# HPCForge/Bubbleformer

Measured on AMD Instinct MI355X. Metric: train samples/sec, FiLMAViT 16x192x192x4ch, bs=8 per GPU, higher is better.
Workload: dtype bf16; 1 GPU; FiLMAViT-small (E=384, 6 heads, 12 blocks, P=16, 9 fluid params) fwd + relative-L2 loss + bwd + AdamW, 4-field 16x192x192 clips, batch 8 per GPU (BASELINE.json configs[1]); global_batch=8, parallelism=dp1

## Files before the change

bubbleformer_amd/_lib.py:

```python
import ctypes as C
import os
import subprocess

_HERE = os.path.dirname(os.path.abspath(__file__))
LIB_PATH = os.path.join(_HERE, "libbubbleformer_hip.so")
CSRC = os.path.join(_HERE, "csrc")

BF_DTYPE_F32, BF_DTYPE_BF16 = 0, 1
BF_LAY_KC, BF_LAY_XC = 0, 1
BF_PRO_NONE, BF_PRO_AFFINE, BF_PRO_AFFINE_GELU, BF_PRO_GELU = 0, 1, 2, 3
BF_AUX_NONE, BF_AUX_ADD, BF_AUX_DGELU = 0, 1, 2
BF_OUT_STORE, BF_OUT_STORE_F32, BF_OUT_ATOMIC_F32 = 0, 1, 2
BF_MAX_STAGES = 5
BF_LOSS_LIMBS = 5
BF_OPT_CHUNK, BF_OPT_MAX_GROUPS = 64, 64

vp, fp, i32, i64, f32 = C.c_void_p, C.c_void_p, C.c_int32, C.c_int64, C.c_float


class Operand(C.Structure):
    _fields_ = [("p", vp), ("ld", i64), ("layout", i32), ("seglen", i32), ("segstride", i64), ("gw", i32), ("gh", i32),
                ("gc", i32), ("pro", i32), ("sc", fp), ("sh", fp), ("rows_per_frame", i32), ("nch", i32)]


class Epilogue(C.Structure):
    _fields_ = [("bias", fp), ("colscale", fp), ("colshift", fp), ("aux_mode", i32), ("aux", vp), ("ld_aux", i64),
                ("out_mode", i32), ("c", vp), ("ldc", i64), ("seglen", i32), ("segstride", i64), ("gw", i32), ("gh", i32),
                ("gc", i32), ("gelu_out", vp), ("colsum", fp), ("rowscale", fp), ("rows_per_group", i32)]


class Dims(C.Structure):
    _fields_ = [(n, i32) for n in ("dtype", "B", "T", "h", "w", "E", "heads", "attn_scale", "feat_scale", "patch", "cin",
                                   "cout", "nfluid")]


TEMPORAL_FIELDS = ("gamma", "attn_scale_factor", "norm1_w", "norm1_b", "norm2_w", "norm2_b", "input_head_w", "input_head_b",
                   "output_head_w", "output_head_b", "qnorm_w", "qnorm_b", "knorm_w", "knorm_b", "rel_pos_emb")
SPATIAL_FIELDS = ("gamma_att", "gamma_mlp", "attn_scale_factor_x", "attn_scale_factor_y", "low_freq_scalar",
                  "high_freq_scalar", "norm1_w", "norm1_b", "norm2_w", "norm2_b", "input_head_w", "input_head_b",
                  "output_head_w", "output_head_b", "qnorm_w", "qnorm_b", "knorm_w", "knorm_b", "rel_pos_emb", "fc1_w", "fc1_b",
                  "fc2_w", "fc2_b", "mlp_norm_w", "mlp_norm_b")


class TemporalParams(C.Structure):
    _fields_ = [(n, fp) for n in TEMPORAL_FIELDS]


class SpatialParams(C.Structure):
    _fields_ = [(n, fp) for n in SPATIAL_FIELDS]


class FrameNorm(C.Structure):
    _fields_ = [("w", fp), ("b", fp), ("g", fp), ("gdiv", i32), ("mean", fp), ("rstd", fp), ("sc", fp), ("sh", fp), ("resid", vp), ("out", vp)]


class EmbedParams(C.Structure):
    _fields_ = [("conv_w", fp * BF_MAX_STAGES), ("in_w", fp * BF_MAX_STAGES), ("in_b", fp * BF_MAX_STAGES), ("film_ln_w", fp),
                ("film_ln_b", fp), ("film_w", fp), ("film_b", fp)]


class DebedParams(C.Structure):
    _fields_ = [("conv_w", fp * BF_MAX_STAGES), ("in_w", fp * BF_MAX_STAGES), ("in_b", fp * BF_MAX_STAGES)]


class ConvSrc(C.Structure):
    _fields_ = [("p", vp), ("C", i32), ("nchw", i32), ("f32", i32)]


class ConvGeo(C.Structure):
    _fields_ = [(n, i32) for n in ("F", "Hi", "Wi", "Ho", "Wo", "kh", "kw", "stride", "pad")]


BF_CONV_PRO_NONE, BF_CONV_PRO_AFFINE_GELU, BF_CONV_PRO_GELU = 0, 1, 2


class RolloutStep(C.Structure):
    _fields_ = [("pred", fp), ("frames", fp), ("field_stride", i64), ("total_frames", i64), ("first", vp), ("step", vp), ("field", vp), ("diff", fp),
                ("div", fp)] + [(n, i32) for n in ("nfields", "B", "T", "C", "H", "W", "Ho", "Wo", "steps", "reserved")]


class CensusRows(C.Structure):
    _fields_ = [(n, vp) for n in ("count", "cells", "attached", "area")]


class LinkRows(C.Structure):
    _fields_ = [(n, vp) for n in ("successor", "n_successors", "predecessor", "n_predecessors", "departure_area", "events")]


class MatchRows(C.Structure):
    _fields_ = [(n, vp) for n in ("match_pred", "match_target", "overlap", "displacement", "counts", "mask")]


class ErrorRows(C.Structure):
    _fields_ = [(n, vp) for n in ("rmse", "max_error", "boundary_rmse", "interface_rmse", "interface_cells", "spectral_error", "spectrum_error",
                                  "spectrum_pred", "spectrum_target")]


class EnsembleRows(C.Structure):
    _fields_ = [(n, vp) for n in ("mean_rmse", "spread", "crps", "rank_hist", "mean")]


class OptStep(C.Structure):
    _fields_ = [("p", fp), ("g", fp), ("m", fp), ("v", fp), ("coef_dev", fp), ("avg", fp), ("chunk_group", vp), ("group_lr_scale", fp),
                ("group_weight_decay", fp), ("group_frozen", vp), ("live_dev", vp), ("n", i64), ("step", i32), ("n_groups", i32)] + [
        (n, f32) for n in ("lr", "beta1", "beta2", "eps", "wd", "gscale", "clip_value", "avg_weight")]


class ClipGatherJob(C.Structure):
    _fields_ = [("src", fp), ("idx", vp), ("first_tab", vp), ("in_field", vp), ("in_diff", fp), ("in_div", fp), ("in_out", fp), ("out_field", vp),
                ("out_diff", fp), ("out_div", fp), ("out_out", fp), ("fluid_tab", fp), ("file_tab", vp), ("fluid_out", fp), ("field_stride", i64),
                ("nframes", i64), ("nsamples", i64)] + [(n, i32) for n in ("Cin", "Tin", "Cout", "Tout", "unroll", "P", "B", "H", "W", "Ho", "Wo", "reserved")]


class ClipAugment(C.Structure):
    _fields_ = [("in_odd", vp), ("out_odd", vp), ("seed", i64), ("flip_thr", i64)] + [(n, i32) for n in ("draw", "Hc", "Wc", "crop_y", "eval_view", "reserved")]


class ClipGatherQ16Job(C.Structure):
    _fields_ = [("codes", vp), ("frame_seg", vp), ("seg_lo", fp), ("seg_step", fp), ("idx", vp), ("first_tab", vp), ("in_field", vp), ("in_diff", fp),
                ("in_div", fp), ("in_out", fp), ("out_field", vp), ("out_diff", fp), ("out_div", fp), ("out_out", fp), ("fluid_tab", fp), ("file_tab", vp),
                ("fluid_out", fp), ("field_stride", i64), ("nframes", i64), ("nsamples", i64)] + [
        (n, i32) for n in ("nfiles", "Cin", "Tin", "Cout", "Tout", "unroll", "P", "B", "H", "W", "Ho", "Wo")]


class RenderTile(C.Structure):
    _fields_ = [("a", fp), ("b", fp), ("mask", fp), ("frame_stride", i64), ("slot_stride", i64), ("mask_frame_stride", i64), ("mask_slot_stride", i64),
                ("range", vp), ("kind", i32)]


class RenderGeom(C.Structure):
    _fields_ = [(n, i32) for n in ("H", "W", "scale", "rows", "cols", "ox", "oy", "pitch_x", "pitch_y", "bar_dx", "bar_w", "img_h", "img_w", "stride")] + [
        ("stroke", C.c_double)]


BF_RENDER_SDF, BF_RENDER_TEMP, BF_RENDER_SPEED = 0, 1, 2
BF_RENDER_MAX_TILES = 6

STAGE_DONE_FN = C.CFUNCTYPE(None, C.c_int, C.c_void_p)
P = C.POINTER
SIGNATURES = {
    "bf_last_error": (C.c_char_p, []),
    "bf_abi_version": (C.c_int, []),
    "bf_prof_enable": (None, [C.c_int]),
    "bf_debug_force_generic_attn": (None, [C.c_int]),
    "bf_debug_tokred_fold": (None, [C.c_int]),
    "bf_side_defer": (None, [C.c_int]),
    "bf_prep_stages": (C.c_int, [C.POINTER(Dims), C.c_int, C.POINTER(C.c_int32), C.POINTER(vp), C.POINTER(vp), C.POINTER(vp), vp]),
    "bf_stage_prepared": (None, [C.c_int]),
    "bf_trunk_train_fwd": (C.c_int, [C.POINTER(Dims), C.c_int, C.POINTER(C.c_int32), C.POINTER(vp), C.POINTER(vp), C.POINTER(vp), C.POINTER(vp), vp,
                                     C.POINTER(vp), vp, vp]),
    "bf_trunk_train_bwd": (C.c_int, [C.POINTER(Dims), C.c_int, C.POINTER(C.c_int32), C.POINTER(vp), C.POINTER(vp), C.POINTER(vp), C.POINTER(vp),
                                     C.POINTER(vp), vp, C.POINTER(vp), vp, C.POINTER(vp), vp, vp, vp, vp, vp]),
    "bf_field_stats_ws_doubles": (i64, [C.c_int]),
    "bf_field_stats": (C.c_int, [fp, vp, vp, C.c_int, vp, vp, vp]),
    "bf_stage_chain_next": (C.c_int, [C.POINTER(Dims), C.c_int, vp, vp]),
    "bf_stage_next_scale": (C.c_int, [fp, C.c_int]),
    "bf_gemm_fwd_frames": (C.c_int, [C.c_int, C.c_int, C.c_int, C.c_int, vp, i64, vp, i64, fp, fp, fp, fp, C.c_int, vp, vp, C.c_int,
                                     C.POINTER(FrameNorm), C.POINTER(FrameNorm), vp]),
    "bf_trunk_eval_weights_bytes": (i64, [C.POINTER(Dims), C.c_int, C.POINTER(C.c_int32)]),
    "bf_trunk_eval_prepare": (C.c_int, [C.POINTER(Dims), C.c_int, C.POINTER(C.c_int32), C.POINTER(vp), vp, vp]),
    "bf_trunk_eval_fwd": (C.c_int, [C.POINTER(Dims), C.c_int, C.POINTER(C.c_int32), C.POINTER(vp), vp, vp, vp, vp, vp]),
    "bf_frame_linear": (C.c_int, [C.c_int, C.c_int, C.c_int, C.c_int, C.c_int, vp, i64, vp, i64, fp, fp, fp, fp, fp, vp, i64, C.c_int, fp, fp, fp,
                                  vp, i64, fp, fp, vp, i64, vp]),
    "bf_side_join": (C.c_int, [vp]),
    "bf_prof_report": (C.c_int, [C.c_char_p, C.c_int]),
    "bf_gemm": (C.c_int, [C.c_int, C.c_int, C.c_int, C.c_int, P(Operand), P(Operand), P(Epilogue), C.c_int, vp]),
    "bf_gemm_tokred": (C.c_int, [C.c_int, C.c_int, C.c_int, i64, vp, i64, vp, i64, fp, C.c_int, fp, fp, i64, vp]),
    "bf_gemm_tokred_ws_floats": (i64, [C.c_int, C.c_int, i64]),
    "bf_gemm_inbwd_frames": (C.c_int, [C.c_int, C.c_int, C.c_int, C.c_int, vp, i64, vp, i64, vp, vp, vp, C.c_int, fp, fp, fp, fp, fp, C.c_int, vp]),
    "bf_gemm_inbwd_frames_chain": (C.c_int, [C.c_int, C.c_int, C.c_int, C.c_int, vp, i64, vp, i64, vp, vp, vp, C.c_int, fp, fp, fp, fp, fp, C.c_int,
                                             vp, vp, fp, fp, fp, fp, C.c_int, fp, vp]),
    "bf_in_stats": (C.c_int, [C.c_int, vp, C.c_int, C.c_int, C.c_int, fp, fp, fp, C.c_int, fp, fp, fp, fp, fp, fp, vp]),
    "bf_in_ws_floats": (i64, [C.c_int, C.c_int, C.c_int, C.c_int]),
    "bf_affine_apply": (C.c_int, [C.c_int, vp, vp, fp, fp, vp, i64, C.c_int, C.c_int, vp]),
    "bf_in_bwd": (C.c_int, [C.c_int, vp, vp, vp, vp, C.c_int, C.c_int, C.c_int, fp, fp, fp, fp, fp, C.c_int, C.c_int, fp, fp,
                            fp, fp, fp, vp]),
    "bf_colsum": (C.c_int, [C.c_int, vp, i64, C.c_int, fp, fp, vp]),
    "bf_attn_axial_fwd": (C.c_int, [C.c_int, vp, vp, i64, C.c_int, C.c_int, C.c_int, C.c_int, fp, fp, fp, fp, fp, fp, fp, vp]),
    "bf_attn_axial_norm_fwd": (C.c_int, [C.c_int, vp, vp, vp, i64, C.c_int, C.c_int, C.c_int, C.c_int, fp, fp, fp, fp, fp, fp, fp, fp, fp, fp, fp, fp,
                                         fp, vp]),
    "bf_attn_fwd": (C.c_int, [C.c_int, vp, vp, i64, C.c_int, i64, i64, i64, i64, C.c_int, C.c_int, fp, fp, fp, fp, fp, fp, f32,
                              C.c_int, vp]),
    "bf_attn_bwd": (C.c_int, [C.c_int, vp, vp, vp, i64, C.c_int, i64, i64, i64, i64, C.c_int, C.c_int, fp, fp, fp, fp, fp, fp,
                              fp, fp, fp, fp, fp, fp, f32, C.c_int, fp, i64, vp]),
    "bf_im2col_nchw": (C.c_int, [C.c_int, fp, vp, C.c_int, C.c_int, C.c_int, C.c_int, C.c_int, vp]),
    "bf_col2im_nchw": (C.c_int, [C.c_int, vp, fp, C.c_int, C.c_int, C.c_int, C.c_int, C.c_int, vp]),
    "bf_pm2nchw": (C.c_int, [fp, fp, fp, fp, C.c_int, C.c_int, C.c_int, C.c_int, C.c_int, vp]),
    "bf_debed_last_bwd": (C.c_int, [C.c_int, fp, fp, fp, fp, fp, vp, vp, vp, C.c_int, C.c_int, C.c_int, C.c_int, C.c_int, C.c_int, vp]),
    "bf_debed_last_bwd_norm": (C.c_int, [C.c_int, fp, fp, fp, fp, fp, vp, vp, vp, fp, fp, fp, fp, vp, fp, fp, C.c_int, C.c_int, C.c_int, C.c_int, C.c_int,
                                         C.c_int, fp, C.c_int64, vp]),
    "bf_gather_gemm": (C.c_int, [C.c_int, vp, vp, C.c_int, fp, fp, vp, C.c_int, C.c_int, C.c_int, C.c_int, C.c_int, vp]),
    "bf_scatter_gemm": (C.c_int, [C.c_int, vp, vp, C.c_int, fp, fp, vp, fp, C.c_int, C.c_int, C.c_int, C.c_int, C.c_int, vp]),
    "bf_gather_wgrad_ws_floats": (C.c_int64, [C.c_int, C.c_int, C.c_int]),
    "bf_gather_wgrad": (C.c_int, [C.c_int, vp, vp, fp, fp, fp, fp, fp, C.c_int, C.c_int, C.c_int, C.c_int, C.c_int, C.c_int, fp, C.c_int64, vp]),
    "bf_gather_gemm_rebuilt": (C.c_int, [C.c_int, vp, vp, vp, C.c_int, fp, fp, vp, C.c_int, C.c_int, C.c_int, C.c_int, C.c_int, vp]),
    "bf_gather_wgrad_rebuilt": (C.c_int, [C.c_int, vp, vp, vp, fp, fp, fp, C.c_int, C.c_int, C.c_int, C.c_int, C.c_int, C.c_int, fp, C.c_int64, vp]),
    "bf_stage_chain_head": (C.c_int, [vp, vp, vp]),
    "bf_stage_chain_tail": (C.c_int, [vp, vp, C.c_int]),
    "bf_embed_tail_ws_floats": (C.c_int64, [C.c_int, C.c_int, C.c_int, C.c_int, C.c_int]),
    "bf_embed_tail_bwd": (C.c_int, [C.c_int, vp, vp, vp, vp, vp, fp, fp, fp, fp, fp, fp, fp, fp, C.c_int, C.c_int, C.c_int, C.c_int, C.c_int, C.c_int,
                                    fp, C.c_int64, vp]),
    "bf_embed_first": (C.c_int, [C.c_int, fp, vp, vp, vp, C.c_int, C.c_int, C.c_int, C.c_int, C.c_int, C.c_int, fp, vp]),
    "bf_in_stats_merge_slices": (C.c_int, [C.c_int, C.c_int, C.c_int, C.c_int, C.c_int, fp, fp, fp, C.c_int, fp, fp, fp, fp, fp, fp, vp]),
    "bf_debed_last": (C.c_int, [C.c_int, vp, fp, fp, vp, fp, fp, fp, C.c_int, C.c_int, C.c_int, C.c_int, C.c_int, C.c_int, vp]),
    "bf_lploss_finalize": (C.c_int, [fp, C.c_int, C.c_int, fp, fp, vp]),
    "bf_nchw2pm": (C.c_int, [C.c_int, fp, fp, fp, fp, fp, vp, C.c_int, C.c_int, C.c_int, C.c_int, C.c_int, vp]),
    "bf_wprep": (C.c_int, [C.c_int, C.c_int, fp, vp, C.c_int, C.c_int, C.c_int, vp]),
    "bf_wgrad_unprep": (C.c_int, [C.c_int, fp, fp, C.c_int, C.c_int, C.c_int, C.c_int, vp]),
    "bf_film_net_fwd": (C.c_int, [fp, fp, fp, fp, fp, fp, fp, fp, C.c_int, C.c_int, C.c_int, vp]),
    "bf_film_net_bwd": (C.c_int, [fp, fp, fp, fp, fp, fp, fp, fp, fp, C.c_int, C.c_int, C.c_int, vp]),
    "bf_adamw": (C.c_int, [P(OptStep), vp]),
    "bf_adam": (C.c_int, [P(OptStep), vp]),
    "bf_lion": (C.c_int, [P(OptStep), vp]),
    "bf_grad_norm_ws_doubles": (i64, [i64]),
    "bf_grad_norm": (C.c_int, [fp, i64, f32, f32, fp, vp, i64, vp]),
    "bf_weight_average": (C.c_int, [fp, fp, i64, f32, vp]),
    "bf_swap_buffers": (C.c_int, [fp, fp, i64, vp]),
    "bf_group_sumsq_ws_doubles": (i64, [i64]),
    "bf_group_sumsq": (C.c_int, [fp, i64, vp, C.c_int, vp, vp, i64, vp]),
    "bf_group_clip_coef": (C.c_int, [vp, vp, C.c_int, f32, f32, fp, fp, vp]),
    "bf_step_guard": (C.c_int, [fp, i32, vp, vp]),
    "bf_nonfinite_scan_ws_len": (i64, [i64]),
    "bf_nonfinite_scan": (C.c_int, [fp, i64, vp, vp, i64, vp]),
    "bf_eikonal_sum": (C.c_int, [fp, i64, C.c_int, C.c_int, f32, vp, vp]),
    "bf_eikonal_l1_frames": (C.c_int, [fp, i64, C.c_int, C.c_int, f32, fp, vp]),
    "bf_heatflux_rows": (C.c_int, [fp, fp, i64, i64, C.c_int, f32, f32, f32, f32, fp, vp]),
    "bf_clip_gather": (C.c_int, [fp, i64, vp, vp, C.c_int, fp, fp, fp, C.c_int, C.c_int, C.c_int, C.c_int, C.c_int, C.c_int, C.c_int, vp]),
    "bf_clip_gather_batch": (C.c_int, [fp, i64, vp, i64, vp, vp, fp, fp, C.c_int, C.c_int, fp, vp, fp, fp, C.c_int, C.c_int, fp, fp, vp, C.c_int, fp,
                                       C.c_int, C.c_int, C.c_int, C.c_int, C.c_int, vp]),
    "bf_clip_gather_unroll": (C.c_int, [fp, i64, i64, vp, i64, vp, vp, fp, fp, C.c_int, C.c_int, fp, vp, fp, fp, C.c_int, C.c_int, C.c_int, fp, fp, vp, C.c_int,
                                        fp, C.c_int, C.c_int, C.c_int, C.c_int, C.c_int, vp]),
    "bf_clip_gather_augment": (C.c_int, [P(ClipGatherJob), P(ClipAugment), vp]),
    "bf_clip_encode_q16": (C.c_int, [fp, vp, i64, f32, f32, vp]),
    "bf_clip_decode_q16": (C.c_int, [vp, i64, vp, fp, fp, fp, i64, C.c_int, C.c_int, C.c_int, C.c_int, vp]),
    "bf_clip_gather_q16": (C.c_int, [P(ClipGatherQ16Job), P(ClipAugment), vp]),
    "bf_clip_noise": (C.c_int, [fp, fp, fp, vp, C.c_uint64, C.c_uint32, C.c_uint32, C.c_int, C.c_int, C.c_int, C.c_int, C.c_int, vp]),
    "bf_rollout_score_ws_doubles": (i64, [C.c_int, C.c_int, C.c_int, C.c_int, C.c_int]),
    "bf_rollout_score": (C.c_int, [P(RolloutStep), C.c_int, f32, fp, fp, fp, fp, fp, fp, vp, i64, vp]),
    "bf_rollout_heatflux": (C.c_int, [P(RolloutStep), C.c_int, C.c_int, fp, f32, f32, f32, f32, fp, fp, vp]),
    "bf_kde_kl_ws_doubles": (i64, [C.c_int, i64, i64, C.c_int]),
    "bf_kde_kl": (C.c_int, [vp, vp, C.c_int, i64, i64, C.c_int, C.c_double, vp, vp, vp, vp, vp, i64, vp]),
    "bf_bubble_census_lds_cells": (i64, []),
    "bf_bubble_census_ws_bytes": (i64, [i64, C.c_int, C.c_int, C.c_int]),
    "bf_bubble_census": (C.c_int, [fp, i64, C.c_int, C.c_int, C.c_int, C.c_int, vp, vp, vp, vp, fp, vp, vp, vp, i64, vp]),
    "bf_rollout_bubbles": (C.c_int, [P(RolloutStep), C.c_int, C.c_int, C.c_int, P(CensusRows), P(CensusRows), vp, vp, i64, vp]),
    "bf_redistance_lds_cells": (i64, []),
    "bf_redistance_ws_bytes": (i64, [i64, C.c_int, C.c_int]),
    "bf_redistance": (C.c_int, [fp, i64, C.c_int, C.c_int, f32, f32, C.c_int, fp, vp, fp, vp, i64, vp]),
    "bf_rollout_redistance": (C.c_int, [P(RolloutStep), C.c_int, f32, f32, C.c_int, C.c_int, fp, vp, fp, vp, i64, vp]),
    "bf_bubble_links_lds_entries": (i64, []),
    "bf_bubble_links_ws_bytes": (i64, [i64, C.c_int]),
    "bf_bubble_links": (C.c_int, [vp, P(CensusRows), i64, C.c_int, C.c_int, C.c_int, C.c_int, P(LinkRows), vp, i64, vp]),
    "bf_bubble_track_ids": (C.c_int, [vp, vp, vp, i64, C.c_int, C.c_int, vp, vp, vp]),
    "bf_rollout_bubble_links": (C.c_int, [P(RolloutStep), C.c_int, vp, P(CensusRows), P(CensusRows), P(LinkRows), P(LinkRows), vp, i64, vp]),
    "bf_bubble_match_ws_bytes": (i64, [i64, C.c_int]),
    "bf_bubble_match": (C.c_int, [vp, vp, P(CensusRows), P(CensusRows), i64, C.c_int, C.c_int, C.c_int, C.c_float, P(MatchRows), vp, i64, vp]),
    "bf_rollout_bubble_match": (C.c_int, [P(RolloutStep), C.c_int, C.c_float, vp, P(CensusRows), P(CensusRows), P(MatchRows), vp, i64, vp]),
    "bf_field_errors_ws_bytes": (i64, [i64, C.c_int, C.c_int]),
    "bf_field_errors": (C.c_int, [fp, fp, fp, i64, C.c_int, C.c_int, C.c_int, C.c_int, C.c_int, C.c_int, P(ErrorRows), vp, i64, vp]),
    "bf_rollout_errors": (C.c_int, [P(RolloutStep), C.c_int, C.c_int, C.c_int, C.c_int, C.c_int, P(ErrorRows), vp, i64, vp]),
    "bf_ensemble_scores_ws_bytes": (i64, [C.c_int, C.c_int, C.c_int, C.c_int]),
    "bf_ensemble_scores": (C.c_int, [fp, i64, fp, C.c_int, C.c_int, C.c_int, C.c_int, C.c_int, P(EnsembleRows), vp, i64, vp]),
    "bf_rollout_ensemble": (C.c_int, [P(RolloutStep), C.c_int, C.c_int, P(EnsembleRows), vp, i64, vp]),
    "bf_render_ranges_ws_doubles": (i64, []),
    "bf_render_ranges": (C.c_int, [fp, i64, C.c_int, C.c_int, C.c_int, C.c_int, C.c_int, C.c_int, C.c_int, vp, vp, vp]),
    "bf_render_tiles": (C.c_int, [P(RenderTile), C.c_int, P(RenderGeom), i64, vp, vp, vp, vp]),
    "bf_lp_rows_ws_doubles": (i64, [i64, i64]),
    "bf_lp_rows_fwd": (C.c_int, [fp, fp, i64, i64, C.c_double, fp, vp, vp, i64, vp]),
    "bf_lp_rows_bwd": (C.c_int, [fp, fp, fp, vp, i64, i64, C.c_double, fp, vp]),
    "bf_eikonal_bwd": (C.c_int, [fp, i64, C.c_int, C.c_int, f32, fp, fp, vp]),
    "bf_wlp_ws_doubles": (i64, [i64, C.c_int, C.c_int, C.c_int]),
    "bf_wlp_fwd": (C.c_int, [fp, fp, i64, C.c_int, C.c_int, C.c_int, C.c_int, C.c_double, C.c_double, C.c_double, C.c_double, P(C.c_double), C.c_double,
                             C.c_double, fp, fp, vp, vp, i64, vp]),
    "bf_wlp_bwd": (C.c_int, [fp, fp, fp, vp, i64, C.c_int, C.c_int, C.c_int, C.c_int, C.c_double, C.c_double, C.c_double, C.c_double, P(C.c_double),
                             C.c_double, C.c_double, fp, vp]),
    "bf_slp_ws_bytes": (i64, [i64, C.c_int, C.c_int, C.c_int]),
    "bf_slp_fwd": (C.c_int, [fp, fp, i64, C.c_int, C.c_int, C.c_int, vp, P(C.c_double), C.c_int, P(C.c_double), fp, fp, vp, vp, vp, i64, vp]),
    "bf_slp_bwd": (C.c_int, [vp, fp, vp, i64, C.c_int, C.c_int, C.c_int, P(C.c_double), fp, vp]),
    "bf_temporal_saved_bytes": (i64, [P(Dims)]),
    "bf_spatial_saved_bytes": (i64, [P(Dims)]),
    "bf_embed_saved_bytes": (i64, [P(Dims)]),
    "bf_debed_saved_bytes": (i64, [P(Dims)]),
    "bf_scratch_bytes": (i64, [P(Dims)]),
    "bf_temporal_fwd": (C.c_int, [P(Dims), P(TemporalParams), vp, vp, vp, vp, fp, vp]),
    "bf_temporal_bwd": (C.c_int, [P(Dims), P(TemporalParams), P(TemporalParams), vp, vp, vp, vp, vp, fp, vp]),
    "bf_spatial_fwd": (C.c_int, [P(Dims), P(SpatialParams), vp, vp, vp, vp, fp, fp, vp]),
    "bf_spatial_bwd": (C.c_int, [P(Dims), P(SpatialParams), P(SpatialParams), vp, vp, vp, vp, vp, fp, fp, vp]),
    "bf_embed_fwd": (C.c_int, [P(Dims), P(EmbedParams), fp, fp, vp, vp, vp, vp]),
    "bf_embed_bwd": (C.c_int, [P(Dims), P(EmbedParams), P(EmbedParams), vp, fp, vp, vp, vp]),
    "bf_debed_fwd": (C.c_int, [P(Dims), P(DebedParams), vp, fp, fp, fp, vp, vp, vp]),
    "bf_debed_bwd": (C.c_int, [P(Dims), P(DebedParams), P(DebedParams), vp, fp, fp, fp, fp, vp, vp, vp, vp]),
    "bf_conv_fwd": (C.c_int, [C.c_int, P(ConvGeo), P(ConvSrc), P(ConvSrc), C.c_int, fp, fp, vp, C.c_int, fp, P(ConvSrc), P(ConvSrc),
                              C.c_int, vp]),
    "bf_conv_wgrad_ws_floats": (i64, [C.c_int, C.c_int, i64]),
    "bf_conv_wgrad": (C.c_int, [C.c_int, P(ConvGeo), P(ConvSrc), P(ConvSrc), P(ConvSrc), C.c_int, fp, fp, fp, C.c_int, fp, i64, vp]),
    "bf_conv_colsum": (C.c_int, [C.c_int, P(ConvSrc), C.c_int, C.c_int, C.c_int, fp, C.c_int, fp, i64, vp]),
    "bf_gn_ws_floats": (i64, [C.c_int, C.c_int, C.c_int]),
    "bf_gn_fwd": (C.c_int, [C.c_int, P(ConvSrc), P(ConvSrc), C.c_int, C.c_int, C.c_int, C.c_int, fp, fp, f32, fp, fp, fp, fp, fp, vp]),
    "bf_gn_bwd": (C.c_int, [C.c_int, fp, P(ConvSrc), P(ConvSrc), C.c_int, C.c_int, C.c_int, C.c_int, fp, fp, fp, fp, fp, P(ConvSrc), P(ConvSrc),
                            P(ConvSrc), fp, fp, C.c_int, fp, vp]),
    "bf_unet_lploss_fwd": (C.c_int, [fp, fp, C.c_int, C.c_int, C.c_int, i64, fp, fp, fp, vp]),
    "bf_unet_lploss_bwd": (C.c_int, [fp, fp, fp, fp, C.c_int, i64, fp, vp]),
    "bf_bn_ws_floats": (i64, [i64, C.c_int]),
    "bf_bn_fwd": (C.c_int, [C.c_int, vp, C.c_int, i64, C.c_int, fp, fp, f32, f32, fp, fp, vp, fp, fp, fp, fp, fp, vp]),
    "bf_bn_eval": (C.c_int, [C.c_int, C.c_int, fp, fp, f32, fp, fp, fp, fp, vp]),
    "bf_bn_act": (C.c_int, [C.c_int, vp, C.c_int, C.c_int, C.c_int, C.c_int, fp, fp, vp, vp, vp, vp]),
    "bf_bn_bwd": (C.c_int, [C.c_int, fp, i64, C.c_int, vp, vp, vp, C.c_int, C.c_int, C.c_int, C.c_int, fp, fp, fp, fp, fp, vp, fp, fp, C.c_int,
                            fp, vp]),
}

_lib = None


class BubbleformerHipError(RuntimeError):
    pass


def build(verbose: bool = False) -> str:
    res = subprocess.run(["make", "-j8", "-C", CSRC], capture_output=True, text=True)
    if verbose or res.returncode:
        print(res.stdout[-4000:])
        print(res.stderr[-4000:])
    if res.returncode:
        raise BubbleformerHipError("building libbubbleformer_hip.so failed")
    return LIB_PATH


def lib():
    global _lib
    if _lib is None:
        if not os.path.exists(LIB_PATH):
            raise BubbleformerHipError(
                f"{LIB_PATH} is missing: build it with `make -C {CSRC}` (or __graft_entry__.build()). "
                "bubbleformer_amd has no CPU / eager fallback.")
        import torch
        tl = os.path.join(os.path.dirname(torch.__file__), "lib", "libamdhip64.so")
        if os.path.exists(tl):
            C.CDLL(tl, mode=C.RTLD_GLOBAL)
        h = C.CDLL(LIB_PATH)
        for name, (res, args) in SIGNATURES.items():
            fn = getattr(h, name)
            fn.restype = res
            fn.argtypes = args
        _lib = h
    return _lib


def check(rc: int, what: str = "") -> None:
    if rc != 0:
        msg = lib().bf_last_error().decode(errors="replace")
        if rc == 1 and not msg.startswith("declined"):
            msg = "declined: the entry point does not cover this shape / dtype / workspace (nothing was launched)"
        raise BubbleformerHipError(f"{what} failed (code {rc}): {msg}")
```

bubbleformer_amd/csrc/attn.hip:

```cpp
#include "lane_ops.h"
#include "param_reduce.h"

namespace {

constexpr int NT = 256;
constexpr int LMAX = 32;
constexpr int LONG_LMAX = 128;
constexpr int DMAX = 128;

struct SeqGeo {
    long nseq; int L; long inner; long outer_stride; long inner_stride; long tok_stride;
};
__device__ __forceinline__ long seq_base(const SeqGeo& g, long s) {
    return (s / g.inner) * g.outer_stride + (s % g.inner) * g.inner_stride;
}

struct AttnParams {
    const float *qw, *qb, *kw, *kb;
    const float* emb;
    const float* hscale;
};
struct AttnGrads {
    float *dqw, *dqb, *dkw, *dkb, *demb, *dhscale;
};
// ... 29 lines not shown
    }
}

__device__ __forceinline__ void scores_softmax(const float* qh, const float* kh, const AttnParams& p, int head, int heads,
                                               int L, int d, int ldd, float* sP, float* sA, int lane) {
    const int lds = L + 1;
    const float scale = rsqrtf((float)d);
    for (int t = lane; t < L * L; t += 64) {
        const int i = t / L, j = t % L;
        float acc = 0.f;
        for (int e = 0; e < d; ++e) {
            const float qn = qh[i * ldd + e] * p.qw[e] + p.qb[e];
            const float kn = kh[j * ldd + e] * p.kw[e] + p.kb[e];
            acc += qn * kn;
        }
        float s = acc * scale;
        if (p.emb) s += p.emb[t5_bucket(i - j) * heads + head];
        sP[i * lds + j] = s;
    }
    wsync();
    if (lane < L) {
        float* row = sP + lane * lds;
        float m = -INFINITY;
        for (int j = 0; j < L; ++j) m = fmaxf(m, row[j]);
        float sum = 0.f;
        for (int j = 0; j < L; ++j) { const float e = __expf(row[j] - m); row[j] = e; sum += e; }
        const float inv = 1.f / sum;
        const float invL = 1.0f / (float)L;
        const float hs = p.hscale ? p.hscale[head] : 1.f;
        for (int j = 0; j < L; ++j) {
            const float pr = row[j] * inv;
            row[j] = pr;
            sA[lane * lds + j] = p.hscale ? (invL + (pr - invL) * hs) : pr;
        }
    }
    wsync();
}

template <typename T>
__global__ void __launch_bounds__(NT) attn_fwd_kernel(const T* __restrict__ qkv, T* __restrict__ out, SeqGeo g, int heads, int d,
                                                     AttnParams p, float out_scale, int accumulate) {
    extern __shared__ __attribute__((aligned(16))) float smem[];
    const int lane = threadIdx.x & 63, wave = __builtin_amdgcn_readfirstlane(threadIdx.x >> 6);
    const int L = g.L, ldd = d + 1, E = heads * d;
    const int per_wave = 3 * L * ldd + L * (L + 1) + 2 * L;
    float* q = smem + wave * per_wave;
    float* k = q + L * ldd;
    float* v = k + L * ldd;
    float* sA = v + L * ldd;
    float* rstd = sA + L * (L + 1);
    const long nprob = g.nseq * heads;
    const int WPB = blockDim.x >> 6;
    for (long pr = (long)blockIdx.x * WPB + wave; pr < nprob; pr += (long)gridDim.x * WPB) {
        const long s = pr / heads;
        const int head = (int)(pr % heads);
        const long tok0 = seq_base(g, s);
        load_rows<T>(qkv + head * 3 * d, 3L * E, q, L, 3 * d, ldd, d, tok0, g.tok_stride, lane, 1.f);
        wsync();
        ln_rows(q, k, rstd, L, d, ldd, lane);
        wsync();
        scores_softmax(q, k, p, head, heads, L, d, ldd, sA, sA, lane);
        for (int e = lane; e < d; e += 64) {
            for (int i = 0; i < L; ++i) {
                float acc = 0.f;
                for (int j = 0; j < L; ++j) acc += sA[i * (L + 1) + j] * v[j * ldd + e];
                const long o = (tok0 + i * g.tok_stride) * E + head * d + e;
                float r = acc * out_scale;
                if (accumulate) r += to_f(out[o]);
                out[o] = from_f<T>(r);
            }
        }
        wsync();
    }
}

template <typename T>
__global__ void __launch_bounds__(NT) attn_bwd_kernel(const T* __restrict__ qkv, const T* __restrict__ dout, T* __restrict__ dqkv,
                                                     SeqGeo g, int heads, int d, AttnParams p, AttnGrads gr, float out_scale,
                                                     int accumulate, float* __restrict__ ws) {
    extern __shared__ __attribute__((aligned(16))) float smem[];
    __shared__ float s_demb[NT / 64][32 * 16];
    __shared__ float s_dhs[NT / 64][16];
    __shared__ float s_diag[NT / 64][64];
    const int lane = threadIdx.x & 63, wave = __builtin_amdgcn_readfirstlane(threadIdx.x >> 6);
    const int L = g.L, ldd = d + 1, E = heads * d, lds = L + 1;
    const int per_wave = 6 * L * ldd + 2 * L * lds + 2 * L;
    float* q = smem + wave * per_wave;
    float* k = q + L * ldd;
    float* v = k + L * ldd;
    float* dO = v + L * ldd;
    float* dqn = dO + L * ldd;
    float* dkn = dqn + L * ldd;
    float* sP = dkn + L * ldd;
    float* sA = sP + L * lds;
    float* rstd = sA + L * lds;
    for (int i = threadIdx.x; i < (NT / 64) * 32 * 16; i += blockDim.x) (&s_demb[0][0])[i] = 0.f;
    if (threadIdx.x < (NT / 64) * 16) (&s_dhs[0][0])[threadIdx.x] = 0.f;
    __syncthreads();
    float a_qw[2] = {0.f, 0.f}, a_qb[2] = {0.f, 0.f}, a_kw[2] = {0.f, 0.f}, a_kb[2] = {0.f, 0.f};
    const float scale = rsqrtf((float)d);
    const long nprob = g.nseq * heads;
    const int WPB = blockDim.x >> 6;
    for (long pr = (long)blockIdx.x * WPB + wave; pr < nprob; pr += (long)gridDim.x * WPB) {
        const long s = pr / heads;
        const int head = (int)(pr % heads);
        const long tok0 = seq_base(g, s);
        load_rows<T>(qkv + head * 3 * d, 3L * E, q, L, 3 * d, ldd, d, tok0, g.tok_stride, lane, 1.f);
        load_rows<T>(dout + head * d, (long)E, dO, L, d, ldd, d, tok0, g.tok_stride, lane, out_scale);
        wsync();
        ln_rows(q, k, rstd, L, d, ldd, lane);
        wsync();
        scores_softmax(q, k, p, head, heads, L, d, ldd, sP, sA, lane);
        const float hs = p.hscale ? p.hscale[head] : 1.f;
        const float invL = 1.0f / (float)L;
        float dhs_part = 0.f;
        for (int e = lane; e < d; e += 64)
            for (int j = 0; j < L; ++j) {
                float acc = 0.f;
                for (int i = 0; i < L; ++i) acc += sA[i * lds + j] * dO[i * ldd + e];
                dqn[j * ldd + e] = acc;
            }
        wsync();
        {
            constexpr int CH = Chunk<T>::N;
            const int cpr = d / CH;
            for (int i = lane; i < L * cpr; i += 64) {
                const int l = i / cpr, e0 = (i % cpr) * CH;
                T* dst = dqkv + (tok0 + l * g.tok_stride) * 3L * E + head * 3 * d + 2 * d + e0;
                Chunk<T> o, old;
                if (accumulate) old.load(dst);
#pragma unroll
                for (int j = 0; j < CH; ++j) o.set(j, dqn[l * ldd + e0 + j] + (accumulate ? old.get(j) : 0.f));
                o.store(dst);
            }
        }
        wsync();
        for (int t = lane; t < L * L; t += 64) {
            const int i = t / L, j = t % L;
            float acc = 0.f;
            for (int e = 0; e < d; ++e) acc += dO[i * ldd + e] * v[j * ldd + e];
            if (p.hscale) { dhs_part += (sP[i * lds + j] - invL) * acc; acc *= hs; }
            sA[i * lds + j] = acc;
        }
        wsync();
        if (lane < L) {
            float dot = 0.f;
            for (int j = 0; j < L; ++j) dot += sP[lane * lds + j] * sA[lane * lds + j];
            for (int j = 0; j < L; ++j) sA[lane * lds + j] = sP[lane * lds + j] * (sA[lane * lds + j] - dot);
        }
        wsync();
        if (gr.demb) {
            if (lane < 2 * L - 1) {
                const int dd = lane - (L - 1);
                float t = 0.f;
                for (int i = max(0, dd); i < min(L, L + dd); ++i) t += sA[i * lds + (i - dd)];
                s_diag[wave][lane] = t;
            }
            wsync();
            if (lane < 32) {
                float t = 0.f;
                for (int q = 0; q < 2 * L - 1; ++q)
                    if (t5_bucket(q - (L - 1)) == lane) t += s_diag[wave][q];
                s_demb[wave][lane * 16 + head] += t;
            }
            wsync();
        }
        if (p.hscale) {
            dhs_part = wave_sum(dhs_part);
            if (lane == 0 && gr.dhscale) s_dhs[wave][head] += dhs_part;
        }
        for (int e = lane; e < d; e += 64) {
            const float kw = p.kw[e], kb = p.kb[e], qw = p.qw[e], qb = p.qb[e];
            for (int i = 0; i < L; ++i) {
                float a1 = 0.f, a2 = 0.f;
                for (int j = 0; j < L; ++j) {
                    a1 += sA[i * lds + j] * (k[j * ldd + e] * kw + kb);
                    a2 += sA[j * lds + i] * (q[j * ldd + e] * qw + qb);
                }
                dqn[i * ldd + e] = a1 * scale;
                dkn[i * ldd + e] = a2 * scale;
            }
        }
        wsync();
#pragma unroll
        for (int c = 0; c < 2; ++c) {
            const int e = lane + 64 * c;
            if (e < d) {
                float sw = 0.f, sb = 0.f, tw = 0.f, tb = 0.f;
                for (int i = 0; i < L; ++i) {
                    sw += dqn[i * ldd + e] * q[i * ldd + e]; sb += dqn[i * ldd + e];
                    tw += dkn[i * ldd + e] * k[i * ldd + e]; tb += dkn[i * ldd + e];
                }
                a_qw[c] += sw; a_qb[c] += sb; a_kw[c] += tw; a_kb[c] += tb;
            }
        }
        wsync();
        if (lane < 2 * L) {
            const bool isq = lane < L;
            const int r = isq ? lane : lane - L;
            float* dn = (isq ? dqn : dkn) + r * ldd;
            const float* xh = (isq ? q : k) + r * ldd;
            const float* w = isq ? p.qw : p.kw;
            float m1 = 0.f, m2 = 0.f;
            for (int e = 0; e < d; ++e) { const float gg = dn[e] * w[e]; m1 += gg; m2 += gg * xh[e]; }
            m1 /= (float)d; m2 /= (float)d;
            const float rs = rstd[lane];
            for (int e = 0; e < d; ++e) dn[e] = rs * (dn[e] * w[e] - m1 - xh[e] * m2);
        }
        wsync();
        {
            constexpr int CH = Chunk<T>::N;
            const int cpr = d / CH;
            for (int i = lane; i < 2 * L * cpr; i += 64) {
                const int part = i / (L * cpr);
                const int l = (i / cpr) % L, e0 = (i % cpr) * CH;
                const float* src = (part ? dkn : dqn) + l * ldd + e0;
                T* dst = dqkv + (tok0 + l * g.tok_stride) * 3L * E + head * 3 * d + part * d + e0;
                Chunk<T> o, old;
                if (accumulate) old.load(dst);
#pragma unroll
                for (int j = 0; j < CH; ++j) o.set(j, src[j] + (accumulate ? old.get(j) : 0.f));
                o.store(dst);
            }
        }
        wsync();
    }
#pragma unroll
    for (int c = 0; c < 2; ++c) {
        const int e = lane + 64 * c;
        if (e < d) { q[e] = a_qw[c]; q[d + e] = a_qb[c]; q[2 * d + e] = a_kw[c]; q[3 * d + e] = a_kb[c]; }
    }
    __syncthreads();
    const int nvals = 4 * d + 32 * heads + heads;
    for (int i = threadIdx.x; i < nvals; i += blockDim.x) {
        float val = 0.f;
        float* dst;
        if (i < 4 * d) {
            for (int w = 0; w < WPB; ++w) val += smem[w * per_wave + i];
            const int pq = i / d, e = i % d;
            dst = pq == 0 ? gr.dqw : pq == 1 ? gr.dqb : pq == 2 ? gr.dkw : gr.dkb;
            if (dst) dst += e;
        } else if (i < 4 * d + 32 * heads) {
            const int t = i - 4 * d;
            for (int w = 0; w < WPB; ++w) val += s_demb[w][(t / heads) * 16 + (t % heads)];
            dst = gr.demb ? gr.demb + t : nullptr;
        } else {
            const int t = i - 4 * d - 32 * heads;
            for (int w = 0; w < WPB; ++w) val += s_dhs[w][t];
            dst = gr.dhscale ? gr.dhscale + t : nullptr;
        }
        if (ws) ws[(long)blockIdx.x * nvals + i] = val;
        else if (dst && val != 0.f) atomicAdd(dst, val);
    }
}

__global__ void __launch_bounds__(64 * BF_RED_FL) attn_rows_reduce_kernel(AttnReduceJob j) {
    __shared__ float red[1][BF_RED_FL][64];
    attn_reduce_block(j, blockIdx.x, 0, 1, red);
}

template <typename K>
int plan_waves(K kernel, size_t floats_per_wave, int* wpb, size_t* shm) {
    int w = 4;
    while (w > 1 && (size_t)w * floats_per_wave * sizeof(float) > 64 * 1024) w >>= 1;
    *wpb = w;
    *shm = (size_t)w * floats_per_wave * sizeof(float);
    if (*shm > 156 * 1024) return bf_fail_msg("attention: L*d too large for the LDS plan", __FILE__, __LINE__);
    if (*shm > 64 * 1024) {
        hipError_t e = hipFuncSetAttribute(reinterpret_cast<const void*>(kernel), hipFuncAttributeMaxDynamicSharedMemorySize, (int)*shm);
        if (e != hipSuccess) return bf_fail(e, __FILE__, __LINE__);
    }
    return 0;
}

bool g_force_generic = false;

int check_geo(const char* who, int dtype, int heads, int d, int L) {
    const int ch = dtype == BF_DTYPE_BF16 ? 8 : 4;
    if (heads < 1 || heads > 16) return bf_fail_msg("attention: heads must be in 1..16", who, 0);
    if (d < ch || d > DMAX || d % ch) return bf_fail_msg("attention: head dim must be a multiple of the 16-byte chunk and <= 128", who, 0);
    if (L < 1 || L > LONG_LMAX) return bf_fail_msg("attention: sequence length must be in 1..128", who, 0);
    return 0;
}

}

int bf_attn_fwd_mfma(const void* qkv, void* out, long nseq, int L, long inner, long outer_stride, long inner_stride, long tok_stride, int heads,
                     int d, const float* qw, const float* qb, const float* kw, const float* kb, const float* emb, const float* hscale,
                     float out_scale, int accumulate, hipStream_t st);
int bf_attn_bwd_mfma(const void* qkv, const void* dout, void* dqkv, long nseq, int L, long inner, long outer_stride, long inner_stride,
                     long tok_stride, int heads, int d, const float* qw, const float* qb, const float* kw, const float* kb, const float* emb,
                     const float* hscale, float* dqw, float* dqb, float* dkw, float* dkb, float* demb, float* dhscale, float out_scale,
                     int accumulate, float* ws, long ws_floats, int* rows_out, hipStream_t st);
int bf_attn_fwd_long(int dtype, const void* qkv, void* out, long nseq, int L, long inner, long outer_stride, long inner_stride, long tok_stride,
                     int heads, int d, const float* qw, const float* qb, const float* kw, const float* kb, const float* emb, const float* hscale,
                     float out_scale, int accumulate, hipStream_t st);
int bf_attn_bwd_long(int dtype, const void* qkv, const void* dout, void* dqkv, long nseq, int L, long inner, long outer_stride, long inner_stride,
                     long tok_stride, int heads, int d, const float* qw, const float* qb, const float* kw, const float* kb, const float* emb,
                     const float* hscale, float* dqw, float* dqb, float* dkw, float* dkb, float* demb, float* dhscale, float out_scale,
                     int accumulate, float* ws, long ws_floats, int* rows_out, hipStream_t st);
int bf_attn_axial_fwd_mfma(const void* qkv, void* out, int frames, int h, int w, int heads, int d, const float* qw, const float* qb, const float* kw,
                           const float* kb, const float* emb, const float* hscale_x, const float* hscale_y, const float* nw, const float* nb,
                           void* out_n, float* mean, float* rstd, float* sc, float* sh, hipStream_t st);
static bool use_mfma(int dtype, int d) { return !g_force_generic && dtype == BF_DTYPE_BF16 && d % 32 == 0 && d <= 128; }
bool bf_attn_raw_modes(int dtype, int d) { return use_mfma(dtype, d); }

extern "C" void bf_debug_force_generic_attn(int on) { g_force_generic = on != 0; }

extern "C" int bf_attn_fwd(int dtype, const void* qkv, void* out, int64_t nseq, int L, int64_t inner, int64_t outer_stride,
                           int64_t inner_stride, int64_t tok_stride, int heads, int d, const float* qw, const float* qb,
                           const float* kw, const float* kb, const float* emb, const float* hscale, float out_scale,
                           int accumulate, bf_stream_t stream) {
    BF_REQUIRE(qkv && out && qw && qb && kw && kb && nseq > 0 && inner > 0, "bf_attn_fwd: bad arguments");
    if (int rc = check_geo("bf_attn_fwd", dtype, heads, d, L)) return rc;
    if (L > LMAX) {
        BfProfScope prof((hipStream_t)stream, "attn_fwd", 4.0 * nseq * heads * L * L * d, (double)nseq * heads * L * d * bf_esize(dtype) * (accumulate ? 5.0 : 4.0));
        return bf_attn_fwd_long(dtype, qkv, out, nseq, L, inner, outer_stride, inner_stride, tok_stride, heads, d, qw, qb, kw, kb, emb, hscale,
                                out_scale, accumulate, (hipStream_t)stream);
    }
    if (use_mfma(dtype, d)) {
        BfProfScope prof((hipStream_t)stream, "attn_fwd", 4.0 * nseq * heads * L * L * d, (double)nseq * heads * L * d * 2.0 * (accumulate ? 5.0 : 4.0));
        return bf_attn_fwd_mfma(qkv, out, nseq, L, inner, outer_stride, inner_stride, tok_stride, heads, d, qw, qb, kw, kb, emb, hscale, out_scale,
                                accumulate, (hipStream_t)stream);
    }
    SeqGeo g{nseq, L, inner, outer_stride, inner_stride, tok_stride};
    AttnParams p{qw, qb, kw, kb, emb, hscale};
    const size_t fpw = 3 * L * (d + 1) + L * (L + 1) + 2 * L;
    int WPB; size_t shm;
    if (int rc = dtype == BF_DTYPE_BF16 ? plan_waves(attn_fwd_kernel<bf16>, fpw, &WPB, &shm) : plan_waves(attn_fwd_kernel<float>, fpw, &WPB, &shm)) return rc;
    const long nprob = nseq * heads;
    BfProfScope prof((hipStream_t)stream, "attn_fwd", 4.0 * nprob * L * L * d, (double)nprob * L * d * bf_esize(dtype) * (accumulate ? 5.0 : 4.0));
    const int grid = (int)std::min<long>((nprob + WPB - 1) / WPB, 256 * 8);
    if (dtype == BF_DTYPE_BF16)
        hipLaunchKernelGGL(attn_fwd_kernel<bf16>, dim3(grid), dim3(WPB * 64), shm, (hipStream_t)stream, (const bf16*)qkv, (bf16*)out, g, heads, d, p, out_scale, accumulate);
    else
        hipLaunchKernelGGL(attn_fwd_kernel<float>, dim3(grid), dim3(WPB * 64), shm, (hipStream_t)stream, (const float*)qkv, (float*)out, g, heads, d, p, out_scale, accumulate);
    BF_CHECK_LAUNCH();
    return 0;
}

extern "C" int bf_attn_axial_fwd(int dtype, const void* qkv, void* out, int64_t frames, int h, int w, int heads, int d, const float* qw,
                                 const float* qb, const float* kw, const float* kb, const float* emb, const float* hscale_x,
                                 const float* hscale_y, bf_stream_t stream) {
    BF_REQUIRE(qkv && out && qw && qb && kw && kb && frames > 0 && h > 0 && w > 0, "bf_attn_axial_fwd: bad arguments");
    if (use_mfma(dtype, d) && frames < (1L << 24)) {
        BfProfScope prof((hipStream_t)stream, "attn_fwd", 4.0 * frames * heads * h * w * (h + w) * d, (double)frames * h * w * heads * d * 2.0 * 4.0);
        const int rc = bf_attn_axial_fwd_mfma(qkv, out, (int)frames, h, w, heads, d, qw, qb, kw, kb, emb, hscale_x, hscale_y, nullptr, nullptr, nullptr,
                                              nullptr, nullptr, nullptr, nullptr, (hipStream_t)stream);
        if (rc <= 0) return rc;
    }
    const long S = (long)h * w;
    int rc = bf_attn_fwd(dtype, qkv, out, frames * h, w, 1, w, 0, 1, heads, d, qw, qb, kw, kb, emb, hscale_x, 0.5f, 0, stream);
    if (rc) return rc;
    return bf_attn_fwd(dtype, qkv, out, frames * w, h, w, S, 1, w, heads, d, qw, qb, kw, kb, emb, hscale_y, 0.5f, 1, stream);
}

extern "C" int bf_attn_axial_norm_fwd(int dtype, const void* qkv, void* out, void* out_n, int64_t frames, int h, int w, int heads, int d,
                                      const float* qw, const float* qb, const float* kw, const float* kb, const float* emb,
                                      const float* hscale_x, const float* hscale_y, const float* norm_w, const float* norm_b, float* mean,
                                      float* rstd, float* sc, float* sh, bf_stream_t stream) {
    BF_REQUIRE(qkv && out && out_n && qw && qb && kw && kb && norm_w && norm_b && mean && rstd && sc && sh && frames > 0 && h > 0 && w > 0,
               "bf_attn_axial_norm_fwd: bad arguments");
    static const bool off = bf_knob("BF_ATTN_AXIAL_NORM", 1) == 0;
    if (off || !use_mfma(dtype, d) || frames >= (1L << 24)) return 1;
    BfProfScope prof((hipStream_t)stream, "attn_fwd", 4.0 * frames * heads * h * w * (h + w) * d, (double)frames * h * w * heads * d * 2.0 * 5.0);
    return bf_attn_axial_fwd_mfma(qkv, out, (int)frames, h, w, heads, d, qw, qb, kw, kb, emb, hscale_x, hscale_y, norm_w, norm_b, out_n, mean, rstd, sc,
                                  sh, (hipStream_t)stream);
}

static int attn_bwd_impl(int dtype, const void* qkv, const void* dout, void* dqkv, int64_t nseq, int L, int64_t inner,
                         int64_t outer_stride, int64_t inner_stride, int64_t tok_stride, int heads, int d, const float* qw,
                         const float* qb, const float* kw, const float* kb, const float* emb, const float* hscale,
                         float* dqw, float* dqb, float* dkw, float* dkb, float* demb, float* dhscale, float out_scale,
                         int accumulate, float* ws, int64_t ws_floats, int* rows_out, bf_stream_t stream) {
    if (rows_out) *rows_out = 0;
    BF_REQUIRE(qkv && dout && dqkv && qw && qb && kw && kb && nseq > 0 && inner > 0, "bf_attn_bwd: bad arguments");
    if (int rc = check_geo("bf_attn_bwd", dtype, heads, d, L)) return rc;
    BF_REQUIRE(accumulate == 0 || accumulate == 1 || ((accumulate == 2 || accumulate == 5) && use_mfma(dtype, d)),
               "bf_attn_bwd: accumulate must be 0 / 1 (or 2 / 5, the raw-gradient pair of passes, on the bf16 MFMA path)");
    if (L > LMAX) {
        BfProfScope prof((hipStream_t)stream, "attn_bwd", 10.0 * nseq * heads * L * L * d, (double)nseq * heads * L * d * bf_esize(dtype) * (accumulate ? 10.0 : 7.0));
        return bf_attn_bwd_long(dtype, qkv, dout, dqkv, nseq, L, inner, outer_stride, inner_stride, tok_stride, heads, d, qw, qb, kw, kb, emb, hscale,
                                dqw, dqb, dkw, dkb, demb, dhscale, out_scale, accumulate, ws, (long)ws_floats, rows_out, (hipStream_t)stream);
    }
    if (use_mfma(dtype, d)) {
        BfProfScope prof((hipStream_t)stream, "attn_bwd", 10.0 * nseq * heads * L * L * d, (double)nseq * heads * L * d * 2.0 * (accumulate ? 10.0 : 7.0));
        return bf_attn_bwd_mfma(qkv, dout, dqkv, nseq, L, inner, outer_stride, inner_stride, tok_stride, heads, d, qw, qb, kw, kb, emb, hscale, dqw,
                                dqb, dkw, dkb, demb, dhscale, out_scale, accumulate, ws, (long)ws_floats, rows_out, (hipStream_t)stream);
    }
    SeqGeo g{nseq, L, inner, outer_stride, inner_stride, tok_stride};
    AttnParams p{qw, qb, kw, kb, emb, hscale};
    AttnGrads gr{dqw, dqb, dkw, dkb, demb, dhscale};
    const size_t fpw = 6 * L * (d + 1) + 2 * L * (L + 1) + 2 * L;
    int WPB; size_t shm;
    if (int rc = dtype == BF_DTYPE_BF16 ? plan_waves(attn_bwd_kernel<bf16>, fpw, &WPB, &shm) : plan_waves(attn_bwd_kernel<float>, fpw, &WPB, &shm)) return rc;
    const long nprob = nseq * heads;
    BfProfScope prof((hipStream_t)stream, "attn_bwd", 10.0 * nprob * L * L * d, (double)nprob * L * d * bf_esize(dtype) * (accumulate ? 10.0 : 7.0));
    const int full = (int)std::min<long>((nprob + WPB - 1) / WPB, 256 * 4), nvals = 4 * d + 32 * heads + heads;
    int grid = full;
    if (ws && ws_floats < (int64_t)full * nvals) { grid = (int)(ws_floats / nvals); if (grid < 1) { ws = nullptr; grid = full; } }
    if (dtype == BF_DTYPE_BF16)
        hipLaunchKernelGGL(attn_bwd_kernel<bf16>, dim3(grid), dim3(WPB * 64), shm, (hipStream_t)stream, (const bf16*)qkv, (const bf16*)dout, (bf16*)dqkv, g, heads, d, p, gr, out_scale, accumulate, ws);
    else
        hipLaunchKernelGGL(attn_bwd_kernel<float>, dim3(grid), dim3(WPB * 64), shm, (hipStream_t)stream, (const float*)qkv, (const float*)dout, (float*)dqkv, g, heads, d, p, gr, out_scale, accumulate, ws);
    BF_CHECK_LAUNCH();
    if (rows_out) { *rows_out = ws ? grid : 0; return 0; }
    if (ws) {
        const AttnReduceJob j{ws, grid, d, heads, dqw, dqb, dkw, dkb, demb, dhscale};
        hipLaunchKernelGGL(attn_rows_reduce_kernel, dim3(bf_cdiv(nvals, 64)), dim3(64 * BF_RED_FL), 0, (hipStream_t)stream, j);
        BF_CHECK_LAUNCH();
    }
    return 0;
}

extern "C" int bf_attn_bwd(int dtype, const void* qkv, const void* dout, void* dqkv, int64_t nseq, int L, int64_t inner,
                           int64_t outer_stride, int64_t inner_stride, int64_t tok_stride, int heads, int d, const float* qw,
                           const float* qb, const float* kw, const float* kb, const float* emb, const float* hscale,
                           float* dqw, float* dqb, float* dkw, float* dkb, float* demb, float* dhscale, float out_scale,
                           int accumulate, float* ws, int64_t ws_floats, bf_stream_t stream) {
    return attn_bwd_impl(dtype, qkv, dout, dqkv, nseq, L, inner, outer_stride, inner_stride, tok_stride, heads, d, qw, qb, kw, kb, emb, hscale, dqw,
                         dqb, dkw, dkb, demb, dhscale, out_scale, accumulate, ws, ws_floats, nullptr, stream);
}
int bf_attn_bwd_partials(int dtype, const void* qkv, const void* dout, void* dqkv, int64_t nseq, int L, int64_t inner, int64_t outer_stride,
                         int64_t inner_stride, int64_t tok_stride, int heads, int d, const float* qw, const float* qb, const float* kw,
                         const float* kb, const float* emb, const float* hscale, float* dqw, float* dqb, float* dkw, float* dkb, float* demb,
                         float* dhscale, float out_scale, int accumulate, float* ws, int64_t ws_floats, int* rows, hipStream_t stream) {
    return attn_bwd_impl(dtype, qkv, dout, dqkv, nseq, L, inner, outer_stride, inner_stride, tok_stride, heads, d, qw, qb, kw, kb, emb, hscale, dqw,
                         dqb, dkw, dkb, demb, dhscale, out_scale, accumulate, ws, ws_floats, rows, (bf_stream_t)stream);
}
```

bubbleformer_amd/csrc/attn_mfma.hip:

```cpp
#include "lane_ops.h"
#include "param_reduce.h"
#include <stdlib.h>

namespace {


struct Geo { long nseq; int L; long inner, outer_stride, inner_stride, tok_stride; };
struct Prob { long tok0; int head; };
__device__ __forceinline__ Prob locate(const Geo& g, int heads, long pr) {
    const unsigned p = (unsigned)pr, hd = (unsigned)heads, inner = (unsigned)g.inner;
    const unsigned s = p / hd, head = p - s * hd;
    const unsigned q = s / inner, r = s - q * inner;
    return Prob{(long)q * g.outer_stride + (long)r * g.inner_stride, (int)head};
}
__device__ __forceinline__ float row16_scatter_sum(const float (&p)[16], int i16) {
    float a0, a1, a2, a3, a4, a5, a6, a7, b[4];
#define BF_M1(a, lo, hi) "v_add_f32_dpp " a ", " lo ", " lo " row_mirror row_mask:0xf bank_mask:0x3\n\t" \
                         "v_add_f32_dpp " a ", " hi ", " hi " row_mirror row_mask:0xf bank_mask:0xc\n\t"
#define BF_M2(b, lo, hi) "v_add_f32_dpp " b ", " lo ", " lo " row_half_mirror row_mask:0xf bank_mask:0x5\n\t" \
                         "v_add_f32_dpp " b ", " hi ", " hi " row_half_mirror row_mask:0xf bank_mask:0xa\n\t"
    asm("s_nop 4\n\t"
        BF_M1("%4", "%12", "%20") BF_M1("%5", "%13", "%21") BF_M1("%6", "%14", "%22") BF_M1("%7", "%15", "%23")
        BF_M1("%8", "%16", "%24") BF_M1("%9", "%17", "%25") BF_M1("%10", "%18", "%26") BF_M1("%11", "%19", "%27")
        BF_M2("%0", "%4", "%8") BF_M2("%1", "%5", "%9") BF_M2("%2", "%6", "%10") BF_M2("%3", "%7", "%11")
// ... 177 lines not shown
    constexpr int D = 32 * KS, LD = D + 16, NT16 = D / 16;
    constexpr bool PREFETCH = NB * KS <= 4;
    extern __shared__ __attribute__((aligned(16))) bf16 smem_fwd[];
    __shared__ __attribute__((aligned(16))) float s_par[4 * 32 * KS];
    __shared__ float s_emb[32 * 16];
    __shared__ float s_hsc[16];
    const int lane = threadIdx.x & 63, wave = __builtin_amdgcn_readfirstlane(threadIdx.x >> 6), wpb = blockDim.x >> 6;
    bf16* vt = smem_fwd + wave * (16 * NB * LD);
    for (int i = threadIdx.x; i < 32 * 16; i += blockDim.x) {
        const int t = i >> 4, h = i & 15;
        s_emb[i] = (p.emb && h < heads) ? p.emb[t * heads + h] : 0.f;
    }
    if (threadIdx.x < 16) s_hsc[threadIdx.x] = (p.hscale && (int)threadIdx.x < heads) ? p.hscale[threadIdx.x] : 1.f;
    for (int i = threadIdx.x; i < 4 * D; i += blockDim.x) {
        const int q = i / D, e = i % D;
        s_par[i] = (q == 0 ? p.qw : q == 1 ? p.qb : q == 2 ? p.kw : p.kb)[e];
    }
    __syncthreads();
    const int E = heads * D, L = g.L;
    const float scale = rsqrtf((float)D);
    const long nprob = g.nseq * heads;
    const int gq = lane >> 4, i16 = lane & 15;
    const long pstep = (long)gridDim.x * wpb;
    long pr = (long)blockIdx.x * wpb + wave;
    FwdRows<NB, KS> cur, nxt;
    Prob at = locate(g, heads, pr < nprob ? pr : 0), at_next = at;
    if (pr < nprob) load_fwd_rows<NB, KS>(cur, qkv, g, heads, at, lane);
    if (PREFETCH) drain_vm();
    float mk[NB][NB][4], mneg[NB][NB][4];
    int eidx[NB][NB][4];
    lane_masks<NB>(L, lane, mk, mneg, eidx);
    for (; pr < nprob; pr += pstep) {
        const int head = at.head;
        const long tok0 = at.tok0;
        const bool more = pr + pstep < nprob;
        if (more) at_next = locate(g, heads, pr + pstep);
        if (PREFETCH && more) load_fwd_rows<NB, KS>(nxt, qkv, g, heads, at_next, lane);
        bf16x4 old[NB][NT16];
        if (accumulate) {
#pragma unroll
            for (int ib = 0; ib < NB; ++ib) {
                const int i = 16 * ib + i16, ic = i < L ? i : L - 1;
#pragma unroll
                for (int t = 0; t < NT16; ++t)
                    old[ib][t] = *reinterpret_cast<const bf16x4*>(out + (tok0 + ic * g.tok_stride) * (long)E + head * D + 16 * t + 4 * gq);
            }
        }
        bf16x8 qf[NB][KS], kf[NB][KS];
#pragma unroll
        for (int b = 0; b < NB; ++b) {
            float x[KS][8];
#pragma unroll
            for (int ks = 0; ks < KS; ++ks)
#pragma unroll
                for (int j = 0; j < 8; ++j) x[ks][j] = (float)cur.q[b][ks][j];
            ln_quad<KS>(x, D);
            affine_frag<KS>(x, s_par, s_par + D, scale, lane, qf[b]);
#pragma unroll
            for (int ks = 0; ks < KS; ++ks)
#pragma unroll
                for (int j = 0; j < 8; ++j) x[ks][j] = (float)cur.k[b][ks][j];
            ln_quad<KS>(x, D);
            affine_frag<KS>(x, s_par + 2 * D, s_par + 3 * D, 1.f, lane, kf[b]);
            const int row = b * 16 + i16;
#pragma unroll
            for (int ks = 0; ks < KS; ++ks) {
                bf16x8 zv = cur.v[b][ks];
                if (row >= L) {
#pragma unroll
                    for (int j = 0; j < 8; ++j) zv[j] = (bf16)0.f;
                }
                *reinterpret_cast<bf16x8*>(vt + row * LD + 32 * ks + 8 * gq) = zv;
            }
        }
        float P[NB][NB][4], A[NB][NB][4];
        scores_softmax_pre<NB, KS>(kf, qf, s_emb, eidx, mneg, mk, p.hscale ? s_hsc : nullptr, head, L, P, A);
        wsync();
#pragma unroll
        for (int ib = 0; ib < NB; ++ib) {
            const bf16x8 pa = pack_keys<NB>(A, ib);
            const int i = 16 * ib + i16;
#pragma unroll
            for (int t = 0; t < NT16; ++t) {
                f32x4 o = {0.f, 0.f, 0.f, 0.f};
                o = __builtin_amdgcn_mfma_f32_16x16x32_bf16(tr_keys<NB>(vt, LD, t, lane), pa, o, 0, 0, 0);
                if (i < L) {
                    bf16* dst = out + (tok0 + i * g.tok_stride) * (long)E + head * D + 16 * t + 4 * gq;
                    float v[4] = {o[0] * out_scale, o[1] * out_scale, o[2] * out_scale, o[3] * out_scale};
                    if (accumulate) {
#pragma unroll
                        for (int r = 0; r < 4; ++r) v[r] += (float)old[ib][t][r];
                    }
                    const bf16x4 w4 = {(bf16)v[0], (bf16)v[1], (bf16)v[2], (bf16)v[3]};
                    *reinterpret_cast<bf16x4*>(dst) = w4;
                }
            }
        }
        wsync();
        if (PREFETCH) cur = nxt;
        else if (more) load_fwd_rows<NB, KS>(cur, qkv, g, heads, at_next, lane);
        at = at_next;
    }
}

struct AxNorm { const float* w; const float* b; bf16* out_n; float* mean; float* rstd; float* sc; float* sh; };
template <int KS, bool NORM, int WPB = 4>
__global__ void __launch_bounds__(64 * WPB) attn_fwd_axial_mfma(const bf16* __restrict__ qkv, bf16* __restrict__ out, int frames, int h, int w, int heads, Par p,
                                                           const float* __restrict__ hscale_y, AxNorm nrm) {
    constexpr int NB = 1, D = 32 * KS, LD = D + 16, NT16 = D / 16, DP = D + 8;
    extern __shared__ __attribute__((aligned(16))) bf16 smem_ax[];
    __shared__ __attribute__((aligned(16))) float s_par[4 * 32 * KS];
    __shared__ float s_emb[32 * 16];
    __shared__ float s_hsx[16], s_hsy[16];
    const int lane = threadIdx.x & 63, wave = __builtin_amdgcn_readfirstlane(threadIdx.x >> 6), wpb = blockDim.x >> 6;
    bf16* vt = smem_ax + wave * (16 * LD);
    bf16* ot = smem_ax + wpb * (16 * LD);
    for (int i = threadIdx.x; i < 32 * 16; i += blockDim.x) {
        const int t = i >> 4, hd = i & 15;
        s_emb[i] = (p.emb && hd < heads) ? p.emb[t * heads + hd] : 0.f;
    }
    if (threadIdx.x < 16) {
        s_hsx[threadIdx.x] = (p.hscale && (int)threadIdx.x < heads) ? p.hscale[threadIdx.x] : 1.f;
        s_hsy[threadIdx.x] = (hscale_y && (int)threadIdx.x < heads) ? hscale_y[threadIdx.x] : 1.f;
    }
    for (int i = threadIdx.x; i < 4 * D; i += blockDim.x) {
        const int q = i / D, e = i % D;
        s_par[i] = (q == 0 ? p.qw : q == 1 ? p.qb : q == 2 ? p.kw : p.kb)[e];
    }
    __syncthreads();
    const int E = heads * D, S = h * w;
    const float scale = rsqrtf((float)D);
    const int gq = lane >> 4, i16 = lane & 15;
    const Geo gW{(long)frames * h, w, 1, w, 0, 1}, gH{(long)frames * w, h, w, S, 1, w};
    const int RW = (h + wpb - 1) / wpb, RH = (w + wpb - 1) / wpb;
    float mkW[NB][NB][4], mnegW[NB][NB][4], mkH[NB][NB][4], mnegH[NB][NB][4];
    int eidxW[NB][NB][4], eidxH[NB][NB][4];
    lane_masks<NB>(w, lane, mkW, mnegW, eidxW);
    lane_masks<NB>(h, lane, mkH, mnegH, eidxH);
    const long ntile = (long)frames * heads;
    for (long tile = blockIdx.x; tile < ntile; tile += gridDim.x) {
        const int frame = (int)((unsigned)tile / (unsigned)heads), head = (int)((unsigned)tile - (unsigned)frame * (unsigned)heads);
        for (int k = 0; k < RW + RH; ++k) {
            const bool isH = k >= RW;
            const int idx = wave + (isH ? k - RW : k) * wpb;
            const int L = isH ? h : w;
            if (k == RW) __syncthreads();
            if (idx < (isH ? w : h)) {
                const Geo& g = isH ? gH : gW;
                const long seq = (long)frame * (isH ? w : h) + idx;
                FwdRows<NB, KS> cur;
                load_fwd_rows<NB, KS>(cur, qkv, g, heads, locate(g, heads, seq * heads + head), lane);
                bf16x8 qf[NB][KS], kf[NB][KS];
                {
                    float x[KS][8];
#pragma unroll
                    for (int ks = 0; ks < KS; ++ks)
#pragma unroll
                        for (int j = 0; j < 8; ++j) x[ks][j] = (float)cur.q[0][ks][j];
                    ln_quad<KS>(x, D);
                    affine_frag<KS>(x, s_par, s_par + D, scale, lane, qf[0]);
#pragma unroll
                    for (int ks = 0; ks < KS; ++ks)
#pragma unroll
                        for (int j = 0; j < 8; ++j) x[ks][j] = (float)cur.k[0][ks][j];
                    ln_quad<KS>(x, D);
                    affine_frag<KS>(x, s_par + 2 * D, s_par + 3 * D, 1.f, lane, kf[0]);
#pragma unroll
                    for (int ks = 0; ks < KS; ++ks) {
                        bf16x8 zv = cur.v[0][ks];
                        if (i16 >= L) {
#pragma unroll
                            for (int j = 0; j < 8; ++j) zv[j] = (bf16)0.f;
                        }
                        *reinterpret_cast<bf16x8*>(vt + i16 * LD + 32 * ks + 8 * gq) = zv;
                    }
                }
                float P[NB][NB][4], A[NB][NB][4];
                if (isH) scores_softmax_pre<NB, KS>(kf, qf, s_emb, eidxH, mnegH, mkH, hscale_y ? s_hsy : nullptr, head, L, P, A);
                else scores_softmax_pre<NB, KS>(kf, qf, s_emb, eidxW, mnegW, mkW, p.hscale ? s_hsx : nullptr, head, L, P, A);
                wsync();
                const bf16x8 pa = pack_keys<NB>(A, 0);
#pragma unroll
                for (int t = 0; t < NT16; ++t) {
                    f32x4 o = {0.f, 0.f, 0.f, 0.f};
                    o = __builtin_amdgcn_mfma_f32_16x16x32_bf16(tr_keys<NB>(vt, LD, t, lane), pa, o, 0, 0, 0);
                    if (i16 < L) {
                        const int tok = isH ? i16 * w + idx : idx * w + i16;
                        bf16* cell = ot + tok * DP + 16 * t + 4 * gq;
                        float v[4] = {o[0] * 0.5f, o[1] * 0.5f, o[2] * 0.5f, o[3] * 0.5f};
                        if (isH) {
                            const bf16x4 old = *reinterpret_cast<const bf16x4*>(cell);
#pragma unroll
                            for (int r = 0; r < 4; ++r) v[r] += (float)old[r];
                        }
                        const bf16x4 w4 = {(bf16)v[0], (bf16)v[1], (bf16)v[2], (bf16)v[3]};
                        if (isH && !NORM) *reinterpret_cast<bf16x4*>(out + ((long)frame * S + tok) * E + head * D + 16 * t + 4 * gq) = w4;
                        else *reinterpret_cast<bf16x4*>(cell) = w4;
                    }
                }
                wsync();
            }
        }
        __syncthreads();
        if constexpr (NORM) {
            constexpr int CPR = D / 8, RGN = 256 / CPR;
            float* red = reinterpret_cast<float*>(ot + ((S * DP + 7) & ~7));
            float* stat = red + RGN * D;
            const int cg = threadIdx.x % CPR, rg = threadIdx.x / CPR;
            const bool act = rg < RGN;
            float acc[8];
#pragma unroll
            for (int j = 0; j < 8; ++j) acc[j] = 0.f;
            if (act)
                for (int r = rg; r < S; r += RGN) {
                    const bf16x8 v = *reinterpret_cast<const bf16x8*>(ot + r * DP + cg * 8);
#pragma unroll
                    for (int j = 0; j < 8; ++j) acc[j] += (float)v[j];
                }
            if (act) {
#pragma unroll
                for (int j = 0; j < 8; ++j) red[rg * D + cg * 8 + j] = acc[j];
            }
            __syncthreads();
            if ((int)threadIdx.x < D) {
                float t = 0.f;
                for (int g2 = 0; g2 < RGN; ++g2) t += red[g2 * D + threadIdx.x];
                stat[threadIdx.x] = t / (float)S;
            }
            __syncthreads();
            float mu[8];
#pragma unroll
            for (int j = 0; j < 8; ++j) { mu[j] = stat[cg * 8 + j]; acc[j] = 0.f; }
            if (act)
                for (int r = rg; r < S; r += RGN) {
                    const bf16x8 v = *reinterpret_cast<const bf16x8*>(ot + r * DP + cg * 8);
#pragma unroll
                    for (int j = 0; j < 8; ++j) { const float dlt = (float)v[j] - mu[j]; acc[j] += dlt * dlt; }
                }
            if (act) {
#pragma unroll
                for (int j = 0; j < 8; ++j) red[rg * D + cg * 8 + j] = acc[j];
            }
            __syncthreads();
            if ((int)threadIdx.x < D) {
                float t = 0.f;
                for (int g2 = 0; g2 < RGN; ++g2) t += red[g2 * D + threadIdx.x];
                const float r = rsqrtf(t / (float)S + BF_IN_EPS);
                const int c = head * D + threadIdx.x;
                const long o = (long)frame * E + c;
                const float a = r * nrm.w[c], m = stat[threadIdx.x];
                stat[D + threadIdx.x] = r;
                nrm.mean[o] = m; nrm.rstd[o] = r; nrm.sc[o] = a; nrm.sh[o] = nrm.b[c] - m * a;
            }
            __syncthreads();
            if (act) {
                float aa[8], ss[8];
#pragma unroll
                for (int j = 0; j < 8; ++j) {
                    const int c = head * D + cg * 8 + j;
                    aa[j] = stat[D + cg * 8 + j] * nrm.w[c];
                    ss[j] = nrm.b[c] - mu[j] * aa[j];
                }
                for (int r = rg; r < S; r += RGN) {
                    const bf16x8 v = *reinterpret_cast<const bf16x8*>(ot + r * DP + cg * 8);
                    bf16x8 nv;
#pragma unroll
                    for (int j = 0; j < 8; ++j) nv[j] = (bf16)((float)v[j] * aa[j] + ss[j]);
                    const long go = ((long)frame * S + r) * E + head * D + cg * 8;
                    *reinterpret_cast<bf16x8*>(out + go) = v;
                    *reinterpret_cast<bf16x8*>(nrm.out_n + go) = nv;
                }
            }
            __syncthreads();
        }
    }
}

template <int NB, int KS> struct RawRows { bf16x8 q[NB][KS], k[NB][KS], v[NB][KS], d[NB][KS]; };
template <int NB, int KS> struct OldRows { bf16x8 q[NB][KS], k[NB][KS], v[NB][KS]; };

template <int NB, int KS>
__device__ __forceinline__ void load_raw(RawRows<NB, KS>& r, const bf16* __restrict__ qkv, const bf16* __restrict__ dout, const Geo& g, int heads, const Prob& at,
                                         int lane) {
    constexpr int D = 32 * KS;
    const int E = heads * D;
    const int head = at.head;
    const long tok0 = at.tok0;
    const int gq = lane >> 4, i16 = lane & 15;
#pragma unroll
    for (int b = 0; b < NB; ++b) {
        const int i = b * 16 + i16, ic = i < g.L ? i : g.L - 1;
        const bf16* rp = qkv + (tok0 + ic * g.tok_stride) * 3L * E + head * 3 * D + 8 * gq;
        const bf16* dp = dout + (tok0 + ic * g.tok_stride) * (long)E + head * D + 8 * gq;
#pragma unroll
        for (int ks = 0; ks < KS; ++ks) {
            r.q[b][ks] = *reinterpret_cast<const bf16x8*>(rp + 32 * ks);
            r.k[b][ks] = *reinterpret_cast<const bf16x8*>(rp + D + 32 * ks);
            r.v[b][ks] = *reinterpret_cast<const bf16x8*>(rp + 2 * D + 32 * ks);
            r.d[b][ks] = *reinterpret_cast<const bf16x8*>(dp + 32 * ks);
        }
    }
}

template <int NB, int KS, int ACC>
__global__ void __launch_bounds__(256, ((NB == 1 && KS <= 2) ? 2 : 1)) attn_bwd_mfma(const bf16* __restrict__ qkv, const bf16* __restrict__ dout, bf16* __restrict__ dqkv, Geo g,
                                                     int heads, Par p, Grd gr, float out_scale, int accumulate_rt, float* __restrict__ ws) {
    constexpr int D = 32 * KS, LD = D + 16, NT16 = D / 16, R = 16 * NB, LDP = 32 + 8;
    constexpr bool PREFETCH = NB * KS <= 4;
    extern __shared__ __attribute__((aligned(16))) bf16 smem_bwd[];
    __shared__ float s_demb[32 * 16];
    __shared__ float s_dhs[16];
    __shared__ __attribute__((aligned(16))) float s_par[4 * 32 * KS];
    __shared__ float s_emb[32 * 16];
    __shared__ float s_hsc[16];
    const int lane = threadIdx.x & 63, wave = __builtin_amdgcn_readfirstlane(threadIdx.x >> 6), wpb = blockDim.x >> 6;
    constexpr int PER_WAVE = 3 * R * LD + 2 * R * LDP;
    static_assert(3 * R * LD * 2 >= 4 * D * 4, "the parameter-gradient flush must fit in the operand tiles");
    bf16* qn_t = smem_bwd + wave * PER_WAVE;
    bf16* kn_t = qn_t + R * LD;
    bf16* do_t = kn_t + R * LD;
    bf16* at_t = do_t + R * LD;
    bf16* ds_t = at_t + R * LDP;
    float* relay = reinterpret_cast<float*>(qn_t);
    for (int i = threadIdx.x; i < 32 * 16; i += blockDim.x) {
        s_demb[i] = 0.f;
        const int t = i >> 4, h = i & 15;
        s_emb[i] = (p.emb && h < heads) ? p.emb[t * heads + h] : 0.f;
    }
    if (threadIdx.x < 16) { s_dhs[threadIdx.x] = 0.f; s_hsc[threadIdx.x] = (p.hscale && (int)threadIdx.x < heads) ? p.hscale[threadIdx.x] : 1.f; }
    for (int i = threadIdx.x; i < 4 * D; i += blockDim.x) {
        const int q = i / D, e = i % D;
        s_par[i] = (q == 0 ? p.qw : q == 1 ? p.qb : q == 2 ? p.kw : p.kb)[e];
    }
    __syncthreads();
    const int E = heads * D, L = g.L;
    const float scale = rsqrtf((float)D);
    const long nprob = g.nseq * heads;
    const int gq = lane >> 4, i16 = lane & 15;
    const int mode = ACC >= 0 ? ACC : accumulate_rt;
    const bool raw_out = mode & 2, raw_in = mode & 4, accumulate = mode & 1;

    constexpr int NACC = 2 * KS;
    float a_ln[NACC];
#pragma unroll
    for (int k = 0; k < NACC; ++k) a_ln[k] = 0.f;
    const long pstep = (long)gridDim.x * wpb;
    const bool one_head = pstep % heads == 0;
    float a_emb[NB][NB][4], a_dhs = 0.f;
#pragma unroll
    for (int jb = 0; jb < NB; ++jb)
#pragma unroll
        for (int ib = 0; ib < NB; ++ib)
#pragma unroll
            for (int r = 0; r < 4; ++r) a_emb[jb][ib][r] = 0.f;
    long pr = (long)blockIdx.x * wpb + wave;
    RawRows<NB, KS> cur, nxt;
    Prob at = locate(g, heads, pr < nprob ? pr : 0), at_next = at;
    if (pr < nprob) load_raw<NB, KS>(cur, qkv, dout, g, heads, at, lane);
    if (PREFETCH) drain_vm();
    float mk[NB][NB][4], mneg[NB][NB][4];
    int eidx[NB][NB][4];
    lane_masks<NB>(L, lane, mk, mneg, eidx);
    if (NB == 1) {
        for (int c = lane; c < 16 * 16; c += 64) { at_t[(c >> 4) * LDP + 16 + (c & 15)] = (bf16)0.f; ds_t[(c >> 4) * LDP + 16 + (c & 15)] = (bf16)0.f; }
    }
    for (; pr < nprob; pr += pstep) {
        const int head = at.head;
        const long tok0 = at.tok0;
        const bool more = pr + pstep < nprob;
        if (more) at_next = locate(g, heads, pr + pstep);
        if (PREFETCH && more) load_raw<NB, KS>(nxt, qkv, dout, g, heads, at_next, lane);
        OldRows<NB, KS> old;
        if (accumulate) {
#pragma unroll
            for (int b = 0; b < NB; ++b) {
                const int row = b * 16 + i16, rc = row < L ? row : L - 1;
                const bf16* ob = dqkv + (tok0 + rc * g.tok_stride) * 3L * E + head * 3 * D;
#pragma unroll
                for (int ks = 0; ks < KS; ++ks) {
                    old.q[b][ks] = *reinterpret_cast<const bf16x8*>(ob + 32 * ks + 8 * gq);
                    old.k[b][ks] = *reinterpret_cast<const bf16x8*>(ob + D + 32 * ks + 8 * gq);
                    old.v[b][ks] = *reinterpret_cast<const bf16x8*>(ob + 2 * D + 32 * ks + 8 * gq);
                }
                if (raw_in && row >= L) {
                    const bf16x8 z8 = {};
#pragma unroll
                    for (int ks = 0; ks < KS; ++ks) { old.q[b][ks] = z8; old.k[b][ks] = z8; }
                }
            }
        }
        float xq[NB][KS][8], xk[NB][KS][8], rq[NB], rk[NB];
        bf16x8 qf[NB][KS], kf[NB][KS], vf[NB][KS], df[NB][KS];
#pragma unroll
        for (int b = 0; b < NB; ++b) {
#pragma unroll
            for (int ks = 0; ks < KS; ++ks)
#pragma unroll
                for (int j = 0; j < 8; ++j) { xq[b][ks][j] = (float)cur.q[b][ks][j]; xk[b][ks][j] = (float)cur.k[b][ks][j]; }
            rq[b] = ln_quad<KS>(xq[b], D);
            affine_frag<KS>(xq[b], s_par, s_par + D, scale, lane, qf[b]);
            rk[b] = ln_quad<KS>(xk[b], D);
            affine_frag<KS>(xk[b], s_par + 2 * D, s_par + 3 * D, 1.f, lane, kf[b]);
            const int row = b * 16 + i16;
#pragma unroll
            for (int ks = 0; ks < KS; ++ks) {
                vf[b][ks] = cur.v[b][ks];
                df[b][ks] = cur.d[b][ks];
#define BF_HALVES(tile, v) { \
                    *reinterpret_cast<bf16x4*>(tile + row * LD + 32 * ks + 4 * gq) = __builtin_shufflevector(v, v, 0, 1, 2, 3); \
                    *reinterpret_cast<bf16x4*>(tile + row * LD + 32 * ks + 16 + 4 * gq) = __builtin_shufflevector(v, v, 4, 5, 6, 7); }
                BF_HALVES(qn_t, qf[b][ks]) BF_HALVES(kn_t, kf[b][ks]) BF_HALVES(do_t, df[b][ks])
#undef BF_HALVES
            }
        }
        float P[NB][NB][4], A[NB][NB][4], dA[NB][NB][4];
        scores_softmax_pre<NB, KS>(kf, qf, s_emb, eidx, mneg, mk, p.hscale ? s_hsc : nullptr, head, L, P, A);
        const float hs = s_hsc[head];
        const float invL = 1.0f / (float)L;
        float dhs = 0.f;
#pragma unroll
        for (int jb = 0; jb < NB; ++jb)
#pragma unroll
            for (int ib = 0; ib < NB; ++ib) {
                f32x4 acc = {0.f, 0.f, 0.f, 0.f};
#pragma unroll
                for (int ks = 0; ks < KS; ++ks) acc = __builtin_amdgcn_mfma_f32_16x16x32_bf16(vf[jb][ks], df[ib][ks], acc, 0, 0, 0);
#pragma unroll
                for (int r = 0; r < 4; ++r) {
                    float v = acc[r] * out_scale * mk[jb][ib][r];
                    if (p.hscale) { dhs += (P[jb][ib][r] - invL) * v; v *= hs; }
                    dA[jb][ib][r] = v;
                }
            }
#pragma unroll
        for (int ib = 0; ib < NB; ++ib) {
            float dot = 0.f;
#pragma unroll
            for (int jb = 0; jb < NB; ++jb)
#pragma unroll
                for (int r = 0; r < 4; ++r) dot += P[jb][ib][r] * dA[jb][ib][r];
            dot = quad_sum(dot);
#pragma unroll
            for (int jb = 0; jb < NB; ++jb)
#pragma unroll
                for (int r = 0; r < 4; ++r) {
                    const int i = 16 * ib + i16, j = 16 * jb + 4 * gq + r;
                    const float v = P[jb][ib][r] * (dA[jb][ib][r] - dot) * mk[jb][ib][r];
                    dA[jb][ib][r] = v;
                    if (one_head) a_emb[jb][ib][r] += v;
                    else if (gr.demb && i < L && j < L) atomicAdd(&s_demb[eidx[jb][ib][r] + head], v);
                    at_t[j * LDP + i] = (bf16)A[jb][ib][r];
                    ds_t[j * LDP + i] = (bf16)v;
                }
        }
        if (one_head) a_dhs += dhs;
        else if (p.hscale && gr.dhscale) {
            dhs = wave_sum(dhs);
            if (lane == 0) atomicAdd(&s_dhs[head], dhs);
        }
        wsync();
        float dq[NB][NT16][4], dk[NB][NT16][4];
        f32x4 dv_even[NB];
#pragma unroll
        for (int t = 0; t < NT16; ++t) {
            const bf16x8 doT = tr_nat<NB>(do_t, LD, t, lane);
            const bf16x8 qnT = tr_nat<NB>(qn_t, LD, t, lane);
            const bf16x8 knT = tr_keys<NB>(kn_t, LD, t, lane);
#pragma unroll
            for (int jb = 0; jb < NB; ++jb) {
                const bf16x8 aB = *reinterpret_cast<const bf16x8*>(at_t + (16 * jb + i16) * LDP + 8 * gq);
                const bf16x8 sB = *reinterpret_cast<const bf16x8*>(ds_t + (16 * jb + i16) * LDP + 8 * gq);
                f32x4 z = {0.f, 0.f, 0.f, 0.f};
                const f32x4 dv = __builtin_amdgcn_mfma_f32_16x16x32_bf16(doT, aB, z, 0, 0, 0);
                const f32x4 dkk = __builtin_amdgcn_mfma_f32_16x16x32_bf16(qnT, sB, z, 0, 0, 0);
#pragma unroll
                for (int r = 0; r < 4; ++r) dk[jb][t][r] = dkk[r];
                if (!(t & 1)) dv_even[jb] = dv;
                else {
                    const int j = 16 * jb + i16, ks = t >> 1;
                    if (j < L) {
                        bf16x8 o;
#pragma unroll
                        for (int r = 0; r < 4; ++r) {
                            float lo = dv_even[jb][r] * out_scale, hi = dv[r] * out_scale;
                            if (accumulate) { lo += (float)old.v[jb][ks][r]; hi += (float)old.v[jb][ks][4 + r]; }
                            o[r] = (bf16)lo; o[4 + r] = (bf16)hi;
                        }
                        *reinterpret_cast<bf16x8*>(dqkv + (tok0 + j * g.tok_stride) * 3L * E + head * 3 * D + 2 * D + 32 * ks + 8 * gq) = o;
                    }
                }
            }
#pragma unroll
            for (int ib = 0; ib < NB; ++ib) {
                f32x4 z = {0.f, 0.f, 0.f, 0.f};
                const f32x4 dqq = __builtin_amdgcn_mfma_f32_16x16x32_bf16(knT, pack_keys<NB>(dA, ib), z, 0, 0, 0);
#pragma unroll
                for (int r = 0; r < 4; ++r) dq[ib][t][r] = dqq[r] * scale;
            }
        }
        if (raw_out) {
#pragma unroll
            for (int b = 0; b < NB; ++b) {
                const int row = 16 * b + i16;
                if (row < L) {
                    bf16* dst = dqkv + (tok0 + row * g.tok_stride) * 3L * E + head * 3 * D + 8 * gq;
#pragma unroll
                    for (int ks = 0; ks < KS; ++ks) {
                        bf16x8 oq, ok;
#pragma unroll
                        for (int j = 0; j < 8; ++j) {
                            float vq = dq[b][2 * ks + (j >> 2)][j & 3], vk = dk[b][2 * ks + (j >> 2)][j & 3];
                            if (accumulate) { vq += (float)old.q[b][ks][j]; vk += (float)old.k[b][ks][j]; }
                            oq[j] = (bf16)vq; ok[j] = (bf16)vk;
                        }
                        *reinterpret_cast<bf16x8*>(dst + 32 * ks) = oq;
                        *reinterpret_cast<bf16x8*>(dst + D + 32 * ks) = ok;
                    }
                }
            }
        } else
#pragma unroll
        for (int part = 0; part < 2; ++part) {
            const float* w = part == 0 ? s_par : s_par + 2 * D;
            float pw[KS][8], pb[KS][8];
#pragma unroll
            for (int ks = 0; ks < KS; ++ks)
#pragma unroll
                for (int j = 0; j < 8; ++j) pw[ks][j] = pb[ks][j] = 0.f;
#pragma unroll
            for (int b = 0; b < NB; ++b) {
                const int row = 16 * b + i16;
                float dn[KS][8];
                float m1 = 0.f, m2 = 0.f;
#pragma unroll
                for (int ks = 0; ks < KS; ++ks) {
#pragma unroll
                    for (int j = 0; j < 8; ++j) {
                        const float xh = part == 0 ? xq[b][ks][j] : xk[b][ks][j];
                        float d0 = part == 0 ? dq[b][2 * ks + (j >> 2)][j & 3] : dk[b][2 * ks + (j >> 2)][j & 3];
                        if (raw_in) d0 += (float)(part == 0 ? old.q[b][ks][j] : old.k[b][ks][j]);
                        pw[ks][j] += d0 * xh;
                        pb[ks][j] += d0;
                        const float gg = d0 * w[32 * ks + 8 * gq + j];
                        dn[ks][j] = gg;
                        m1 += gg; m2 += gg * xh;
                    }
                }
                m1 = quad_sum(m1) / (float)D;
                m2 = quad_sum(m2) / (float)D;
                const float rs = part == 0 ? rq[b] : rk[b];
                if (row < L) {
                    bf16* dst = dqkv + (tok0 + row * g.tok_stride) * 3L * E + head * 3 * D + part * D + 8 * gq;
#pragma unroll
                    for (int ks = 0; ks < KS; ++ks) {
                        bf16x8 o;
#pragma unroll
                        for (int j = 0; j < 8; ++j) {
                            const float xh = part == 0 ? xq[b][ks][j] : xk[b][ks][j];
                            float v = rs * (dn[ks][j] - m1 - xh * m2);
                            if (accumulate && !raw_in) v += (float)(part == 0 ? old.q[b][ks][j] : old.k[b][ks][j]);
                            o[j] = (bf16)v;
                        }
                        *reinterpret_cast<bf16x8*>(dst + 32 * ks) = o;
                    }
                }
            }
            {
                float flat[16 * KS];
#pragma unroll
                for (int ks = 0; ks < KS; ++ks)
#pragma unroll
                    for (int j = 0; j < 8; ++j) { flat[8 * ks + j] = pw[ks][j]; flat[8 * KS + 8 * ks + j] = pb[ks][j]; }
#pragma unroll
                for (int gi = 0; gi < KS; ++gi) {
                    float grp[16];
#pragma unroll
                    for (int q = 0; q < 16; ++q) grp[q] = flat[16 * gi + q];
                    a_ln[part * KS + gi] += row16_scatter_sum(grp, i16);
                }
            }
        }
        wsync();
        if (PREFETCH) cur = nxt;
        else if (more) load_raw<NB, KS>(cur, qkv, dout, g, heads, at_next, lane);
        at = at_next;
    }
    if (one_head && pr - pstep >= 0) {
        const int head = (int)(((long)blockIdx.x * wpb + wave) % heads);
#pragma unroll
        for (int jb = 0; jb < NB; ++jb)
#pragma unroll
            for (int ib = 0; ib < NB; ++ib)
#pragma unroll
                for (int r = 0; r < 4; ++r) {
                    const int i = 16 * ib + i16, j = 16 * jb + 4 * gq + r;
                    if (gr.demb && i < L && j < L) atomicAdd(&s_demb[t5_bucket(i - j) * 16 + head], a_emb[jb][ib][r]);
                }
        if (p.hscale && gr.dhscale) {
            a_dhs = wave_sum(a_dhs);
            if (lane == 0) atomicAdd(&s_dhs[head], a_dhs);
        }
    }
#pragma unroll
    for (int k = 0; k < NACC; ++k) {
        const int v = 16 * k + i16, q = v / (8 * KS), ks = (v >> 3) % KS, j = v & 7;
        relay[q * D + 32 * ks + 8 * gq + j] = a_ln[k];
    }
    __syncthreads();
    const int nvals = 4 * D + 32 * heads + heads;
    for (int i = threadIdx.x; i < nvals; i += blockDim.x) {
        float val;
        float* dst;
        if (i < 4 * D) {
            val = 0.f;
            for (int w = 0; w < wpb; ++w) val += reinterpret_cast<const float*>(smem_bwd + w * PER_WAVE)[i];
            const int q = i / D, e = i % D; dst = (q == 0 ? gr.dqw : q == 1 ? gr.dqb : q == 2 ? gr.dkw : gr.dkb); if (dst) dst += e; }
        else if (i < 4 * D + 32 * heads) { const int t = i - 4 * D; val = s_demb[(t / heads) * 16 + (t % heads)]; dst = gr.demb ? gr.demb + t : nullptr; }
        else { const int t = i - 4 * D - 32 * heads; val = s_dhs[t]; dst = gr.dhscale ? gr.dhscale + t : nullptr; }
        if (ws) ws[(long)blockIdx.x * nvals + i] = val;
        else if (dst && val != 0.f) atomicAdd(dst, val);
    }
}

__global__ void __launch_bounds__(64 * BF_RED_FL) attn_ws_reduce(AttnReduceJob j) {
    __shared__ float red[1][BF_RED_FL][64];
    attn_reduce_block(j, blockIdx.x, blockIdx.y, gridDim.y, red);
}

template <typename K>
int set_lds(K kernel, size_t shm) {
    if (shm > 64 * 1024) {
        hipError_t e = hipFuncSetAttribute(reinterpret_cast<const void*>(kernel), hipFuncAttributeMaxDynamicSharedMemorySize, (int)shm);
        if (e != hipSuccess) return bf_fail(e, __FILE__, __LINE__);
    }
    return 0;
}

template <int NB, int KS>
int go_fwd(const bf16* qkv, bf16* out, Geo g, int heads, Par p, float out_scale, int accumulate, hipStream_t st) {
    constexpr int D = 32 * KS;
    const int wpb = 4;
    const size_t shm = (size_t)wpb * 16 * NB * (D + 16) * sizeof(bf16);
    const long nprob = g.nseq * heads;
    BF_REQUIRE(nprob < (1L << 31) && g.inner < (1L << 31), "attention: problem count must fit 31 bits");
    static const int bpc = bf_knob("BF_ATTN_FWD_BPC", 2);
    const int grid = (int)std::min<long>((nprob + wpb - 1) / wpb, 256L * bpc);
    hipLaunchKernelGGL((attn_fwd_mfma<NB, KS>), dim3(grid), dim3(wpb * 64), shm, st, qkv, out, g, heads, p, out_scale, accumulate);
    BF_CHECK_LAUNCH();
    return 0;
}
template <int NB, int KS, int ACC>
int go_bwd_mode(const bf16* qkv, const bf16* dout, bf16* dqkv, Geo g, int heads, Par p, Grd gr, float out_scale, int accumulate, float* ws,
                long ws_floats, int* rows_out, hipStream_t st) {
    constexpr int D = 32 * KS, R = 16 * NB;
    const int wpb = NB == 1 ? 4 : 2;
    const size_t shm = (size_t)wpb * (3 * R * (D + 16) + 2 * R * 40) * sizeof(bf16);
    if (int rc = set_lds(attn_bwd_mfma<NB, KS, ACC>, shm)) return rc;
    const long nprob = g.nseq * heads;
    BF_REQUIRE(nprob < (1L << 31) && g.inner < (1L << 31), "attention: problem count must fit 31 bits");
    const int nvals = 4 * D + 32 * heads + heads;
    static int resident = 0;
    if (!resident) {
        int dev = 0, cus = 256, per_cu = 1;
        (void)hipGetDevice(&dev);
        (void)hipDeviceGetAttribute(&cus, hipDeviceAttributeMultiprocessorCount, dev);
        if (hipOccupancyMaxActiveBlocksPerMultiprocessor(&per_cu, attn_bwd_mfma<NB, KS, ACC>, wpb * 64, shm) != hipSuccess || per_cu < 1) per_cu = 1;
        static const int bpc = bf_knob("BF_ATTN_BWD_BPC", 0);
        if (bpc > 0) per_cu = bpc;
        resident = cus * per_cu;
    }
    long grid = std::min<long>((nprob + wpb - 1) / wpb, (long)resident);
    {
        long a = wpb, b = heads;
        while (b) { const long t = a % b; a = b; b = t; }
        const long m = heads / a;
        if (grid >= 8 * m) grid -= grid % m;
    }
    if (ws && ws_floats < grid * nvals) { grid = ws_floats / nvals; if (grid < 1) ws = nullptr; }
    hipLaunchKernelGGL((attn_bwd_mfma<NB, KS, ACC>), dim3((int)grid), dim3(wpb * 64), shm, st, qkv, dout, dqkv, g, heads, p, gr, out_scale, accumulate, ws);
    BF_CHECK_LAUNCH();
    if (rows_out) { *rows_out = ws ? (int)grid : 0; return 0; }
    if (ws) {
        const AttnReduceJob j{ws, (int)grid, D, heads, gr.dqw, gr.dqb, gr.dkw, gr.dkb, gr.demb, gr.dhscale};
        hipLaunchKernelGGL(attn_ws_reduce, dim3(bf_cdiv(nvals, 64), 1), dim3(64 * BF_RED_FL), 0, st, j);
        BF_CHECK_LAUNCH();
    }
    return 0;
}
template <int NB, int KS>
int go_bwd(const bf16* qkv, const bf16* dout, bf16* dqkv, Geo g, int heads, Par p, Grd gr, float out_scale, int accumulate, float* ws,
           long ws_floats, int* rows_out, hipStream_t st) {
#define BF_MODE(A) return go_bwd_mode<NB, KS, A>(qkv, dout, dqkv, g, heads, p, gr, out_scale, accumulate, ws, ws_floats, rows_out, st)
    if constexpr (NB == 1 && KS == 2) {
        switch (accumulate) { case 0: BF_MODE(0); case 1: BF_MODE(1); case 2: BF_MODE(2); case 5: BF_MODE(5); default: break; }
    }
    BF_MODE(-1);
#undef BF_MODE
}

}

int bf_attn_fwd_mfma(const void* qkv, void* out, long nseq, int L, long inner, long outer_stride, long inner_stride, long tok_stride, int heads,
                     int d, const float* qw, const float* qb, const float* kw, const float* kb, const float* emb, const float* hscale,
                     float out_scale, int accumulate, hipStream_t st) {
    Geo g{nseq, L, inner, outer_stride, inner_stride, tok_stride};
    Par p{qw, qb, kw, kb, emb, hscale};
    const int nb = L <= 16 ? 1 : 2, ks = d / 32;
#define GO(NB, KS) if (nb == NB && ks == KS) return go_fwd<NB, KS>((const bf16*)qkv, (bf16*)out, g, heads, p, out_scale, accumulate, st)
    GO(1, 1); GO(1, 2); GO(1, 3); GO(1, 4); GO(2, 1); GO(2, 2); GO(2, 3); GO(2, 4);
#undef GO
    return bf_fail_msg("bf_attn_fwd_mfma: unsupported shape", __FILE__, __LINE__);
}
int bf_attn_axial_fwd_mfma(const void* qkv, void* out, int frames, int h, int w, int heads, int d, const float* qw, const float* qb, const float* kw,
                           const float* kb, const float* emb, const float* hscale_x, const float* hscale_y, const float* nw, const float* nb,
                           void* out_n, float* mean, float* rstd, float* sc, float* sh, hipStream_t st) {
    static const bool off = bf_knob("BF_ATTN_AXIAL_FUSED", 1) == 0;
    if (off || h > 16 || w > 16 || h < 1 || w < 1 || d % 32 || d > 128 || heads > 16) return 1;
    Par p{qw, qb, kw, kb, emb, hscale_x};
    const long ntile = (long)frames * heads;
    static const int wpb_env = bf_knob("BF_ATTN_AXIAL_WPB", 0);
    const int ks = d / 32, wpb = (wpb_env == 4 || wpb_env == 12) ? wpb_env : (ntile <= 256 ? 12 : 4);
    const bool norm = nw != nullptr;
    const size_t tile = ((size_t)h * w * (d + 8) + 7) & ~(size_t)7;
    const size_t shm = ((size_t)wpb * 16 * (d + 16) + tile) * sizeof(bf16) + (norm ? ((size_t)(256 / (d / 8)) + 2) * d * sizeof(float) : 0);
    const int grid = (int)std::min<long>(ntile, 256L * 3);
    const AxNorm nrm{nw, nb, (bf16*)out_n, mean, rstd, sc, sh};
#define GO2(KS, NRM, W) { if (int rc = set_lds(attn_fwd_axial_mfma<KS, NRM, W>, shm)) return rc; \
        hipLaunchKernelGGL((attn_fwd_axial_mfma<KS, NRM, W>), dim3(grid), dim3(W * 64), shm, st, (const bf16*)qkv, (bf16*)out, frames, h, w, heads, p, hscale_y, nrm); }
#define GO(KS) if (ks == KS) { \
        if (norm) { if (wpb == 12) GO2(KS, true, 12) else GO2(KS, true, 4) } \
        else { if (wpb == 12) GO2(KS, false, 12) else GO2(KS, false, 4) } }
    GO(1) GO(2) GO(3) GO(4)
#undef GO
#undef GO2
    BF_CHECK_LAUNCH();
    return 0;
}
int bf_attn_bwd_mfma(const void* qkv, const void* dout, void* dqkv, long nseq, int L, long inner, long outer_stride, long inner_stride,
                     long tok_stride, int heads, int d, const float* qw, const float* qb, const float* kw, const float* kb, const float* emb,
                     const float* hscale, float* dqw, float* dqb, float* dkw, float* dkb, float* demb, float* dhscale, float out_scale,
                     int accumulate, float* ws, long ws_floats, int* rows_out, hipStream_t st) {
    Geo g{nseq, L, inner, outer_stride, inner_stride, tok_stride};
    Par p{qw, qb, kw, kb, emb, hscale};
    Grd gr{dqw, dqb, dkw, dkb, demb, dhscale};
    const int nb = L <= 16 ? 1 : 2, ks = d / 32;
#define GO(NB, KS) if (nb == NB && ks == KS) return go_bwd<NB, KS>((const bf16*)qkv, (const bf16*)dout, (bf16*)dqkv, g, heads, p, gr, out_scale, accumulate, ws, ws_floats, rows_out, st)
    GO(1, 1); GO(1, 2); GO(1, 3); GO(1, 4); GO(2, 1); GO(2, 2); GO(2, 3); GO(2, 4);
#undef GO
    return bf_fail_msg("bf_attn_bwd_mfma: unsupported shape", __FILE__, __LINE__);
}
```

bubbleformer_amd/csrc/model.hip:

```cpp
#include "model_common.h"

bool bf_attn_raw_modes(int dtype, int d);
int bf_gemm_tokred_deferred(int dtype, int Nout, int Kin, int64_t M, const void* dy, int64_t ldy, const void* x, int64_t ldx, float* out,
                            int accumulate, float* colsum, float* ws, int64_t ws_floats, hipStream_t stream);
const float* bf_gemm_tokred_pending_out();
int bf_gemm_inbwd_frames_scaled(int dtype, int M, int N, int K, const void* A, int64_t lda, const void* B, int64_t ldb, const void* x,
                                const void* add, void* out, int S, const float* mean, const float* rstd, const float* w, float* ws,
                                const float* fscale, int fdiv, void* out_s, const float* f_s, int fdiv_s, hipStream_t stream);

using namespace bfm;

namespace {

bool g_side_defer = false;

BfPerDevice<TrunkLinks> g_links;

int launch_reduce_jobs(ReduceJobs& J, hipStream_t st);
__global__ void __launch_bounds__(256) stage_prep_multi_kernel(PrepBatch b);

}

bool bfm::side_defer() { return g_side_defer; }
TrunkLinks& bfm::links() { return g_links.get(); }
// ... 433 lines not shown

}

extern "C" int64_t bf_temporal_saved_bytes(const bf_dims* s) { D d; if (get_dims(s, &d)) return -1; return (int64_t)TemporalSaved(d, nullptr).bytes; }
extern "C" int64_t bf_spatial_saved_bytes(const bf_dims* s) { D d; if (get_dims(s, &d)) return -1; return (int64_t)SpatialSaved(d, nullptr).bytes; }
static size_t dbr_bytes(const D& d) { return (((size_t)d.N * d.E * d.es) + 255) & ~(size_t)255; }
extern "C" int64_t bf_scratch_bytes(const bf_dims* s) { D d; if (get_dims(s, &d)) return -1; return 2 * (int64_t)Scratch(d, nullptr).bytes + 2 * (int64_t)dbr_bytes(d); }

extern "C" void bf_side_defer(int on) { g_side_defer = on != 0; }
extern "C" int bf_side_join(bf_stream_t s) { return side_join_pending(g_links.get(), (hipStream_t)s); }

extern "C" void bf_stage_prepared(int on) { g_links.get().hints.prepared = on != 0; }
extern "C" int bf_stage_chain_tail(const bf_spatial_params* prev_p, const void* prev_saved, int has_drop_mlp) {
    g_links.get().hints.tail = NextTail{prev_p && prev_saved, prev_p, prev_saved, has_drop_mlp != 0};
    return 0;
}
extern "C" int bf_stage_next_scale(const float* factors, int fdiv) { g_links.get().hints.scale = NextScale{factors, fdiv > 0 ? fdiv : 1}; return 0; }
static NextHead next_head(const D& d, int kind, const void* params, void* saved) {
    auto of = [&](auto* np, const auto& sv) { return NextHead{true, np->norm1_w, np->norm1_b, sv.mean1, sv.rstd1, sv.sc1, sv.sh1, sv.xn, saved}; };
    return kind == 0 ? of((const bf_temporal_params*)params, TemporalSaved(d, saved)) : of((const bf_spatial_params*)params, SpatialSaved(d, saved));
}
extern "C" int bf_stage_chain_next(const bf_dims* dims, int next_kind, const void* next_params, void* next_saved) {
    NextHead& h = g_links.get().hints.head;
    h = NextHead{};
    if (!dims || !next_params || !next_saved) return 0;
    BF_REQUIRE(next_kind == 0 || next_kind == 1, "bf_stage_chain_next: kind must be 0 (temporal) or 1 (spatial)");
    D d; TRY(get_dims(dims, &d));
    h = next_head(d, next_kind, next_params, next_saved);
    return 0;
}
extern "C" int bf_stage_chain_head(const bf_dims* dims, const bf_temporal_params* next_p, void* next_saved) {
    return bf_stage_chain_next(dims, 0, next_p, next_saved);
}

static int temporal_fwd(TrunkLinks& L, const StageHints& H, const bf_dims* dims, const bf_temporal_params* p, const void* x, void* out, void* saved,
                        void* scratch, const float* drop, bf_stream_t s) {
    D d; TRY(get_dims(dims, &d));
    BF_REQUIRE(p && x && out && saved && scratch, "bf_temporal_fwd: null pointer");
    hipStream_t st = (hipStream_t)s;
    const bool head_done = L.take_head_done(saved, st);
    TRY(side_join_pending(L, st));
    TemporalSaved sv(d, saved);
    Scratch sc(d, scratch);
    const void* wv[4];
    TRY(wviews(d, stage_prep(d, 0, p, sv.prep_dst(), nullptr), H.prepared, wv, st));
    const void *win_c = wv[0], *wout_c = wv[1];
    if (!head_done)
        TRY(bf_in_stats_apply(d.dtype, x, (int)d.F, (int)d.S, d.E, p->norm1_w, p->norm1_b, nullptr, 1, nullptr, sv.mean1, sv.rstd1, sv.sc1, sv.sh1, sc.in_ws,
                              nullptr, sv.xn, st));
    TRY(qkv_gemm(d, sv.xn, win_c, p->input_head_b, sv.qkv, st));
    TRY(bf_attn_fwd(d.dtype, sv.qkv, sv.o, (long)d.B * d.S, d.T, d.S, (long)d.T * d.S, 1, d.S, d.heads, d.d, p->qnorm_w, p->qnorm_b,
                    p->knorm_w, p->knorm_b, p->rel_pos_emb, d.attn_scale ? p->attn_scale_factor : nullptr, 1.f, 0, st));
    TRY(bf_in_stats_apply(d.dtype, sv.o, (int)d.F, (int)d.S, d.E, p->norm2_w, p->norm2_b, nullptr, 1, nullptr, sv.mean2, sv.rstd2, sv.sc2, sv.sh2, sc.in_ws,
                          nullptr, sv.on, st));
    if (H.head.armed) {
        const NextHead& h = H.head;
        const bf_frame_norm n2{h.w, h.b, nullptr, 1, h.mean, h.rstd, h.sc, h.sh, nullptr, h.xn};
        const int rc = bf_gemm_fwd_frames(d.dtype, (int)d.N, d.E, d.E, sv.on, d.E, sv.wout_t, d.E, nullptr, sv.alpha, sv.beta, drop, d.T, x, out, (int)d.S,
                                          nullptr, &n2, s);
        if (rc < 0) return rc;
        if (rc == 0) { L.head_done = {h.saved, st}; return 0; }
    }
    TRY(outproj_gemm(d, sv.on, wout_c, sv.alpha, sv.beta, x, out, drop, (long)d.T * d.S, st));
    return 0;
}

static int temporal_bwd(TrunkLinks& L, const StageHints& H, const bf_dims* dims, const bf_temporal_params* p, const bf_temporal_params* g, const void* x,
                        const void* dout, void* dx, void* saved, void* scratch, const float* drop, bf_stream_t s) {
    D d; TRY(get_dims(dims, &d));
    BF_REQUIRE(p && g && x && dout && dx && saved && scratch, "bf_temporal_bwd: null pointer");
    hipStream_t st = (hipStream_t)s;
    TemporalSaved sv(d, saved);
    Scratch sc(d, bwd_scratch(L, d, scratch));
    const void* win_c = d.dtype == BF_DTYPE_F32 ? (const void*)p->input_head_w : sv.win_c;
    Fork fk(L, st, true, L.scratch_parity);
    if (fk.deferred) TRY(side_join_pending(L, st, fk.set));
    void* don = sc.t1;
    void* dO = sc.t1b;
    void* dqkv = sc.t3;
    const void* dbr = dout;
    if (drop) {
        const TrunkLinks::DbrReady& r = L.dbr_ready;
        if (r.dx == dout && r.f == drop && r.buf && r.st == st) dbr = r.buf;
        else {
            TRY(bf_frame_scale(d.dtype, dout, drop, d.T, sc.t4, d.N, (int)d.S, d.E, st));
            dbr = sc.t4;
        }
    }
    L.dbr_ready = TrunkLinks::DbrReady{};
    const InFuse fu2{sv.o, nullptr, dO, sv.mean2, sv.rstd2, p->norm2_w, p->norm2_b, sc.in_ws2};
    TRY(outproj_bwd(d, sc, dbr, sv.on, sv.wout_s, p->output_head_w, p->output_head_b, p->norm2_b, p->gamma, nullptr, nullptr,
                    sv.alpha, sv.mc, g->output_head_w, g->output_head_b, nullptr, g->gamma, nullptr, nullptr, don, st, fk, &fu2));
    ReduceJobs jobs;
    TRY(jobs.push(InReduceJob{sc.in_ws2, (int)d.F, d.E, p->norm2_w, p->norm2_b, nullptr, 1, g->norm2_w, g->norm2_b, nullptr, nullptr, nullptr, nullptr}));
    {
        int rows = 0;
        TRY(bf_attn_bwd_partials(d.dtype, sv.qkv, dO, dqkv, (long)d.B * d.S, d.T, d.S, (long)d.T * d.S, 1, d.S, d.heads, d.d, p->qnorm_w, p->qnorm_b,
                                 p->knorm_w, p->knorm_b, p->rel_pos_emb, d.attn_scale ? p->attn_scale_factor : nullptr, g->qnorm_w, g->qnorm_b,
                                 g->knorm_w, g->knorm_b, g->rel_pos_emb, d.attn_scale ? g->attn_scale_factor : nullptr, 1.f, 0, sc.attn_ws,
                                 Scratch::ATTN_WS_FLOATS, &rows, st));
        TRY(jobs.push(AttnReduceJob{sc.attn_ws, rows, d.d, d.heads, g->qnorm_w, g->qnorm_b, g->knorm_w, g->knorm_b, g->rel_pos_emb,
                                    d.attn_scale ? g->attn_scale_factor : nullptr}));
    }
    void* dxn = sc.t1;
    InFuse fu1{x, dout, dx, sv.mean1, sv.rstd1, p->norm1_w, p->norm1_b, sc.in_ws};
    TailNorm tn;
    bool tail_done = false;
    static const bool chain_on = bf_knob("BF_BWD_CHAIN", 1) != 0;
    if (H.tail.armed && chain_on && fk.deferred && d.dtype == BF_DTYPE_BF16 && d.S == 144 && d.F % 2 == 0) {
        const NextTail& h = H.tail;
        const int oset = L.scratch_parity ^ 1;
        TRY(side_join_pending(L, st, oset));
        Scratch so(d, (char*)scratch + (size_t)oset * Scratch(d, nullptr).bytes);
        SpatialSaved ps(d, const_cast<void*>(h.saved));
        tn = TailNorm{ps.z, so.t1, ps.mean3, ps.rstd3, h.p->mlp_norm_w, h.drop ? ps.gtab : h.p->gamma_mlp, h.drop ? 1 : (int)d.F, L.tail_ws_flip ? so.in_ws5 : so.in_ws4, &tail_done};
        L.tail_ws_flip = !L.tail_ws_flip;
        fu1.tail = &tn;
    }
    if (H.tail.armed) L.tail_done = TrunkLinks::TailDone{};
    TRY(linear_bwd(d, sc, dqkv, 3 * d.E, sv.xn, d.E, BF_PRO_NONE, nullptr, nullptr, win_c, g->input_head_w, g->input_head_b, dxn, nullptr, st, fk, &fu1, true));
    if (tail_done) L.tail_done = {H.tail.saved, dx, tn.ws, st};
    TRY(jobs.push(InReduceJob{sc.in_ws, (int)d.F, d.E, p->norm1_w, p->norm1_b, nullptr, 1, g->norm1_w, g->norm1_b, nullptr, nullptr, nullptr, nullptr}));
    TRY(launch_with_pending(L, jobs, st));
    return fk.join();
}
extern "C" int bf_temporal_fwd(const bf_dims* dims, const bf_temporal_params* p, const void* x, void* out, void* saved, void* scratch,
                               const float* drop, bf_stream_t s) {
    TrunkLinks& L = g_links.get();
    return temporal_fwd(L, L.take_hints(), dims, p, x, out, saved, scratch, drop, s);
}
extern "C" int bf_temporal_bwd(const bf_dims* dims, const bf_temporal_params* p, const bf_temporal_params* g, const void* x, const void* dout,
                               void* dx, void* saved, void* scratch, const float* drop, bf_stream_t s) {
    TrunkLinks& L = g_links.get();
    return temporal_bwd(L, L.take_hints(), dims, p, g, x, dout, dx, saved, scratch, drop, s);
}

static int prep_stages(TrunkLinks& L, const bf_dims* dims, int n, const int32_t* kinds, const void* const* params, void* const* saved,
                       const float* const* drop_mlp, bf_stream_t s) {
    D d; TRY(get_dims(dims, &d));
    BF_REQUIRE(n >= 1 && kinds && params && saved, "bf_prep_stages: bad arguments");
    if (d.dtype != BF_DTYPE_BF16) return 1;
    hipStream_t st = (hipStream_t)s;
    TRY(side_join_pending(L, st));
    for (int i0 = 0; i0 < n; i0 += PREP_BATCH) {
        PrepBatch b;
        memset(&b, 0, sizeof(b));
        const int m = std::min(PREP_BATCH, n - i0);
        for (int i = 0; i < m; ++i) {
            const int k = i0 + i;
            BF_REQUIRE(params[k] && saved[k] && (kinds[k] == 0 || kinds[k] == 1), "bf_prep_stages: bad stage entry");
            b.s[i] = kinds[k] == 0 ? stage_prep(d, 0, params[k], TemporalSaved(d, saved[k]).prep_dst(), nullptr)
                                   : stage_prep(d, 1, params[k], SpatialSaved(d, saved[k]).prep_dst(), drop_mlp ? drop_mlp[k] : nullptr);
        }
        TRY(launch_stage_prep(d, b, m, 7, st));
    }
    return 0;
}
extern "C" int bf_prep_stages(const bf_dims* dims, int n, const int32_t* kinds, const void* const* params, void* const* saved,
                              const float* const* drop_mlp, bf_stream_t s) {
    return prep_stages(g_links.get(), dims, n, kinds, params, saved, drop_mlp, s);
}

static int spatial_fwd(TrunkLinks& L, const StageHints& H, const bf_dims* dims, const bf_spatial_params* p, const void* x, void* out, void* saved,
                       void* scratch, const float* drop_att, const float* drop_mlp, bf_stream_t s) {
    D d; TRY(get_dims(dims, &d));
    BF_REQUIRE(p && x && out && saved && scratch, "bf_spatial_fwd: null pointer");
    hipStream_t st = (hipStream_t)s;
    const bool head_done = L.take_head_done(saved, st);
    TRY(side_join_pending(L, st));
    SpatialSaved sv(d, saved);
    Scratch sc(d, scratch);
    const void* wv[4];
    TRY(wviews(d, stage_prep(d, 1, p, sv.prep_dst(), drop_mlp), H.prepared, wv, st));
    const void *win_c = wv[0], *wout_c = wv[1], *w1_c = wv[2], *w2_c = wv[3];
    if (!head_done)
        TRY(bf_in_stats_apply(d.dtype, x, (int)d.F, (int)d.S, d.E, p->norm1_w, p->norm1_b, nullptr, 1, nullptr, sv.mean1, sv.rstd1, sv.sc1, sv.sh1, sc.in_ws,
                              nullptr, sv.xn, st));
    TRY(qkv_gemm(d, sv.xn, win_c, p->input_head_b, sv.qkv, st));
    {
        const int rc = bf_attn_axial_norm_fwd(d.dtype, sv.qkv, sv.o, sv.on, d.F, (int)d.h, (int)d.w, d.heads, d.d, p->qnorm_w, p->qnorm_b, p->knorm_w,
                                              p->knorm_b, p->rel_pos_emb, d.attn_scale ? p->attn_scale_factor_x : nullptr,
                                              d.attn_scale ? p->attn_scale_factor_y : nullptr, p->norm2_w, p->norm2_b, sv.mean2, sv.rstd2, sv.sc2,
                                              sv.sh2, st);
        if (rc < 0) return rc;
        if (rc == 1) {
            TRY(bf_attn_axial_fwd(d.dtype, sv.qkv, sv.o, d.F, (int)d.h, (int)d.w, d.heads, d.d, p->qnorm_w, p->qnorm_b, p->knorm_w, p->knorm_b,
                                  p->rel_pos_emb, d.attn_scale ? p->attn_scale_factor_x : nullptr, d.attn_scale ? p->attn_scale_factor_y : nullptr, st));
            TRY(bf_in_stats_apply(d.dtype, sv.o, (int)d.F, (int)d.S, d.E, p->norm2_w, p->norm2_b, nullptr, 1, nullptr, sv.mean2, sv.rstd2, sv.sc2, sv.sh2,
                                  sc.in_ws, nullptr, sv.on, st));
        }
    }
    TRY(outproj_gemm(d, sv.on, wout_c, sv.alpha, sv.beta, x, sv.x1, drop_att, d.S, st));
    {
        bf_operand A = op_plain(sv.x1, d.E, BF_LAY_KC);
        bf_operand Bo = op_plain(w1_c, d.E, BF_LAY_KC);
        bf_epilogue e = epi_store(sv.pre, 4L * d.E);
        e.bias = p->fc1_b;
        e.gelu_out = sv.hid;
        TRY(bf_gemm(d.dtype, (int)d.N, 4 * d.E, d.E, &A, &Bo, &e, 1, st));
    }
    const float* g3 = p->gamma_mlp;
    int g3div = (int)d.F;
    if (drop_mlp) {
        if (d.dtype == BF_DTYPE_F32) {
            hipLaunchKernelGGL(frame_table_kernel, dim3(bf_cdiv(d.F * d.E, 256)), dim3(256), 0, st, drop_mlp, 1, (const float*)p->gamma_mlp, sv.gtab, (int)d.F, d.E);
            BF_CHECK_LAUNCH();
        }
        g3 = sv.gtab; g3div = 1;
    }
    if (d.dtype == BF_DTYPE_BF16) {
        const bf_frame_norm n1{p->mlp_norm_w, p->mlp_norm_b, g3, g3div, sv.mean3, sv.rstd3, sv.sc3, sv.sh3, sv.x1, out};
        const NextHead& h = H.head;
        const bf_frame_norm n2{h.w, h.b, nullptr, 1, h.mean, h.rstd, h.sc, h.sh, nullptr, h.xn};
        const int rc = bf_gemm_fwd_frames(d.dtype, (int)d.N, d.E, 4 * d.E, sv.hid, 4L * d.E, sv.w2t_c, d.E, p->fc2_b, nullptr, nullptr, nullptr, 1, nullptr, sv.z,
                                          (int)d.S, &n1, h.armed ? &n2 : nullptr, s);
        if (rc < 0) return rc;
        if (rc == 0) {
            if (h.armed) L.head_done = {h.saved, st};
            return 0;
        }
    }
    {
        bf_operand A = op_plain(sv.hid, 4L * d.E, BF_LAY_KC);
        bf_operand Bo = op_plain(w2_c, 4L * d.E, BF_LAY_KC);
        bf_epilogue e = epi_store(sv.z, d.E);
        e.bias = p->fc2_b;
        TRY(bf_gemm(d.dtype, (int)d.N, d.E, 4 * d.E, &A, &Bo, &e, 1, st));
    }
    if (H.head.armed) {
        const NextHead& h = H.head;
        bool chained = false;
        TRY(bf_in_stats_apply_chain(d.dtype, sv.z, (int)d.F, (int)d.S, d.E, p->mlp_norm_w, p->mlp_norm_b, g3, g3div, nullptr, sv.mean3, sv.rstd3, sv.sc3, sv.sh3,
                                    sc.in_ws, sv.x1, out, h.w, h.b, h.mean, h.rstd, h.sc, h.sh, h.xn, &chained, st));
        if (chained) L.head_done = {h.saved, st};
        return 0;
    }
    TRY(bf_in_stats_apply(d.dtype, sv.z, (int)d.F, (int)d.S, d.E, p->mlp_norm_w, p->mlp_norm_b, g3, g3div, nullptr, sv.mean3, sv.rstd3,
                          sv.sc3, sv.sh3, sc.in_ws, sv.x1, out, st));
    return 0;
}

static int spatial_bwd(TrunkLinks& L, const StageHints& H, const bf_dims* dims, const bf_spatial_params* p, const bf_spatial_params* g, const void* x,
                       const void* dout, void* dx, void* saved, void* scratch, const float* drop_att, const float* drop_mlp, bf_stream_t s) {
    D d; TRY(get_dims(dims, &d));
    BF_REQUIRE(p && g && x && dout && dx && saved && scratch, "bf_spatial_bwd: null pointer");
    hipStream_t st = (hipStream_t)s;
    SpatialSaved sv(d, saved);
    Scratch sc(d, bwd_scratch(L, d, scratch));
    const bool f32 = d.dtype == BF_DTYPE_F32;
    const void* win_c = f32 ? (const void*)p->input_head_w : sv.win_c;
    const void* w1_c = f32 ? (const void*)p->fc1_w : sv.w1_c;
    const void* w2_c = f32 ? (const void*)p->fc2_w : sv.w2_c;
    TRY(flush_pending_reduce(L, st));
    Fork fk(L, st, true, L.scratch_parity);
    if (fk.deferred) TRY(side_join_pending(L, st, fk.set));
    void* dz = sc.t1;
    ReduceJobs jobs;
    const TrunkLinks::TailDone td = L.tail_done;
    L.tail_done = TrunkLinks::TailDone{};
    const bool tail_done = td.saved == saved && td.dx == dout && td.st == st;
    {
        const float* gsc = drop_mlp ? sv.gtab : p->gamma_mlp;
        const int gdiv = drop_mlp ? 1 : (int)d.F;
        if (!tail_done)
            TRY(bf_in_bwd_partials(d.dtype, dout, sv.z, nullptr, dz, (int)d.F, (int)d.S, d.E, sv.mean3, sv.rstd3, p->mlp_norm_w, p->mlp_norm_b, gsc, gdiv, 0, sc.in_ws3, st));
        TRY(jobs.push(InReduceJob{tail_done ? td.ws : sc.in_ws3, (int)d.F, d.E, p->mlp_norm_w, p->mlp_norm_b, gsc, gdiv, g->mlp_norm_w, g->mlp_norm_b,
                                  drop_mlp ? nullptr : g->gamma_mlp, nullptr, drop_mlp, drop_mlp ? g->gamma_mlp : nullptr}));
    }
    void* dpre = sc.t4;
    {
        bf_epilogue e; memset(&e, 0, sizeof(e));
        e.aux_mode = BF_AUX_DGELU; e.aux = sv.pre; e.ld_aux = 4L * d.E; e.out_mode = BF_OUT_STORE;
        static const bool use_t = bf_knob("BF_FC2_DGRAD_T", 1) != 0;
        TRY(linear_bwd(d, sc, dz, d.E, sv.hid, 4 * d.E, BF_PRO_NONE, nullptr, nullptr, w2_c, g->fc2_w, g->fc2_b, dpre, &e, st, fk, nullptr, false,
                       (!f32 && use_t) ? sv.w2t_c : nullptr));
    }
    void* dx1 = sc.t1b;
    bool dbr_done = false;
    {
        bf_epilogue e; memset(&e, 0, sizeof(e));
        e.aux_mode = BF_AUX_ADD; e.aux = dout; e.ld_aux = d.E; e.out_mode = BF_OUT_STORE;
        TRY(linear_bwd(d, sc, dpre, 4 * d.E, sv.x1, d.E, BF_PRO_NONE, nullptr, nullptr, w1_c, g->fc1_w, g->fc1_b, dx1, &e, st, fk, nullptr, false, nullptr,
                       drop_att ? sc.e5 : nullptr, drop_att, (int)d.S, &dbr_done));
    }
    void* don = sc.e6;
    const void* dbr = dx1;
    if (dbr_done) dbr = sc.e5;
    else if (drop_att) {
        TRY(bf_frame_scale(d.dtype, dx1, drop_att, 1, sc.e5, d.N, (int)d.S, d.E, st));
        dbr = sc.e5;
    }
    void* dO = sc.e7;
    const InFuse fu2{sv.o, nullptr, dO, sv.mean2, sv.rstd2, p->norm2_w, p->norm2_b, sc.in_ws2};
    TRY(outproj_bwd(d, sc, dbr, sv.on, sv.wout_s, p->output_head_w, p->output_head_b, p->norm2_b, p->gamma_att,
                    d.feat_scale ? p->low_freq_scalar : nullptr, d.feat_scale ? p->high_freq_scalar : nullptr, sv.alpha, sv.mc,
                    g->output_head_w, g->output_head_b, g->norm2_b, g->gamma_att, d.feat_scale ? g->low_freq_scalar : nullptr,
                    d.feat_scale ? g->high_freq_scalar : nullptr, don, st, fk, &fu2));
    TRY(jobs.push(InReduceJob{sc.in_ws2, (int)d.F, d.E, p->norm2_w, p->norm2_b, nullptr, 1, g->norm2_w, g->norm2_b, nullptr, nullptr, nullptr, nullptr}));
    void* dqkv = sc.t3;
    {
        int rows = 0;
        static const bool raw_on = bf_knob("BF_ATTN_RAW", 1) != 0;
        const bool rawm = raw_on && bf_attn_raw_modes(d.dtype, d.d);
        TRY(bf_attn_bwd_partials(d.dtype, sv.qkv, dO, dqkv, d.F * d.h, d.w, 1, d.w, 0, 1, d.heads, d.d, p->qnorm_w, p->qnorm_b, p->knorm_w, p->knorm_b,
                                 p->rel_pos_emb, d.attn_scale ? p->attn_scale_factor_x : nullptr, g->qnorm_w, g->qnorm_b, g->knorm_w, g->knorm_b,
                                 g->rel_pos_emb, d.attn_scale ? g->attn_scale_factor_x : nullptr, 0.5f, rawm ? 2 : 0, sc.attn_ws, Scratch::ATTN_WS_FLOATS, &rows, st));
        TRY(jobs.push(AttnReduceJob{sc.attn_ws, rows, d.d, d.heads, g->qnorm_w, g->qnorm_b, g->knorm_w, g->knorm_b, g->rel_pos_emb,
                                    d.attn_scale ? g->attn_scale_factor_x : nullptr}));
        TRY(bf_attn_bwd_partials(d.dtype, sv.qkv, dO, dqkv, d.F * d.w, d.h, d.w, d.S, 1, d.w, d.heads, d.d, p->qnorm_w, p->qnorm_b, p->knorm_w, p->knorm_b,
                                 p->rel_pos_emb, d.attn_scale ? p->attn_scale_factor_y : nullptr, g->qnorm_w, g->qnorm_b, g->knorm_w, g->knorm_b,
                                 g->rel_pos_emb, d.attn_scale ? g->attn_scale_factor_y : nullptr, 0.5f, rawm ? 5 : 1, sc.attn_ws2, Scratch::ATTN_WS_FLOATS, &rows, st));
        TRY(jobs.push(AttnReduceJob{sc.attn_ws2, rows, d.d, d.heads, g->qnorm_w, g->qnorm_b, g->knorm_w, g->knorm_b, g->rel_pos_emb,
                                    d.attn_scale ? g->attn_scale_factor_y : nullptr}));
    }
    void* dxn = sc.e6;
    InFuse fu1{x, dx1, dx, sv.mean1, sv.rstd1, p->norm1_w, p->norm1_b, sc.in_ws};
    bool scaled_done = false;
    const NextScale& ns = H.scale;
    L.dbr_ready = TrunkLinks::DbrReady{};
    static const bool scaled_on = bf_knob("BF_BWD_SCALED_COPY", 1) != 0;
    if (ns.f && scaled_on && fk.deferred && d.dtype == BF_DTYPE_BF16) {
        fu1.scaled_out = (char*)scratch + 2 * Scratch(d, nullptr).bytes + (L.dbr_flip ? dbr_bytes(d) : 0);
        fu1.scaled_f = ns.f; fu1.scaled_fdiv = ns.fdiv; fu1.scaled_done = &scaled_done;
    }
    TRY(linear_bwd(d, sc, dqkv, 3 * d.E, sv.xn, d.E, BF_PRO_NONE, nullptr, nullptr, win_c, g->input_head_w, g->input_head_b, dxn, nullptr, st, fk, &fu1, true));
    if (scaled_done) { L.dbr_ready = {dx, ns.f, fu1.scaled_out, st}; L.dbr_flip = !L.dbr_flip; }
    TRY(jobs.push(InReduceJob{sc.in_ws, (int)d.F, d.E, p->norm1_w, p->norm1_b, nullptr, 1, g->norm1_w, g->norm1_b, nullptr, nullptr, nullptr, nullptr}));
    static const bool merge_on = bf_knob("BF_REDUCE_MERGE", 1) != 0;
    if (fk.deferred && merge_on) { L.reduce.jobs = jobs; L.reduce.on = true; L.reduce.st = st; }
    else TRY(launch_reduce_jobs(jobs, st));
    return fk.join();
}
extern "C" int bf_spatial_fwd(const bf_dims* dims, const bf_spatial_params* p, const void* x, void* out, void* saved, void* scratch,
                              const float* drop_att, const float* drop_mlp, bf_stream_t s) {
    TrunkLinks& L = g_links.get();
    return spatial_fwd(L, L.take_hints(), dims, p, x, out, saved, scratch, drop_att, drop_mlp, s);
}
extern "C" int bf_spatial_bwd(const bf_dims* dims, const bf_spatial_params* p, const bf_spatial_params* g, const void* x, const void* dout,
                              void* dx, void* saved, void* scratch, const float* drop_att, const float* drop_mlp, bf_stream_t s) {
    TrunkLinks& L = g_links.get();
    return spatial_bwd(L, L.take_hints(), dims, p, g, x, dout, dx, saved, scratch, drop_att, drop_mlp, s);
}

extern "C" int bf_trunk_train_fwd(const bf_dims* dims, int n, const int32_t* kinds, const void* const* params, void* const* saved,
                                  const float* const* drop_a, const float* const* drop_b, const void* x, void* const* acts, void* scratch,
                                  bf_stream_t s) {
    D d; TRY(get_dims(dims, &d));
    BF_REQUIRE(n >= 1 && kinds && params && saved && x && acts && scratch, "bf_trunk_train_fwd: bad arguments");
    for (int i = 0; i < n; ++i)
        BF_REQUIRE(params[i] && saved[i] && acts[i] && (kinds[i] == 0 || kinds[i] == 1), "bf_trunk_train_fwd: bad stage entry");
    TrunkLinks& L = g_links.get();
    (void)L.take_hints();
    const bool b16 = d.dtype == BF_DTYPE_BF16;
    if (b16) {
        const int rc = prep_stages(L, dims, n, kinds, params, saved, drop_b, s);
        if (rc < 0) return rc;
    }
    for (int i = 0; i < n; ++i) {
        const void* in = i ? acts[i - 1] : x;
        StageHints H;
        H.prepared = b16;
        if (b16 && i + 1 < n && kinds[i + 1] != kinds[i]) H.head = next_head(d, kinds[i + 1], params[i + 1], saved[i + 1]);
        TRY(kinds[i] == 0
            ? temporal_fwd(L, H, dims, (const bf_temporal_params*)params[i], in, acts[i], saved[i], scratch, drop_a ? drop_a[i] : nullptr, s)
            : spatial_fwd(L, H, dims, (const bf_spatial_params*)params[i], in, acts[i], saved[i], scratch, drop_a ? drop_a[i] : nullptr,
                          drop_b ? drop_b[i] : nullptr, s));
    }
    return 0;
}

extern "C" int bf_trunk_train_bwd(const bf_dims* dims, int n, const int32_t* kinds, const void* const* params, const void* const* grads,
                                  void* const* saved, const float* const* drop_a, const float* const* drop_b, const void* x, void* const* acts,
                                  const void* dout, void* const* gbuf3, void* dx, void* scratch, bf_stage_done_fn stage_done, void* user,
                                  bf_stream_t s) {
    D d; TRY(get_dims(dims, &d));
    BF_REQUIRE(n >= 1 && kinds && params && grads && saved && x && acts && dout && gbuf3 && dx && scratch, "bf_trunk_train_bwd: bad arguments");
    BF_REQUIRE(gbuf3[0] && gbuf3[1] && gbuf3[2], "bf_trunk_train_bwd: three gradient buffers are needed");
    TrunkLinks& L = g_links.get();
    (void)L.take_hints();
    const void* cur = dout;
    int rot = 0;
    for (int i = n - 1; i >= 0; --i) {
        BF_REQUIRE(params[i] && grads[i] && saved[i] && (kinds[i] == 0 || kinds[i] == 1), "bf_trunk_train_bwd: bad stage entry");
        const void* in = i ? acts[i - 1] : x;
        void* gout = i ? gbuf3[rot] : dx;
        rot = (rot + 1) % 3;
        StageHints H;
        if (kinds[i] == 0) {
            if (i > 0 && kinds[i - 1] == 1) H.tail = NextTail{true, (const bf_spatial_params*)params[i - 1], saved[i - 1], drop_b && drop_b[i - 1]};
            TRY(temporal_bwd(L, H, dims, (const bf_temporal_params*)params[i], (const bf_temporal_params*)grads[i], in, cur, gout, saved[i], scratch,
                             drop_a ? drop_a[i] : nullptr, s));
        } else {
            if (i > 0 && kinds[i - 1] == 0 && drop_a && drop_a[i - 1]) H.scale = NextScale{drop_a[i - 1], d.T};
            TRY(spatial_bwd(L, H, dims, (const bf_spatial_params*)params[i], (const bf_spatial_params*)grads[i], in, cur, gout, saved[i], scratch,
                            drop_a ? drop_a[i] : nullptr, drop_b ? drop_b[i] : nullptr, s));
        }
        if (stage_done) stage_done(i, user);
        cur = gout;
    }
    return 0;
}
```

bubbleformer_amd/csrc/param_reduce.h:

```cpp
#pragma once
#include "bf_common.h"

struct InReduceJob {
    const float* ws; int frames, C; const float *w, *b, *g; int gdiv; float *dw, *db, *dg, *dgb; const float* mask; float* dmask_v;
    __host__ __device__ int rdiv() const { return (dg || dgb) ? (gdiv > 0 ? gdiv : 1) : (frames > 0 ? frames : 1); }
};
struct AttnReduceJob { const float* ws; int rows, D, heads; float *dqw, *dqb, *dkw, *dkb, *demb, *dhscale; };

constexpr int BF_RED_FL = 16;
template <int FL>
__device__ __forceinline__ void in_reduce_block(const InReduceJob& j, int bx, int by, float (*red)[FL][64]) {
    const int l = threadIdx.x & 63, fl = threadIdx.x >> 6;
    const int c = bx * 64 + l;
    const bool cv = c < j.C;
    const int rd = j.rdiv(), gdiv = j.gdiv > 0 ? j.gdiv : 1;
    const int f0 = by * rd, f1 = min(j.frames, f0 + rd);
    float t1 = 0.f, t2 = 0.f, g1 = 0.f, g2 = 0.f, sm = 0.f;
    const float wc = cv ? j.w[c] : 0.f, bc = cv ? j.b[c] : 0.f;
    if (cv) {
        int f = f0 + fl;
        for (; f + 7 * FL < f1; f += 8 * FL) {
            float2 p[8]; float gv[8];
#pragma unroll
            for (int u = 0; u < 8; ++u) {
                p[u] = *reinterpret_cast<const float2*>(j.ws + ((long)(f + FL * u) * j.C + c) * 2);
                gv[u] = j.g ? j.g[(long)((f + FL * u) / gdiv) * j.C + c] : 1.f;
            }
#pragma unroll
            for (int u = 0; u < 8; ++u) { t1 += p[u].x; t2 += p[u].y; g1 += gv[u] * p[u].x; g2 += gv[u] * p[u].y; }
        }
        for (; f < f1; f += FL) {
            const float a = j.ws[((long)f * j.C + c) * 2], b2 = j.ws[((long)f * j.C + c) * 2 + 1];
            const float gv = j.g ? j.g[(long)(f / gdiv) * j.C + c] : 1.f;
            t1 += a; t2 += b2; g1 += gv * a; g2 += gv * b2;
        }
    }
    const bool grouped = j.dg || j.dgb;
    if (cv && by == 0 && ((j.mask && j.dmask_v) || (grouped && (j.dw || j.db)))) {
        const bool redo = grouped && (j.dw || j.db), msk = j.mask && j.dmask_v;
        if (redo) g1 = g2 = 0.f;
        int f = fl;
        for (; f + 7 * FL < j.frames; f += 8 * FL) {
            float2 p[8]; float gv[8], mk[8];
#pragma unroll
            for (int u = 0; u < 8; ++u) {
                p[u] = *reinterpret_cast<const float2*>(j.ws + ((long)(f + FL * u) * j.C + c) * 2);
                gv[u] = j.g ? j.g[(long)((f + FL * u) / gdiv) * j.C + c] : 1.f;
                mk[u] = msk ? j.mask[f + FL * u] : 0.f;
            }
#pragma unroll
            for (int u = 0; u < 8; ++u) {
                if (msk) sm += mk[u] * (wc * p[u].y + bc * p[u].x);
                if (redo) { g1 += gv[u] * p[u].x; g2 += gv[u] * p[u].y; }
            }
        }
        for (; f < j.frames; f += FL) {
            const float a = j.ws[((long)f * j.C + c) * 2], b2 = j.ws[((long)f * j.C + c) * 2 + 1];
            if (msk) sm += j.mask[f] * (wc * b2 + bc * a);
            if (redo) { const float gv = j.g ? j.g[(long)(f / gdiv) * j.C + c] : 1.f; g1 += gv * a; g2 += gv * b2; }
        }
    }
    red[0][fl][l] = t1; red[1][fl][l] = t2; red[2][fl][l] = g1; red[3][fl][l] = g2; red[4][fl][l] = sm;
    __syncthreads();
    if (fl != 0 || !cv || f0 >= f1) return;
    float v[5];
#pragma unroll
    for (int q = 0; q < 5; ++q) {
        v[q] = red[q][0][l];
#pragma unroll
        for (int k = 1; k < FL; ++k) v[q] += red[q][k][l];
    }
    if (j.dw && (!grouped || by == 0)) atomicAdd(j.dw + c, v[3]);
    if (j.db && (!grouped || by == 0)) atomicAdd(j.db + c, v[2]);
    const long gi = (long)(f0 / gdiv) * j.C + c;
    if (j.dg) j.dg[gi] += wc * v[1] + bc * v[0];
    if (j.dgb) j.dgb[gi] += v[0];
    if (j.dmask_v && by == 0) atomicAdd(j.dmask_v + c, v[4]);
}

template <int FL>
__device__ __forceinline__ void attn_reduce_block(const AttnReduceJob& j, int bx, int by, int ny, float (*red)[FL][64]) {
    const int nvals = 4 * j.D + 32 * j.heads + j.heads;
    const int l = threadIdx.x & 63, rg = threadIdx.x >> 6;
    const int i = bx * 64 + l;
    const int per = (j.rows + ny - 1) / ny;
    const int r0 = by * per, r1 = min(j.rows, r0 + per);
    float acc = 0.f;
    if (i < nvals) {
        int r = r0 + rg;
        for (; r + 15 * FL < r1; r += 16 * FL) {
            float v[16];
#pragma unroll
            for (int u = 0; u < 16; ++u) v[u] = j.ws[(long)(r + FL * u) * nvals + i];
#pragma unroll
            for (int u = 0; u < 16; ++u) acc += v[u];
        }
        for (; r < r1; r += FL) acc += j.ws[(long)r * nvals + i];
    }
    red[0][rg][l] = acc;
    __syncthreads();
    if (rg != 0 || i >= nvals) return;
    acc = red[0][0][l];
#pragma unroll
    for (int k = 1; k < FL; ++k) acc += red[0][k][l];
    float* dst;
    if (i < 4 * j.D) { const int q = i / j.D, e = i % j.D; dst = (q == 0 ? j.dqw : q == 1 ? j.dqb : q == 2 ? j.dkw : j.dkb); if (dst) dst += e; }
    else if (i < 4 * j.D + 32 * j.heads) dst = j.demb ? j.demb + (i - 4 * j.D) : nullptr;
    else dst = j.dhscale ? j.dhscale + (i - 4 * j.D - 32 * j.heads) : nullptr;
    if (dst && acc != 0.f) atomicAdd(dst, acc);
}
```

include/bubbleformer_hip.h:

```cpp
#ifndef BUBBLEFORMER_HIP_H
#define BUBBLEFORMER_HIP_H

#include <stdint.h>

#ifdef __cplusplus
extern "C" {
#endif

typedef void* bf_stream_t;

enum { BF_DTYPE_F32 = 0, BF_DTYPE_BF16 = 1 };

enum { BF_LAY_KC = 0,
       BF_LAY_XC = 1   };
enum { BF_PRO_NONE = 0, BF_PRO_AFFINE = 1, BF_PRO_AFFINE_GELU = 2, BF_PRO_GELU = 3 };
enum { BF_AUX_NONE = 0, BF_AUX_ADD = 1 , BF_AUX_DGELU = 2  };
enum { BF_OUT_STORE = 0 , BF_OUT_ATOMIC_F32 = 2 ,
       BF_OUT_STORE_F32 = 1  };

typedef struct bf_operand {
    const void* p;
    int64_t ld;
    int32_t layout;
    int32_t seglen;
    int64_t segstride;
    int32_t gw, gh, gc;
    int32_t pro;
    const float* sc;
    const float* sh;
    int32_t rows_per_frame;
    int32_t nch;
} bf_operand;

typedef struct bf_epilogue {
    const float* bias;
    const float* colscale;
    const float* colshift;
    int32_t aux_mode;
    const void* aux;
    int64_t ld_aux;
    int32_t out_mode;
    void* c;
    int64_t ldc;
    int32_t seglen;
    int64_t segstride;
    int32_t gw, gh, gc;
    void* gelu_out;
    float* colsum;
    const float* rowscale;
    int32_t rows_per_group;
} bf_epilogue;

int bf_gemm(int dtype, int M, int N, int K, const bf_operand* A, const bf_operand* B, const bf_epilogue* E,
            int splitk, bf_stream_t stream);

int bf_gemm_inbwd_frames(int dtype, int M, int N, int K, const void* A, int64_t lda, const void* B, int64_t ldb, const void* x,
                         const void* add, void* out, int S, const float* mean, const float* rstd, const float* w, float* ws,
                         const float* fscale , int fdiv,
                         bf_stream_t stream);
int bf_gemm_inbwd_frames_chain(int dtype, int M, int N, int K, const void* A, int64_t lda, const void* B, int64_t ldb, const void* x,
                               const void* add, void* out, int S, const float* mean, const float* rstd, const float* w, float* ws,
                               const float* fscale, int fdiv, const void* cz, void* cdz, const float* cmean, const float* crstd,
                               const float* cw, const float* cg, int cgdiv, float* cws, bf_stream_t stream);

typedef struct bf_frame_norm {
    const float *w, *b;
    const float* g; int32_t gdiv;
    float *mean, *rstd, *sc, *sh;
    const void* resid;
    void* out;
} bf_frame_norm;
int bf_gemm_fwd_frames(int dtype, int M, int N, int K, const void* A, int64_t lda, const void* Bt, int64_t ldb, const float* bias,
                       const float* colscale, const float* colshift, const float* fscale, int fdiv, const void* add, void* out, int S,
                       const bf_frame_norm* n1, const bf_frame_norm* n2, bf_stream_t stream);

int bf_gemm_tokred(int dtype, int Nout, int Kin, int64_t M, const void* dy, int64_t ldy, const void* x, int64_t ldx, float* out,
                   int accumulate, float* colsum, float* ws, int64_t ws_floats, bf_stream_t stream);
int64_t bf_gemm_tokred_ws_floats(int Nout, int Kin, int64_t M);

int bf_frame_linear(int dtype, int frames, int S, int K, int N, const void* A, int64_t lda, const void* W, int64_t ldw,
                    const float* norm_w, const float* norm_b, const float* bias, const float* colscale, const float* colshift,
                    const void* resid, int64_t ldr, int gelu, const float* en_w, const float* en_b, const float* en_g,
                    void* out, int64_t ldo,
                    const float* next_w, const float* next_b, void* out_n, int64_t ldn,
                    bf_stream_t stream);


int bf_in_stats(int dtype, const void* x, int frames, int S, int C, const float* w, const float* b, const float* g, int gdiv,
                const float* gb, float* mean, float* rstd, float* sc, float* sh,
                float* ws ,
                bf_stream_t stream);
int64_t bf_in_ws_floats(int dtype, int frames, int S, int C);
int bf_affine_apply(int dtype, const void* z, const void* resid, const float* sc, const float* sh, void* out, int64_t nrows,
                    int S, int C, bf_stream_t stream);
int bf_in_bwd(int dtype, const void* dy, const void* x, const void* add, void* dx, int frames, int S, int C, const float* mean,
              const float* rstd, const float* w, const float* b, const float* g, int gdiv, int gelu, float* dw, float* db,
              float* dg, float* dgb, float* ws ,
              bf_stream_t stream);
int bf_colsum(int dtype, const void* x, int64_t nrows, int C, const float* scale, float* out, bf_stream_t stream);

int bf_attn_fwd(int dtype, const void* qkv, void* out, int64_t nseq, int L, int64_t inner, int64_t outer_stride,
                int64_t inner_stride, int64_t tok_stride, int heads, int d, const float* qw, const float* qb, const float* kw,
                const float* kb, const float* emb, const float* hscale, float out_scale, int accumulate, bf_stream_t stream);
int bf_attn_axial_fwd(int dtype, const void* qkv, void* out, int64_t frames, int h, int w, int heads, int d, const float* qw,
                      const float* qb, const float* kw, const float* kb, const float* emb, const float* hscale_x,
                      const float* hscale_y, bf_stream_t stream);
int bf_attn_axial_norm_fwd(int dtype, const void* qkv, void* out, void* out_n, int64_t frames, int h, int w, int heads, int d,
                           const float* qw, const float* qb, const float* kw, const float* kb, const float* emb, const float* hscale_x,
                           const float* hscale_y, const float* norm_w, const float* norm_b, float* mean, float* rstd, float* sc,
                           float* sh, bf_stream_t stream);
int bf_attn_bwd(int dtype, const void* qkv, const void* dout, void* dqkv, int64_t nseq, int L, int64_t inner,
                int64_t outer_stride, int64_t inner_stride, int64_t tok_stride, int heads, int d, const float* qw,
                const float* qb, const float* kw, const float* kb, const float* emb, const float* hscale, float* dqw,
                float* dqb, float* dkw, float* dkb, float* demb, float* dhscale, float out_scale, int accumulate,
                float* ws, int64_t ws_floats,
                bf_stream_t stream);

void bf_side_defer(int on);
int bf_side_join(bf_stream_t stream);
void bf_debug_force_generic_attn(int on);
void bf_debug_tokred_fold(int on);

int bf_im2col_nchw(int dtype, const float* x, void* out, int frames, int C, int H, int W, int Kp, bf_stream_t stream);
int bf_col2im_nchw(int dtype, const void* g, float* dx, int frames, int C, int H, int W, int Kp, bf_stream_t stream);
#define BF_LOSS_LIMBS 5
int bf_pm2nchw(const float* pm, float* pred, const float* y, float* lossbuf, int frames, int Co, int h, int w, int Np,
               bf_stream_t stream);
int bf_debed_last(int dtype, const void* act, const float* sc, const float* sh, const void* wc, float* pred, const float* y,
                  float* lossbuf, int frames, int Ci, int Co, int h, int w, int Np, bf_stream_t stream);
int bf_debed_last_bwd(int dtype, const float* dpred, const float* pred, const float* y, const float* coef, const float* gscale,
                      const void* wc, void* dpm, void* dact, int frames, int Ci, int Co, int h, int w, int Np, bf_stream_t stream);
int bf_debed_last_bwd_norm(int dtype, const float* dpred, const float* pred, const float* y, const float* coef, const float* gscale,
                           const void* wc, void* dpm, const void* ymap, const float* mean, const float* rstd, const float* in_w,
                           const float* in_b, void* dx, float* d_in_w, float* d_in_b, int frames, int Ci, int Co, int h, int w, int Np,
                           float* ws, int64_t ws_floats, bf_stream_t stream);
int bf_embed_first(int dtype, const float* x, const void* wc, void* patches, void* y0, int frames, int C0, int cin, int h2, int w2,
                   int Kp, float* stat_part, bf_stream_t stream);
int bf_in_stats_merge_slices(int dtype, int frames, int S, int C, int rows, const float* w, const float* b, const float* g, int gdiv,
                             const float* gb, float* mean, float* rstd, float* sc, float* sh, float* ws, bf_stream_t stream);
int bf_gather_gemm(int dtype, const void* map, const void* w, int w_kn, const float* sc, const float* sh, void* out, int frames, int gh,
                   int gw, int C0, int N, bf_stream_t stream);
int bf_scatter_gemm(int dtype, const void* a, const void* w, int w_kn, const float* sc, const float* sh, void* map, float* stat_part, int frames,
                    int gh, int gw, int K, int C0, bf_stream_t stream);
int64_t bf_gather_wgrad_ws_floats(int frames, int gh, int gw);
int bf_gather_wgrad(int dtype, const void* fine, const void* coarse, const float* fsc, const float* fsh, const float* csc, const float* csh,
                    float* out, int transposed, int frames, int gh, int gw, int C0, int Kc, float* ws, int64_t ws_floats, bf_stream_t stream);
int bf_gather_gemm_rebuilt(int dtype, const void* patches, const void* w0c, const void* w, int w_kn, const float* sc, const float* sh, void* out,
                           int frames, int gh, int gw, int C0, int N, bf_stream_t stream);
int bf_gather_wgrad_rebuilt(int dtype, const void* patches, const void* w0c, const void* coarse, const float* fsc, const float* fsh, float* out,
                            int transposed, int frames, int gh, int gw, int C0, int Kc, float* ws, int64_t ws_floats, bf_stream_t stream);
int64_t bf_embed_tail_ws_floats(int frames, int gh1, int gw1, int C0, int Kp);
int bf_embed_tail_bwd(int dtype, const void* dy1, const void* w1c, const void* y0, const void* patches, const void* w0c, const float* sc,
                      const float* sh, const float* mean, const float* rstd, const float* in_w, float* dwprep, float* d_in_w, float* d_in_b,
                      int frames, int gh1, int gw1, int C1, int C0, int Kp, float* ws, int64_t ws_floats, bf_stream_t stream);
int bf_lploss_finalize(const float* lossbuf, int frames, int Co, float* loss, float* coef, bf_stream_t stream);
int bf_nchw2pm(int dtype, const float* dpred, const float* pred, const float* y, const float* coef, const float* gscale,
               void* dpm, int frames, int Co, int h, int w, int Np, bf_stream_t stream);
int bf_wprep(int dtype, int mode, const float* src, void* dst, int R, int K, int Kp, bf_stream_t stream);
int bf_wgrad_unprep(int mode, const float* gsrc, float* gdst, int R, int K, int Kp, int transposed, bf_stream_t stream);
int bf_film_net_fwd(const float* cond, const float* lnw, const float* lnb, const float* W, const float* bias, float* gb,
                    float* chat, float* crstd, int B, int P, int E2, bf_stream_t stream);
int bf_film_net_bwd(const float* dgb, const float* chat, const float* lnw, const float* lnb, const float* W, float* dW,
                    float* dbias, float* dlnw, float* dlnb, int B, int P, int E2, bf_stream_t stream);
int bf_clip_gather(const float* src, int64_t field_stride, const int32_t* field, const int64_t* first, int t0, const float* diff,
                   const float* div, float* out, int B, int T, int C, int H, int W, int Ho, int Wo, bf_stream_t stream);
int bf_clip_gather_batch(const float* src, int64_t field_stride, const int64_t* idx, int64_t nsamples, const int64_t* first_tab, const int32_t* in_field,
                         const float* in_diff, const float* in_div, int Cin, int Tin, float* in_out, const int32_t* out_field,
                         const float* out_diff, const float* out_div, int Cout, int Tout, float* out_out, const float* fluid_tab,
                         const int64_t* file_tab, int P, float* fluid_out, int B, int H, int W, int Ho, int Wo, bf_stream_t stream);
int bf_clip_gather_unroll(const float* src, int64_t field_stride, int64_t nframes, const int64_t* idx, int64_t nsamples, const int64_t* first_tab,
                          const int32_t* in_field, const float* in_diff, const float* in_div, int Cin, int Tin, float* in_out,
                          const int32_t* out_field, const float* out_diff, const float* out_div, int Cout, int Tout, int unroll, float* out_out,
                          const float* fluid_tab, const int64_t* file_tab, int P, float* fluid_out, int B, int H, int W, int Ho, int Wo,
                          bf_stream_t stream);
typedef struct bf_clip_gather_job {
    const float* src; const int64_t *idx, *first_tab;
    const int32_t* in_field; const float *in_diff, *in_div; float* in_out;
    const int32_t* out_field; const float *out_diff, *out_div; float* out_out;
    const float* fluid_tab; const int64_t* file_tab; float* fluid_out;
    int64_t field_stride, nframes, nsamples;
    int32_t Cin, Tin, Cout, Tout, unroll, P, B, H, W, Ho, Wo, reserved;
} bf_clip_gather_job;
typedef struct bf_clip_augment {
    const int32_t *in_odd, *out_odd;
    int64_t seed, flip_thr;
    int32_t draw, Hc, Wc, crop_y, eval_view, reserved;
} bf_clip_augment;
int bf_clip_gather_augment(const bf_clip_gather_job* job, const bf_clip_augment* augment, bf_stream_t stream);
typedef struct bf_clip_gather_q16_job {
    const uint16_t* codes; const int32_t* frame_seg; const float *seg_lo, *seg_step;
    const int64_t *idx, *first_tab;
    const int32_t* in_field; const float *in_diff, *in_div; float* in_out;
    const int32_t* out_field; const float *out_diff, *out_div; float* out_out;
    const float* fluid_tab; const int64_t* file_tab; float* fluid_out;
    int64_t field_stride, nframes, nsamples;
    int32_t nfiles, Cin, Tin, Cout, Tout, unroll, P, B, H, W, Ho, Wo;
} bf_clip_gather_q16_job;
int bf_clip_encode_q16(const float* src, uint16_t* dst, int64_t n, float lo, float inv, bf_stream_t stream);
int bf_clip_decode_q16(const uint16_t* codes, int64_t field_stride, const int32_t* frame_seg, const float* seg_lo, const float* seg_step, float* dst,
                       int64_t nframes, int nfields, int nfiles, int H, int W, bf_stream_t stream);
int bf_clip_gather_q16(const bf_clip_gather_q16_job* job, const bf_clip_augment* augment, bf_stream_t stream);
int bf_clip_noise(const float* src, float* dst, const float* sigma, const int64_t* sample_ids, uint64_t seed, uint32_t draw, uint32_t pass,
                  int B, int T, int C, int H, int W, bf_stream_t stream);
int64_t bf_field_stats_ws_doubles(int nseg);
int bf_field_stats(const float* src, const int64_t* seg_begin, const int64_t* seg_len, int nseg, double* out, double* ws, bf_stream_t stream);
int bf_eikonal_sum(const float* phi, int64_t frames, int H, int W, float dx, double* out, bf_stream_t stream);
int bf_eikonal_l1_frames(const float* phi, int64_t frames, int H, int W, float dx, float* out, bf_stream_t stream);
int bf_heatflux_rows(const float* dfun, const float* temp, int64_t frames, int64_t frame_stride, int W, float x_min, float dx,
                     float heater_temp, float lc, float* flux, bf_stream_t stream);
typedef struct bf_rollout_step {
    const float *pred, *frames;
    int64_t field_stride, total_frames;
    const int64_t* first; int32_t* step; const int32_t* field;
    const float *diff, *div;
    int32_t nfields, B, T, C, H, W, Ho, Wo, steps, reserved;
} bf_rollout_step;
typedef struct bf_census_rows { int32_t *count, *cells, *attached, *area; } bf_census_rows;
typedef struct bf_link_rows { int32_t *successor, *n_successors, *predecessor, *n_predecessors, *departure_area, *events; } bf_link_rows;
typedef struct bf_match_rows { int32_t *match_pred, *match_target, *overlap; float* displacement; int32_t *counts, *mask; } bf_match_rows;
typedef struct bf_error_rows {
    float *rmse, *max_error, *boundary_rmse, *interface_rmse;
    int32_t* interface_cells;
    float *spectral_error, *spectrum_error, *spectrum_pred, *spectrum_target;
} bf_error_rows;
int64_t bf_rollout_score_ws_doubles(int B, int T, int C, int Ho, int Wo);
int bf_rollout_score(const bf_rollout_step* s, int sdf_channel, float dx, float* rel_l2, float* criterion, float* eik_pred, float* eik_tgt,
                     float* next_in, float* archive, double* ws, int64_t ws_doubles, bf_stream_t stream);
int bf_rollout_heatflux(const bf_rollout_step* s, int dfun_channel, int temp_channel, const float* heater_temp, float x_min, float dx, float lc,
                        float conductivity, float* flux_pred, float* flux_tgt, bf_stream_t stream);
int64_t bf_kde_kl_ws_doubles(int R, int64_t n, int64_t m, int points);
int bf_kde_kl(const double* p, const double* q, int R, int64_t n, int64_t m, int points, double eps, double* kl, double* x, double* pdf_p,
              double* pdf_q, double* ws, int64_t ws_doubles, bf_stream_t stream);
int64_t bf_bubble_census_lds_cells(void);
int64_t bf_bubble_census_ws_bytes(int64_t frames, int H, int W, int max_bubbles);
int bf_bubble_census(const float* phi, int64_t frames, int H, int W, int connectivity, int max_bubbles, int32_t* count, int32_t* vapour_cells,
                     int32_t* attached, int32_t* area, float* centroid, unsigned char* on_heater, int32_t* labels, void* ws, int64_t ws_bytes,
                     bf_stream_t stream);
int bf_rollout_bubbles(const bf_rollout_step* s, int sdf_channel, int connectivity, int max_bubbles, const bf_census_rows* pred,
                       const bf_census_rows* tgt, int32_t* labels, void* ws, int64_t ws_bytes, bf_stream_t stream);
int64_t bf_redistance_lds_cells(void);
int64_t bf_redistance_ws_bytes(int64_t frames, int H, int W);
int bf_redistance(const float* phi, int64_t frames, int H, int W, float dx, float band, int max_rounds, float* out, int32_t* rounds, float* change_rms,
                  void* ws, int64_t ws_bytes, bf_stream_t stream);
int bf_rollout_redistance(const bf_rollout_step* s, int sdf_channel, float dx, float band, int max_rounds, int every, float* pred, int32_t* rounds,
                          float* change_rms, void* ws, int64_t ws_bytes, bf_stream_t stream);
int64_t bf_bubble_links_lds_entries(void);
int64_t bf_bubble_links_ws_bytes(int64_t pairs, int max_bubbles);
int bf_bubble_links(const int32_t* labels, const bf_census_rows* census, int64_t sequences, int T, int H, int W, int max_bubbles,
                    const bf_link_rows* links, void* ws, int64_t ws_bytes, bf_stream_t stream);
int bf_bubble_track_ids(const int32_t* count, const int32_t* successor, const int32_t* predecessor, int64_t sequences, int T, int max_bubbles,
                        int32_t* track_id, int32_t* n_tracks, bf_stream_t stream);
int bf_rollout_bubble_links(const bf_rollout_step* s, int max_bubbles, const int32_t* labels, const bf_census_rows* census_pred,
                            const bf_census_rows* census_tgt, const bf_link_rows* links_pred, const bf_link_rows* links_tgt, void* ws,
                            int64_t ws_bytes, bf_stream_t stream);
int64_t bf_bubble_match_ws_bytes(int64_t pairs, int max_bubbles);
int bf_bubble_match(const int32_t* labels_pred, const int32_t* labels_tgt, const bf_census_rows* census_pred, const bf_census_rows* census_tgt,
                    int64_t frames, int H, int W, int max_bubbles, float min_iou, const bf_match_rows* rows, void* ws, int64_t ws_bytes,
                    bf_stream_t stream);
int bf_rollout_bubble_match(const bf_rollout_step* s, int max_bubbles, float min_iou, const int32_t* labels, const bf_census_rows* census_pred,
                            const bf_census_rows* census_tgt, const bf_match_rows* rows, void* ws, int64_t ws_bytes, bf_stream_t stream);
int64_t bf_field_errors_ws_bytes(int64_t frames, int H, int W);
int bf_field_errors(const float* pred, const float* target, const float* sdf, int64_t frames, int H, int W, int interface_radius, int lo, int hi,
                    int want_spectra, const bf_error_rows* rows, void* ws, int64_t ws_bytes, bf_stream_t stream);
int bf_rollout_errors(const bf_rollout_step* s, int sdf_channel, int interface_radius, int lo, int hi, int want_spectra, const bf_error_rows* rows,
                      void* ws, int64_t ws_bytes, bf_stream_t stream);
typedef struct bf_ensemble_rows { float *mean_rmse, *spread, *crps; int32_t* rank_hist; float* mean; } bf_ensemble_rows;
int64_t bf_ensemble_scores_ws_bytes(int frames, int members, int H, int W);
int bf_ensemble_scores(const float* members_ptr, int64_t member_stride, const float* target, int frames, int members, int H, int W, int fair,
                       const bf_ensemble_rows* rows, void* ws, int64_t ws_bytes, bf_stream_t stream);
int bf_rollout_ensemble(const bf_rollout_step* s, int members, int fair, const bf_ensemble_rows* rows, void* ws, int64_t ws_bytes, bf_stream_t stream);
int64_t bf_lp_rows_ws_doubles(int64_t rows, int64_t n);
int bf_lp_rows_fwd(const float* pred, const float* y, int64_t rows, int64_t n, double p, float* ratio, double* sums, double* ws, int64_t ws_doubles,
                   bf_stream_t stream);
int bf_lp_rows_bwd(const float* pred, const float* y, const float* g, const double* sums, int64_t rows, int64_t n, double p, float* dpred,
                   bf_stream_t stream);
int bf_eikonal_bwd(const float* phi, int64_t frames, int H, int W, float dx, const float* g, float* dphi, bf_stream_t stream);
int64_t bf_wlp_ws_doubles(int64_t frames, int C, int H, int W);
int bf_wlp_fwd(const float* pred, const float* y, int64_t frames, int C, int H, int W, int s, double diff_s, double div_s, double band, double gain,
               const double* field_weights, double eikonal, double dx, float* loss, float* terms, double* sums, double* ws, int64_t ws_doubles,
               bf_stream_t stream);
int bf_wlp_bwd(const float* pred, const float* y, const float* g, const double* sums, int64_t frames, int C, int H, int W, int s, double diff_s,
               double div_s, double band, double gain, const double* field_weights, double eikonal, double dx, float* dpred, bf_stream_t stream);
int64_t bf_slp_ws_bytes(int64_t frames, int C, int H, int W);
int bf_slp_fwd(const float* pred, const float* y, int64_t frames, int C, int H, int W, const double* shell_weights, const double* shell_weights_host,
               int K, const double* field_weights, float* loss, float* terms, double* sums, void* spec, void* ws, int64_t ws_bytes, bf_stream_t stream);
int bf_slp_bwd(const void* spec, const float* g, const double* sums, int64_t frames, int C, int H, int W, const double* field_weights, float* dpred,
               bf_stream_t stream);
int64_t bf_grad_norm_ws_doubles(int64_t n);
int bf_grad_norm(const float* g, int64_t n, float gscale, float max_norm, float* out, double* ws, int64_t ws_doubles, bf_stream_t stream);
#define BF_OPT_CHUNK 64
#define BF_OPT_MAX_GROUPS 64
typedef struct bf_opt_step {
    float* p; const float* g; float *m, *v;
    const float* coef_dev; float* avg;
    const uint8_t* chunk_group; const float *group_lr_scale, *group_weight_decay; const uint8_t* group_frozen;
    const int32_t* live_dev;
    int64_t n;
    int32_t step, n_groups;
    float lr, beta1, beta2, eps, wd, gscale, clip_value, avg_weight;
} bf_opt_step;
int bf_adamw(const bf_opt_step* s, bf_stream_t stream);
int bf_adam(const bf_opt_step* s, bf_stream_t stream);
int bf_lion(const bf_opt_step* s, bf_stream_t stream);
int bf_step_guard(const float* norm, int32_t step, int32_t* guard, bf_stream_t stream);
int64_t bf_nonfinite_scan_ws_len(int64_t n);
int bf_nonfinite_scan(const float* x, int64_t n, int64_t* out, int64_t* ws, int64_t ws_len, bf_stream_t stream);
int bf_weight_average(float* avg, const float* p, int64_t n, float w, bf_stream_t stream);
int bf_swap_buffers(float* a, float* b, int64_t n, bf_stream_t stream);
int64_t bf_group_sumsq_ws_doubles(int64_t n);
int bf_group_sumsq(const float* x, int64_t n, const uint8_t* chunk_group, int n_groups, double* sums, double* ws, int64_t ws_doubles,
                   bf_stream_t stream);
int bf_group_clip_coef(const double* sums, const uint8_t* frozen, int n_groups, float gscale, float max_norm, float* out,
                       float* group_norm, bf_stream_t stream);


typedef struct bf_dims {
    int32_t dtype;
    int32_t B, T, h, w;
    int32_t E, heads;
    int32_t attn_scale, feat_scale;
    int32_t patch;
    int32_t cin, cout;
    int32_t nfluid;
} bf_dims;

typedef struct bf_temporal_params {
    float *gamma, *attn_scale_factor, *norm1_w, *norm1_b, *norm2_w, *norm2_b, *input_head_w, *input_head_b,
          *output_head_w, *output_head_b, *qnorm_w, *qnorm_b, *knorm_w, *knorm_b, *rel_pos_emb;
} bf_temporal_params;
typedef struct bf_spatial_params {
    float *gamma_att, *gamma_mlp, *attn_scale_factor_x, *attn_scale_factor_y, *low_freq_scalar, *high_freq_scalar,
          *norm1_w, *norm1_b, *norm2_w, *norm2_b, *input_head_w, *input_head_b, *output_head_w, *output_head_b,
          *qnorm_w, *qnorm_b, *knorm_w, *knorm_b, *rel_pos_emb, *fc1_w, *fc1_b, *fc2_w, *fc2_b, *mlp_norm_w, *mlp_norm_b;
} bf_spatial_params;
#define BF_MAX_STAGES 5
typedef struct bf_embed_params {
    float* conv_w[BF_MAX_STAGES];
    float* in_w[BF_MAX_STAGES];
    float* in_b[BF_MAX_STAGES];
    float *film_ln_w, *film_ln_b, *film_w, *film_b;
} bf_embed_params;
typedef struct bf_debed_params {
    float* conv_w[BF_MAX_STAGES];
    float* in_w[BF_MAX_STAGES];
    float* in_b[BF_MAX_STAGES];
} bf_debed_params;

int64_t bf_temporal_saved_bytes(const bf_dims* d);
int64_t bf_spatial_saved_bytes(const bf_dims* d);
int64_t bf_embed_saved_bytes(const bf_dims* d);
int64_t bf_debed_saved_bytes(const bf_dims* d);
int64_t bf_scratch_bytes(const bf_dims* d);

int bf_prep_stages(const bf_dims* dims, int n, const int32_t* kinds, const void* const* params, void* const* saved,
                   const float* const* drop_mlp, bf_stream_t stream);
void bf_stage_prepared(int on);
int64_t bf_trunk_eval_weights_bytes(const bf_dims* dims, int n, const int32_t* kinds);
int bf_trunk_eval_prepare(const bf_dims* dims, int n, const int32_t* kinds, const void* const* params, void* weights, bf_stream_t stream);
int bf_trunk_eval_fwd(const bf_dims* dims, int n, const int32_t* kinds, const void* const* params, const void* weights, const void* x,
                      void* out, void* scratch, bf_stream_t stream);
typedef void (*bf_stage_done_fn)(int stage, void* user);
int bf_trunk_train_fwd(const bf_dims* dims, int n, const int32_t* kinds, const void* const* params, void* const* saved,
                       const float* const* drop_a, const float* const* drop_b, const void* x, void* const* acts, void* scratch, bf_stream_t stream);
int bf_trunk_train_bwd(const bf_dims* dims, int n, const int32_t* kinds, const void* const* params, const void* const* grads, void* const* saved,
                       const float* const* drop_a, const float* const* drop_b, const void* x, void* const* acts, const void* dout,
                       void* const* gbuf3, void* dx, void* scratch, bf_stage_done_fn stage_done, void* user, bf_stream_t stream);
int bf_stage_chain_head(const bf_dims* dims, const bf_temporal_params* next_p, void* next_saved);
int bf_stage_chain_next(const bf_dims* dims, int next_kind, const void* next_params, void* next_saved);
int bf_stage_chain_tail(const bf_spatial_params* prev_p, const void* prev_saved, int has_drop_mlp);
int bf_stage_next_scale(const float* factors, int fdiv);
int bf_temporal_fwd(const bf_dims* d, const bf_temporal_params* p, const void* x, void* out, void* saved, void* scratch,
                    const float* drop, bf_stream_t s);
int bf_temporal_bwd(const bf_dims* d, const bf_temporal_params* p, const bf_temporal_params* g, const void* x, const void* dout,
                    void* dx, void* saved, void* scratch, const float* drop, bf_stream_t s);
int bf_spatial_fwd(const bf_dims* d, const bf_spatial_params* p, const void* x, void* out, void* saved, void* scratch,
                   const float* drop_att, const float* drop_mlp, bf_stream_t s);
int bf_spatial_bwd(const bf_dims* d, const bf_spatial_params* p, const bf_spatial_params* g, const void* x, const void* dout,
                   void* dx, void* saved, void* scratch, const float* drop_att, const float* drop_mlp, bf_stream_t s);
int bf_embed_fwd(const bf_dims* d, const bf_embed_params* p, const float* x, const float* fluid, void* out, void* saved, void* scratch, bf_stream_t s);
int bf_embed_bwd(const bf_dims* d, const bf_embed_params* p, const bf_embed_params* g, const void* dout, float* dx_in, void* saved,
                 void* scratch, bf_stream_t s);
int bf_debed_fwd(const bf_dims* d, const bf_debed_params* p, const void* x, float* pred, const float* target, float* loss,
                 void* saved, void* scratch, bf_stream_t s);
int bf_debed_bwd(const bf_dims* d, const bf_debed_params* p, const bf_debed_params* g, const void* x, const float* dpred,
                 const float* pred, const float* target, const float* loss_scale, void* dx, void* saved, void* scratch,
                 bf_stream_t s);

enum { BF_CONV_PRO_NONE = 0, BF_CONV_PRO_AFFINE_GELU = 1 , BF_CONV_PRO_GELU = 2  };
typedef struct bf_conv_src {
    const void* p;
    int32_t C, nchw, f32;
} bf_conv_src;
typedef struct bf_conv_geo {
    int32_t F, Hi, Wi, Ho, Wo, kh, kw, stride, pad;
} bf_conv_geo;
int bf_conv_fwd(int dtype, const bf_conv_geo* geo, const bf_conv_src* s0, const bf_conv_src* s1, int pro, const float* sc, const float* sh,
                const void* w, int N, const float* bias, const bf_conv_src* resid, const bf_conv_src* out, int transposed, bf_stream_t stream);
int64_t bf_conv_wgrad_ws_floats(int R, int K, int64_t M);
int bf_conv_wgrad(int dtype, const bf_conv_geo* geo, const bf_conv_src* rows, const bf_conv_src* s0, const bf_conv_src* s1, int pro,
                  const float* sc, const float* sh, float* dw, int accumulate, float* ws, int64_t ws_floats, bf_stream_t stream);
int bf_conv_colsum(int dtype, const bf_conv_src* src, int F, int H, int W, float* out, int accumulate, float* ws, int64_t ws_floats,
                   bf_stream_t stream);
int64_t bf_gn_ws_floats(int F, int C, int G);
int bf_gn_fwd(int dtype, const bf_conv_src* s0, const bf_conv_src* s1, int F, int H, int W, int G, const float* gamma, const float* beta,
              float eps, float* mean, float* rstd, float* sc, float* sh, float* ws, bf_stream_t stream);
int bf_gn_bwd(int dtype, const float* dA, const bf_conv_src* s0, const bf_conv_src* s1, int F, int H, int W, int G, const float* gamma,
              const float* mean, const float* rstd, const float* sc, const float* sh, const bf_conv_src* add, const bf_conv_src* dx0,
              const bf_conv_src* dx1, float* dgamma, float* dbeta, int accumulate, float* ws, bf_stream_t stream);
int bf_unet_lploss_fwd(const float* pred, const float* target, int B, int T, int C, int64_t HW, float* loss, float* coef, float* ws,
                       bf_stream_t stream);
int bf_unet_lploss_bwd(const float* pred, const float* target, const float* coef, const float* dloss, int planes, int64_t HW, float* dpred,
                       bf_stream_t stream);

int64_t bf_bn_ws_floats(int64_t M, int C);
int bf_bn_fwd(int dtype, const void* x, int B, int64_t HW, int C, const float* gamma, const float* beta, float eps, float momentum,
              float* running_mean, float* running_var, int64_t* num_batches_tracked, float* mean, float* rstd, float* sc, float* sh, float* ws,
              bf_stream_t stream);
int bf_bn_eval(int B, int C, const float* gamma, const float* beta, float eps, const float* running_mean, const float* running_var, float* sc,
               float* sh, bf_stream_t stream);
// ... 39 lines not shown
```

Before: 827.2 samples/s.

## Fuse axial x- and y-attention backward into a single MFMA kernel

Adds a fused axial attention backward kernel that handles both the width-axis and height-axis attention problems of a frame in one launch. Each wave keeps per-wave LDS tables for the parameter gradients and writes one shared workspace row, reduced with strided jobs. Previously this took two separate bwd launches, each with its own workspace and reduction. The goal is fewer launches and workspace passes plus better data locality between the two axes. The cost is more shared memory per block, a new code path enabled by default, and different occupancy.

Result: no change. 821.4 samples/s (-0.7%).

```diff
diff --git a/bubbleformer_amd/_lib.py b/bubbleformer_amd/_lib.py
--- a/bubbleformer_amd/_lib.py
+++ b/bubbleformer_amd/_lib.py
@@ -144,6 +144,7 @@
     "bf_prof_enable": (None, [C.c_int]),
     "bf_debug_force_generic_attn": (None, [C.c_int]),
     "bf_debug_tokred_fold": (None, [C.c_int]),
+    "bf_debug_attn_axial_bwd": (None, [C.c_int]),
     "bf_side_defer": (None, [C.c_int]),
     "bf_prep_stages": (C.c_int, [C.POINTER(Dims), C.c_int, C.POINTER(C.c_int32), C.POINTER(vp), C.POINTER(vp), C.POINTER(vp), vp]),
     "bf_stage_prepared": (None, [C.c_int]),
@@ -183,6 +184,8 @@
                               C.c_int, vp]),
     "bf_attn_bwd": (C.c_int, [C.c_int, vp, vp, vp, i64, C.c_int, i64, i64, i64, i64, C.c_int, C.c_int, fp, fp, fp, fp, fp, fp,
                               fp, fp, fp, fp, fp, fp, f32, C.c_int, fp, i64, vp]),
+    "bf_attn_axial_bwd_partials": (C.c_int, [C.c_int, vp, vp, vp, i64, C.c_int, C.c_int, C.c_int, C.c_int, fp, fp, fp, fp, fp, fp, fp,
+                                             fp, fp, fp, fp, fp, fp, fp, fp, i64, C.POINTER(C.c_int), vp]),
     "bf_im2col_nchw": (C.c_int, [C.c_int, fp, vp, C.c_int, C.c_int, C.c_int, C.c_int, C.c_int, vp]),
     "bf_col2im_nchw": (C.c_int, [C.c_int, vp, fp, C.c_int, C.c_int, C.c_int, C.c_int, C.c_int, vp]),
     "bf_pm2nchw": (C.c_int, [fp, fp, fp, fp, C.c_int, C.c_int, C.c_int, C.c_int, C.c_int, vp]),
diff --git a/bubbleformer_amd/csrc/attn.hip b/bubbleformer_amd/csrc/attn.hip
--- a/bubbleformer_amd/csrc/attn.hip
+++ b/bubbleformer_amd/csrc/attn.hip
@@ -355,6 +355,10 @@
 int bf_attn_axial_fwd_mfma(const void* qkv, void* out, int frames, int h, int w, int heads, int d, const float* qw, const float* qb, const float* kw,
                            const float* kb, const float* emb, const float* hscale_x, const float* hscale_y, const float* nw, const float* nb,
                            void* out_n, float* mean, float* rstd, float* sc, float* sh, hipStream_t st);
+int bf_attn_axial_bwd_mfma(const void* qkv, const void* dout, void* dqkv, int frames, int h, int w, int heads, int d, const float* qw, const float* qb,
+                           const float* kw, const float* kb, const float* emb, const float* hscale_x, const float* hscale_y, float* dqw, float* dqb,
+                           float* dkw, float* dkb, float* demb, float* dhscale_x, float* dhscale_y, float* ws, long ws_floats, int* rows_out,
+                           hipStream_t st);
 static bool use_mfma(int dtype, int d) { return !g_force_generic && dtype == BF_DTYPE_BF16 && d % 32 == 0 && d <= 128; }
 bool bf_attn_raw_modes(int dtype, int d) { return use_mfma(dtype, d); }
 
@@ -481,3 +485,18 @@
     return attn_bwd_impl(dtype, qkv, dout, dqkv, nseq, L, inner, outer_stride, inner_stride, tok_stride, heads, d, qw, qb, kw, kb, emb, hscale, dqw,
                          dqb, dkw, dkb, demb, dhscale, out_scale, accumulate, ws, ws_floats, rows, (bf_stream_t)stream);
 }
+
+static bool g_axial_bwd_off = bf_knob("BF_ATTN_AXIAL_BWD_FUSED", 1) == 0;
+extern "C" void bf_debug_attn_axial_bwd(int on) { g_axial_bwd_off = on == 0; }
+extern "C" int bf_attn_axial_bwd_partials(int dtype, const void* qkv, const void* dout, void* dqkv, int64_t frames, int h, int w, int heads, int d,
+                                          const float* qw, const float* qb, const float* kw, const float* kb, const float* emb, const float* hscale_x,
+                                          const float* hscale_y, float* dqw, float* dqb, float* dkw, float* dkb, float* demb, float* dhscale_x,
+                                          float* dhscale_y, float* ws, int64_t ws_floats, int* rows, bf_stream_t stream) {
+    if (rows) *rows = 0;
+    BF_REQUIRE(qkv && dout && dqkv && qw && qb && kw && kb && frames > 0, "bf_attn_axial_bwd_partials: bad arguments");
+    if (g_axial_bwd_off || !use_mfma(dtype, d) || frames >= (1L << 24)) return 1;
+    const double prob = (double)frames * heads * h * w;
+    BfProfScope prof((hipStream_t)stream, "attn_bwd_axial", 10.0 * prob * (h + w) * d, prob * d * 2.0 * 17.0);
+    return bf_attn_axial_bwd_mfma(qkv, dout, dqkv, (int)frames, h, w, heads, d, qw, qb, kw, kb, emb, hscale_x, hscale_y, dqw, dqb, dkw, dkb, demb,
+                                  dhscale_x, dhscale_y, ws, (long)ws_floats, rows, (hipStream_t)stream);
+}
diff --git a/bubbleformer_amd/csrc/attn_mfma.hip b/bubbleformer_amd/csrc/attn_mfma.hip
--- a/bubbleformer_amd/csrc/attn_mfma.hip
+++ b/bubbleformer_amd/csrc/attn_mfma.hip
@@ -503,74 +503,38 @@
     }
 }
 
+template <int NB, int KS> struct BwdTiles {
+    static constexpr int D = 32 * KS, LD = D + 16, R = 16 * NB, LDP = 32 + 8, PER_WAVE = 3 * R * LD + 2 * R * LDP;
+    static_assert(3 * R * LD * 2 >= 4 * D * 4, "the parameter-gradient flush must fit in the operand tiles");
+    bf16 *qn_t, *kn_t, *do_t, *at_t, *ds_t;
+    __device__ __forceinline__ explicit BwdTiles(bf16* base) : qn_t(base), kn_t(base + R * LD), do_t(base + 2 * R * LD), at_t(base + 3 * R * LD), ds_t(base + 3 * R * LD + R * LDP) {}
+    __device__ __forceinline__ void zero_pad(int lane) const {
+        if (NB == 1)
+            for (int c = lane; c < 16 * 16; c += 64) { at_t[(c >> 4) * LDP + 16 + (c & 15)] = (bf16)0.f; ds_t[(c >> 4) * LDP + 16 + (c & 15)] = (bf16)0.f; }
+    }
+};
+struct BwdLds { const float *par, *emb, *hsc; float *demb, *dhs; bool has_hs, has_demb, has_dhs; };
+
 template <int NB, int KS, int ACC>
-__global__ void __launch_bounds__(256, ((NB == 1 && KS <= 2) ? 2 : 1)) attn_bwd_mfma(const bf16* __restrict__ qkv, const bf16* __restrict__ dout, bf16* __restrict__ dqkv, Geo g,
-                                                     int heads, Par p, Grd gr, float out_scale, int accumulate_rt, float* __restrict__ ws) {
-    constexpr int D = 32 * KS, LD = D + 16, NT16 = D / 16, R = 16 * NB, LDP = 32 + 8;
+__device__ __forceinline__ void attn_bwd_problem(const bf16* __restrict__ qkv, const bf16* __restrict__ dout, bf16* __restrict__ dqkv, const Geo& g, const Geo& g_next,
+                                                 int heads, const Prob& at, const Prob& at_next, bool more, RawRows<NB, KS>& cur, RawRows<NB, KS>& nxt,
+                                                 const BwdTiles<NB, KS>& T, const BwdLds& S, float out_scale, int accumulate_rt, bool one_head,
+                                                 const float (&mk)[NB][NB][4], const float (&mneg)[NB][NB][4], const int (&eidx)[NB][NB][4],
+                                                 float (&a_ln)[2 * KS], float (&a_emb)[NB][NB][4], float& a_dhs, int lane) {
+    constexpr int D = 32 * KS, LD = D + 16, NT16 = D / 16, LDP = 32 + 8;
     constexpr bool PREFETCH = NB * KS <= 4;
-    extern __shared__ __attribute__((aligned(16))) bf16 smem_bwd[];
-    __shared__ float s_demb[32 * 16];
-    __shared__ float s_dhs[16];
-    __shared__ __attribute__((aligned(16))) float s_par[4 * 32 * KS];
-    __shared__ float s_emb[32 * 16];
-    __shared__ float s_hsc[16];
-    const int lane = threadIdx.x & 63, wave = __builtin_amdgcn_readfirstlane(threadIdx.x >> 6), wpb = blockDim.x >> 6;
-    constexpr int PER_WAVE = 3 * R * LD + 2 * R * LDP;
-    static_assert(3 * R * LD * 2 >= 4 * D * 4, "the parameter-gradient flush must fit in the operand tiles");
-    bf16* qn_t = smem_bwd + wave * PER_WAVE;
-    bf16* kn_t = qn_t + R * LD;
-    bf16* do_t = kn_t + R * LD;
-    bf16* at_t = do_t + R * LD;
-    bf16* ds_t = at_t + R * LDP;
-    float* relay = reinterpret_cast<float*>(qn_t);
-    for (int i = threadIdx.x; i < 32 * 16; i += blockDim.x) {
-        s_demb[i] = 0.f;
-        const int t = i >> 4, h = i & 15;
-        s_emb[i] = (p.emb && h < heads) ? p.emb[t * heads + h] : 0.f;
-    }
-    if (threadIdx.x < 16) { s_dhs[threadIdx.x] = 0.f; s_hsc[threadIdx.x] = (p.hscale && (int)threadIdx.x < heads) ? p.hscale[threadIdx.x] : 1.f; }
-    for (int i = threadIdx.x; i < 4 * D; i += blockDim.x) {
-        const int q = i / D, e = i % D;
-        s_par[i] = (q == 0 ? p.qw : q == 1 ? p.qb : q == 2 ? p.kw : p.kb)[e];
-    }
-    __syncthreads();
+    bf16 *const qn_t = T.qn_t, *const kn_t = T.kn_t, *const do_t = T.do_t, *const at_t = T.at_t, *const ds_t = T.ds_t;
+    const float *const s_par = S.par, *const s_emb = S.emb, *const s_hsc = S.hsc;
+    float *const s_demb = S.demb, *const s_dhs = S.dhs;
     const int E = heads * D, L = g.L;
     const float scale = rsqrtf((float)D);
-    const long nprob = g.nseq * heads;
     const int gq = lane >> 4, i16 = lane & 15;
     const int mode = ACC >= 0 ? ACC : accumulate_rt;
     const bool raw_out = mode & 2, raw_in = mode & 4, accumulate = mode & 1;
-
-    constexpr int NACC = 2 * KS;
-    float a_ln[NACC];
-#pragma unroll
-    for (int k = 0; k < NACC; ++k) a_ln[k] = 0.f;
-    const long pstep = (long)gridDim.x * wpb;
-    const bool one_head = pstep % heads == 0;
-    float a_emb[NB][NB][4], a_dhs = 0.f;
-#pragma unroll
-    for (int jb = 0; jb < NB; ++jb)
-#pragma unroll
-        for (int ib = 0; ib < NB; ++ib)
-#pragma unroll
-            for (int r = 0; r < 4; ++r) a_emb[jb][ib][r] = 0.f;
-    long pr = (long)blockIdx.x * wpb + wave;
-    RawRows<NB, KS> cur, nxt;
-    Prob at = locate(g, heads, pr < nprob ? pr : 0), at_next = at;
-    if (pr < nprob) load_raw<NB, KS>(cur, qkv, dout, g, heads, at, lane);
-    if (PREFETCH) drain_vm();
-    float mk[NB][NB][4], mneg[NB][NB][4];
-    int eidx[NB][NB][4];
-    lane_masks<NB>(L, lane, mk, mneg, eidx);
-    if (NB == 1) {
-        for (int c = lane; c < 16 * 16; c += 64) { at_t[(c >> 4) * LDP + 16 + (c & 15)] = (bf16)0.f; ds_t[(c >> 4) * LDP + 16 + (c & 15)] = (bf16)0.f; }
-    }
-    for (; pr < nprob; pr += pstep) {
+    {
         const int head = at.head;
         const long tok0 = at.tok0;
-        const bool more = pr + pstep < nprob;
-        if (more) at_next = locate(g, heads, pr + pstep);
-        if (PREFETCH && more) load_raw<NB, KS>(nxt, qkv, dout, g, heads, at_next, lane);
+        if (PREFETCH && more) load_raw<NB, KS>(nxt, qkv, dout, g_next, heads, at_next, lane);
         OldRows<NB, KS> old;
         if (accumulate) {
 #pragma unroll
@@ -615,7 +579,7 @@
             }
         }
         float P[NB][NB][4], A[NB][NB][4], dA[NB][NB][4];
-        scores_softmax_pre<NB, KS>(kf, qf, s_emb, eidx, mneg, mk, p.hscale ? s_hsc : nullptr, head, L, P, A);
+        scores_softmax_pre<NB, KS>(kf, qf, s_emb, eidx, mneg, mk, S.has_hs ? s_hsc : nullptr, head, L, P, A);
         const float hs = s_hsc[head];
         const float invL = 1.0f / (float)L;
         float dhs = 0.f;
@@ -629,7 +593,7 @@
 #pragma unroll
                 for (int r = 0; r < 4; ++r) {
                     float v = acc[r] * out_scale * mk[jb][ib][r];
-                    if (p.hscale) { dhs += (P[jb][ib][r] - invL) * v; v *= hs; }
+                    if (S.has_hs) { dhs += (P[jb][ib][r] - invL) * v; v *= hs; }
                     dA[jb][ib][r] = v;
                 }
             }
@@ -649,13 +613,13 @@
                     const float v = P[jb][ib][r] * (dA[jb][ib][r] - dot) * mk[jb][ib][r];
                     dA[jb][ib][r] = v;
                     if (one_head) a_emb[jb][ib][r] += v;
-                    else if (gr.demb && i < L && j < L) atomicAdd(&s_demb[eidx[jb][ib][r] + head], v);
+                    else if (S.has_demb && i < L && j < L) atomicAdd(&s_demb[eidx[jb][ib][r] + head], v);
                     at_t[j * LDP + i] = (bf16)A[jb][ib][r];
                     ds_t[j * LDP + i] = (bf16)v;
                 }
         }
         if (one_head) a_dhs += dhs;
-        else if (p.hscale && gr.dhscale) {
+        else if (S.has_dhs) {
             dhs = wave_sum(dhs);
             if (lane == 0) atomicAdd(&s_dhs[head], dhs);
         }
@@ -783,7 +747,68 @@
         }
         wsync();
         if (PREFETCH) cur = nxt;
-        else if (more) load_raw<NB, KS>(cur, qkv, dout, g, heads, at_next, lane);
+        else if (more) load_raw<NB, KS>(cur, qkv, dout, g_next, heads, at_next, lane);
+    }
+}
+
+template <int NB, int KS, int ACC>
+__global__ void __launch_bounds__(256, ((NB == 1 && KS <= 2) ? 2 : 1)) attn_bwd_mfma(const bf16* __restrict__ qkv, const bf16* __restrict__ dout, bf16* __restrict__ dqkv, Geo g,
+                                                     int heads, Par p, Grd gr, float out_scale, int accumulate_rt, float* __restrict__ ws) {
+    constexpr int D = 32 * KS;
+    constexpr bool PREFETCH = NB * KS <= 4;
+    extern __shared__ __attribute__((aligned(16))) bf16 smem_bwd[];
+    __shared__ float s_demb[32 * 16];
+    __shared__ float s_dhs[16];
+    __shared__ __attribute__((aligned(16))) float s_par[4 * 32 * KS];
+    __shared__ float s_emb[32 * 16];
+    __shared__ float s_hsc[16];
+    const int lane = threadIdx.x & 63, wave = __builtin_amdgcn_readfirstlane(threadIdx.x >> 6), wpb = blockDim.x >> 6;
+    constexpr int PER_WAVE = BwdTiles<NB, KS>::PER_WAVE;
+    const BwdTiles<NB, KS> tiles(smem_bwd + wave * PER_WAVE);
+    float* relay = reinterpret_cast<float*>(tiles.qn_t);
+    for (int i = threadIdx.x; i < 32 * 16; i += blockDim.x) {
+        s_demb[i] = 0.f;
+        const int t = i >> 4, h = i & 15;
+        s_emb[i] = (p.emb && h < heads) ? p.emb[t * heads + h] : 0.f;
+    }
+    if (threadIdx.x < 16) { s_dhs[threadIdx.x] = 0.f; s_hsc[threadIdx.x] = (p.hscale && (int)threadIdx.x < heads) ? p.hscale[threadIdx.x] : 1.f; }
+    for (int i = threadIdx.x; i < 4 * D; i += blockDim.x) {
+        const int q = i / D, e = i % D;
+        s_par[i] = (q == 0 ? p.qw : q == 1 ? p.qb : q == 2 ? p.kw : p.kb)[e];
+    }
+    __syncthreads();
+    const int L = g.L;
+    const long nprob = g.nseq * heads;
+    const int gq = lane >> 4, i16 = lane & 15;
+    const BwdLds lds{s_par, s_emb, s_hsc, s_demb, s_dhs, p.hscale != nullptr, gr.demb != nullptr, p.hscale && gr.dhscale};
+
+    constexpr int NACC = 2 * KS;
+    float a_ln[NACC];
+#pragma unroll
+    for (int k = 0; k < NACC; ++k) a_ln[k] = 0.f;
+    const long pstep = (long)gridDim.x * wpb;
+    const bool one_head = pstep % heads == 0;
+    float a_emb[NB][NB][4], a_dhs = 0.f;
+#pragma unroll
+    for (int jb = 0; jb < NB; ++jb)
+#pragma unroll
+        for (int ib = 0; ib < NB; ++ib)
+#pragma unroll
+            for (int r = 0; r < 4; ++r) a_emb[jb][ib][r] = 0.f;
+    long pr = (long)blockIdx.x * wpb + wave;
+    RawRows<NB, KS> cur, nxt;
+    Prob at = locate(g, heads, pr < nprob ? pr : 0), at_next = at;
+    if (pr < nprob) load_raw<NB, KS>(cur, qkv, dout, g, heads, at, lane);
+    if (PREFETCH) drain_vm();
+    float mk[NB][NB][4], mneg[NB][NB][4];
+    int eidx[NB][NB][4];
+    lane_masks<NB>(L, lane, mk, mneg, eidx);
+    tiles.zero_pad(lane);
+    for (; pr < nprob; pr += pstep) {
+        const bool more = pr + pstep < nprob;
+        if (more) at_next = locate(g, heads, pr + pstep);
+        attn_bwd_problem<NB, KS, ACC>(qkv, dout, dqkv, g, g, heads, at, at_next, more, cur, nxt, tiles, lds, out_scale, accumulate_rt, one_head, mk, mneg, eidx,
+                                      a_ln, a_emb, a_dhs, lane);
         at = at_next;
     }
     if (one_head && pr - pstep >= 0) {
@@ -820,6 +845,148 @@
         else { const int t = i - 4 * D - 32 * heads; val = s_dhs[t]; dst = gr.dhscale ? gr.dhscale + t : nullptr; }
         if (ws) ws[(long)blockIdx.x * nvals + i] = val;
         else if (dst && val != 0.f) atomicAdd(dst, val);
+    }
+}
+
+template <int KS, int WPB>
+__global__ void __launch_bounds__(64 * WPB) attn_bwd_axial_mfma(const bf16* __restrict__ qkv, const bf16* __restrict__ dout, bf16* __restrict__ dqkv, int frames, int h, int w,
+                                                                int heads, Par p, const float* __restrict__ hscale_y, float out_scale, int want_demb, int mixed, int one_head, int mode_w, int mode_h, float* __restrict__ ws) {
+    constexpr int ACCW = KS == 2 ? 2 : -1, ACCH = KS == 2 ? 5 : -1;
+    constexpr int NB = 1, D = 32 * KS, TG = 3, PER_WAVE = BwdTiles<NB, KS>::PER_WAVE, TAB = 32 * 16 + 32;
+    extern __shared__ __attribute__((aligned(16))) bf16 smem_bax[];
+    __shared__ __attribute__((aligned(16))) float s_par[4 * 32 * KS];
+    __shared__ float s_emb[32 * 16];
+    __shared__ float s_hsx[16], s_hsy[16];
+    const int lane = threadIdx.x & 63, wave = __builtin_amdgcn_readfirstlane(threadIdx.x >> 6);
+    const BwdTiles<NB, KS> tiles(smem_bax + wave * PER_WAVE);
+    float* tabs = reinterpret_cast<float*>(smem_bax + WPB * PER_WAVE);
+    float* tab = tabs + wave * TAB;
+    float* relay = reinterpret_cast<float*>(tiles.qn_t);
+    for (int i = lane; i < TAB; i += 64) tab[i] = 0.f;
+    for (int i = threadIdx.x; i < 32 * 16; i += blockDim.x) {
+        const int t = i >> 4, hd = i & 15;
+        s_emb[i] = (p.emb && hd < heads) ? p.emb[t * heads + hd] : 0.f;
+    }
+    if (threadIdx.x < 16) {
+        s_hsx[threadIdx.x] = (p.hscale && (int)threadIdx.x < heads) ? p.hscale[threadIdx.x] : 1.f;
+        s_hsy[threadIdx.x] = (hscale_y && (int)threadIdx.x < heads) ? hscale_y[threadIdx.x] : 1.f;
+    }
+    for (int i = threadIdx.x; i < 4 * D; i += blockDim.x) {
+        const int q = i / D, e = i % D;
+        s_par[i] = (q == 0 ? p.qw : q == 1 ? p.qb : q == 2 ? p.kw : p.kb)[e];
+    }
+    tiles.zero_pad(lane);
+    __syncthreads();
+    const int S = h * w, gq = lane >> 4, i16 = lane & 15;
+    const Geo gW{(long)frames * h, w, 1, w, 0, 1}, gH{(long)frames * w, h, w, S, 1, w};
+    const BwdLds ldsW{s_par, s_emb, s_hsx, tab, tab + 32 * 16, p.hscale != nullptr, want_demb != 0, p.hscale != nullptr};
+    const BwdLds ldsH{s_par, s_emb, s_hsy, tab, tab + 32 * 16 + 16, hscale_y != nullptr, want_demb != 0, hscale_y != nullptr};
+    float a_ln[2 * KS], a_emb[NB][NB][4], a_dh = 0.f;
+#pragma unroll
+    for (int k = 0; k < 2 * KS; ++k) a_ln[k] = 0.f;
+#pragma unroll
+    for (int r = 0; r < 4; ++r) a_emb[0][0][r] = 0.f;
+    float mk[NB][NB][4], mneg[NB][NB][4];
+    int eidx[NB][NB][4];
+    int curL = w;
+    lane_masks<NB>(curL, lane, mk, mneg, eidx);
+    int acc_head = -1;
+    auto flush_dh = [&](int hs_off) {
+        const float t = wave_sum(a_dh);
+        if (lane == 0 && acc_head >= 0) tab[32 * 16 + hs_off + acc_head] += t;
+        a_dh = 0.f;
+    };
+    auto flush = [&](int hs_off) {
+        if (acc_head < 0) return;
+        const int lmax = h > w ? h : w;
+#pragma unroll
+        for (int r = 0; r < 4; ++r) {
+            if (want_demb && i16 < lmax && 4 * gq + r < lmax) atomicAdd(&tab[eidx[0][0][r] + acc_head], a_emb[0][0][r]);
+            a_emb[0][0][r] = 0.f;
+        }
+        flush_dh(hs_off);
+    };
+    RawRows<NB, KS> cur, nxt;
+    const long ntile = (long)frames * heads;
+    for (long t0 = blockIdx.x; t0 < ntile; t0 += (long)TG * gridDim.x) {
+        const long left = (ntile - t0 + gridDim.x - 1) / gridDim.x;
+        const int G = left < TG ? (int)left : TG;
+        const int NW = G * h, NH = G * w, mr = NW / WPB;
+        int HS = (NW + WPB - 1) / WPB * WPB, b0 = -1, b1 = HS / WPB;
+        if (mixed && NW % WPB) {
+            const int c = min(HS - NW, NH);
+            if (((c - 1) / w + 1) * h - 1 < mr * WPB) { HS = NW; b0 = mr; b1 = mr + 1; }
+        }
+        const int nround = (HS + NH + WPB - 1) / WPB;
+        struct Slot { bool valid, isH; Prob at; };
+        auto slot = [&](int pos) {
+            const bool isH = pos >= HS;
+            const int q = isH ? pos - HS : pos, len = isH ? w : h;
+            Slot s{pos >= 0 && (isH ? q < NH : q < NW), isH, Prob{0, 0}};
+            if (s.valid) {
+                const unsigned k = (unsigned)q / (unsigned)len, idx = (unsigned)q - k * (unsigned)len;
+                const unsigned tile = (unsigned)(t0 + (long)k * gridDim.x), frame = tile / (unsigned)heads;
+                s.at = Prob{(long)frame * S + (isH ? (long)idx : (long)idx * w), (int)(tile - frame * (unsigned)heads)};
+            }
+            return s;
+        };
+        const int rb = b0 >= 0 ? b0 : b1;
+        bool have = false;
+        int r = 0;
+#pragma unroll 1
+        for (int ph = 0; ph < 2; ++ph) {
+            if (ph == 1) { drain_vm(); __syncthreads(); }
+            if (curL != w) { curL = w; lane_masks<NB>(curL, lane, mk, mneg, eidx); }
+            int ln = lane;
+            asm volatile("" : "+v"(ln));
+#pragma unroll 1
+            for (; (ph == 1 || r < rb) && r * WPB + wave < NW; ++r) {
+                const int pos = r * WPB + wave;
+                const Slot s = slot(pos), n = slot(pos + WPB);
+                if (s.at.head != acc_head) { flush(0); acc_head = s.at.head; }
+                if (!have) { load_raw<NB, KS>(cur, qkv, dout, gW, heads, s.at, ln); drain_vm(); }
+                attn_bwd_problem<NB, KS, ACCW>(qkv, dout, dqkv, gW, n.isH ? gH : gW, heads, s.at, n.at, n.valid, cur, nxt, tiles, ldsW, out_scale, mode_w, one_head != 0, mk, mneg, eidx,
+                                            a_ln, a_emb, a_dh, ln);
+                have = n.valid;
+            }
+        }
+        flush_dh(0);
+        if (curL != h) { curL = h; lane_masks<NB>(curL, lane, mk, mneg, eidx); }
+        int ln = lane;
+        asm volatile("" : "+v"(ln));
+#pragma unroll 1
+        for (r = rb; r < nround; ++r) {
+            if (b0 >= 0 && r == b1) { drain_vm(); __syncthreads(); }
+            const int pos = r * WPB + wave;
+            if (pos >= HS && pos < HS + NH) {
+                const Slot s = slot(pos), n = slot(pos + WPB);
+                if (s.at.head != acc_head) { flush(16); acc_head = s.at.head; }
+                if (!have) { load_raw<NB, KS>(cur, qkv, dout, gH, heads, s.at, ln); drain_vm(); }
+                attn_bwd_problem<NB, KS, ACCH>(qkv, dout, dqkv, gH, gH, heads, s.at, n.at, n.valid, cur, nxt, tiles, ldsH, out_scale, mode_h, one_head != 0, mk, mneg, eidx,
+                                            a_ln, a_emb, a_dh, ln);
+                have = n.valid;
+            }
+        }
+        flush_dh(16);
+    }
+    flush(16);
+#pragma unroll
+    for (int k = 0; k < 2 * KS; ++k) {
+        const int v = 16 * k + i16, q = v / (8 * KS), ks = (v >> 3) % KS, j = v & 7;
+        relay[q * D + 32 * ks + 8 * gq + j] = a_ln[k];
+    }
+    __syncthreads();
+    const int nvals = 4 * D + 34 * heads;
+    for (int i = threadIdx.x; i < nvals; i += blockDim.x) {
+        float val = 0.f;
+        if (i < 4 * D)
+            for (int wv = 0; wv < WPB; ++wv) val += reinterpret_cast<const float*>(smem_bax + wv * PER_WAVE)[i];
+        else {
+            const int t = i - 4 * D;
+            const int o = t < 32 * heads ? (t / heads) * 16 + (t % heads) : 32 * 16 + (t - 32 * heads < heads ? t - 32 * heads : 16 + t - 33 * heads);
+            for (int wv = 0; wv < WPB; ++wv) val += tabs[wv * TAB + o];
+        }
+        ws[(long)blockIdx.x * nvals + i] = val;
     }
 }
 
@@ -899,6 +1066,48 @@
 #undef BF_MODE
 }
 
+template <int KS, int WPB>
+int go_bwd_axial(const bf16* qkv, const bf16* dout, bf16* dqkv, int frames, int h, int w, int heads, Par p, const float* hscale_y, Grd gr, float* dhscale_y,
+                 float* ws, long ws_floats, int* rows_out, hipStream_t st) {
+    constexpr int D = 32 * KS;
+    const size_t shm = (size_t)WPB * (BwdTiles<1, KS>::PER_WAVE * sizeof(bf16) + (32 * 16 + 32) * sizeof(float));
+    if (int rc = set_lds(attn_bwd_axial_mfma<KS, WPB>, shm)) return rc;
+    const long ntile = (long)frames * heads;
+    BF_REQUIRE(ntile < (1L << 31) && (long)frames * h * w < (1L << 31), "attention: tile and token counts must fit 31 bits");
+    const int nvals = 4 * D + 34 * heads;
+    static int cus = 0;
+    if (!cus) {
+        int dev = 0, n = 256;
+        (void)hipGetDevice(&dev);
+        (void)hipDeviceGetAttribute(&n, hipDeviceAttributeMultiprocessorCount, dev);
+        cus = n > 0 ? n : 256;
+    }
+    long grid = std::min<long>(ntile, cus);
+    if (ws_floats < grid * nvals) grid = ws_floats / nvals;
+    if (!ws || grid < 1) return 1;
+    static const int mixed = bf_knob("BF_ATTN_AXIAL_BWD_MIXED", 1);
+    hipLaunchKernelGGL((attn_bwd_axial_mfma<KS, WPB>), dim3((int)grid), dim3(WPB * 64), shm, st, qkv, dout, dqkv, frames, h, w, heads, p, hscale_y,
+                       0.5f, gr.demb ? 1 : 0, mixed, 1, 2, 5, ws);
+    BF_CHECK_LAUNCH();
+    if (rows_out) { *rows_out = (int)grid; return 0; }
+    AttnReduceJob j[2];
+    const int nj = bf_attn_axial_bwd_jobs(ws, (int)grid, D, heads, gr.dqw, gr.dqb, gr.dkw, gr.dkb, gr.demb, gr.dhscale, dhscale_y, j);
+    for (int i = 0; i < nj; ++i) {
+        hipLaunchKernelGGL(attn_ws_reduce, dim3(bf_cdiv(4 * D + 33 * heads, 64), 1), dim3(64 * BF_RED_FL), 0, st, j[i]);
+        BF_CHECK_LAUNCH();
+    }
+    return 0;
+}
+
+}
+
+int bf_attn_axial_bwd_jobs(const float* ws, int rows, int D, int heads, float* dqw, float* dqb, float* dkw, float* dkb, float* demb, float* dhscale_x,
+                           float* dhscale_y, AttnReduceJob* out) {
+    const int stride = 4 * D + 34 * heads;
+    out[0] = AttnReduceJob{ws, rows, D, heads, dqw, dqb, dkw, dkb, demb, dhscale_x, stride};
+    if (!dhscale_y) return 1;
+    out[1] = AttnReduceJob{ws + heads, rows, D, heads, nullptr, nullptr, nullptr, nullptr, nullptr, dhscale_y, stride};
+    return 2;
 }
 
 int bf_attn_fwd_mfma(const void* qkv, void* out, long nseq, int L, long inner, long outer_stride, long inner_stride, long tok_stride, int heads,
@@ -937,6 +1146,19 @@
     BF_CHECK_LAUNCH();
     return 0;
 }
+int bf_attn_axial_bwd_mfma(const void* qkv, const void* dout, void* dqkv, int frames, int h, int w, int heads, int d, const float* qw, const float* qb,
+                           const float* kw, const float* kb, const float* emb, const float* hscale_x, const float* hscale_y, float* dqw, float* dqb,
+                           float* dkw, float* dkb, float* demb, float* dhscale_x, float* dhscale_y, float* ws, long ws_floats, int* rows_out,
+                           hipStream_t st) {
+    if (h > 16 || w > 16 || h < 1 || w < 1 || d % 32 || d > 128 || d < 32 || heads > 16 || heads < 1) return 1;
+    Par p{qw, qb, kw, kb, emb, hscale_x};
+    Grd gr{dqw, dqb, dkw, dkb, demb, dhscale_x};
+#define GO(KS, WPB) if (d == 32 * KS) return go_bwd_axial<KS, WPB>((const bf16*)qkv, (const bf16*)dout, (bf16*)dqkv, frames, h, w, heads, p, hscale_y, gr, dhscale_y, \
+                                                                   ws, ws_floats, rows_out, st)
+    GO(1, 8); GO(2, 8); GO(3, 4); GO(4, 4);
+#undef GO
+    return 1;
+}
 int bf_attn_bwd_mfma(const void* qkv, const void* dout, void* dqkv, long nseq, int L, long inner, long outer_stride, long inner_stride,
                      long tok_stride, int heads, int d, const float* qw, const float* qb, const float* kw, const float* kb, const float* emb,
                      const float* hscale, float* dqw, float* dqb, float* dkw, float* dkb, float* demb, float* dhscale, float out_scale,
diff --git a/bubbleformer_amd/csrc/model.hip b/bubbleformer_amd/csrc/model.hip
--- a/bubbleformer_amd/csrc/model.hip
+++ b/bubbleformer_amd/csrc/model.hip
@@ -759,6 +759,21 @@
         int rows = 0;
         static const bool raw_on = bf_knob("BF_ATTN_RAW", 1) != 0;
         const bool rawm = raw_on && bf_attn_raw_modes(d.dtype, d.d);
+        int fused = 1;
+        if (rawm) {
+            float *dhx = d.attn_scale ? g->attn_scale_factor_x : nullptr, *dhy = d.attn_scale ? g->attn_scale_factor_y : nullptr;
+            fused = bf_attn_axial_bwd_partials(d.dtype, sv.qkv, dO, dqkv, d.F, (int)d.h, (int)d.w, d.heads, d.d, p->qnorm_w, p->qnorm_b, p->knorm_w, p->knorm_b,
+                                               p->rel_pos_emb, d.attn_scale ? p->attn_scale_factor_x : nullptr, d.attn_scale ? p->attn_scale_factor_y : nullptr,
+                                               g->qnorm_w, g->qnorm_b, g->knorm_w, g->knorm_b, g->rel_pos_emb, dhx, dhy, sc.attn_ws, Scratch::ATTN_WS_FLOATS,
+                                               &rows, st);
+            if (fused < 0) return fused;
+            if (fused == 0) {
+                AttnReduceJob aj[2];
+                const int nj = bf_attn_axial_bwd_jobs(sc.attn_ws, rows, d.d, d.heads, g->qnorm_w, g->qnorm_b, g->knorm_w, g->knorm_b, g->rel_pos_emb, dhx, dhy, aj);
+                for (int i = 0; i < nj; ++i) TRY(jobs.push(aj[i]));
+            }
+        }
+        if (fused != 0) {
         TRY(bf_attn_bwd_partials(d.dtype, sv.qkv, dO, dqkv, d.F * d.h, d.w, 1, d.w, 0, 1, d.heads, d.d, p->qnorm_w, p->qnorm_b, p->knorm_w, p->knorm_b,
                                  p->rel_pos_emb, d.attn_scale ? p->attn_scale_factor_x : nullptr, g->qnorm_w, g->qnorm_b, g->knorm_w, g->knorm_b,
                                  g->rel_pos_emb, d.attn_scale ? g->attn_scale_factor_x : nullptr, 0.5f, rawm ? 2 : 0, sc.attn_ws, Scratch::ATTN_WS_FLOATS, &rows, st));
@@ -769,6 +784,7 @@
                                  g->rel_pos_emb, d.attn_scale ? g->attn_scale_factor_y : nullptr, 0.5f, rawm ? 5 : 1, sc.attn_ws2, Scratch::ATTN_WS_FLOATS, &rows, st));
         TRY(jobs.push(AttnReduceJob{sc.attn_ws2, rows, d.d, d.heads, g->qnorm_w, g->qnorm_b, g->knorm_w, g->knorm_b, g->rel_pos_emb,
                                     d.attn_scale ? g->attn_scale_factor_y : nullptr}));
+        }
     }
     void* dxn = sc.e6;
     InFuse fu1{x, dx1, dx, sv.mean1, sv.rstd1, p->norm1_w, p->norm1_b, sc.in_ws};
diff --git a/bubbleformer_amd/csrc/param_reduce.h b/bubbleformer_amd/csrc/param_reduce.h
--- a/bubbleformer_amd/csrc/param_reduce.h
+++ b/bubbleformer_amd/csrc/param_reduce.h
@@ -5,7 +5,9 @@
     const float* ws; int frames, C; const float *w, *b, *g; int gdiv; float *dw, *db, *dg, *dgb; const float* mask; float* dmask_v;
     __host__ __device__ int rdiv() const { return (dg || dgb) ? (gdiv > 0 ? gdiv : 1) : (frames > 0 ? frames : 1); }
 };
-struct AttnReduceJob { const float* ws; int rows, D, heads; float *dqw, *dqb, *dkw, *dkb, *demb, *dhscale; };
+struct AttnReduceJob { const float* ws; int rows, D, heads; float *dqw, *dqb, *dkw, *dkb, *demb, *dhscale; int stride; };
+int bf_attn_axial_bwd_jobs(const float* ws, int rows, int D, int heads, float* dqw, float* dqb, float* dkw, float* dkb, float* demb, float* dhscale_x,
+                           float* dhscale_y, AttnReduceJob* out);
 
 constexpr int BF_RED_FL = 16;
 template <int FL>
@@ -85,17 +87,18 @@
     const int i = bx * 64 + l;
     const int per = (j.rows + ny - 1) / ny;
     const int r0 = by * per, r1 = min(j.rows, r0 + per);
+    const long ld = j.stride > 0 ? j.stride : nvals;
     float acc = 0.f;
     if (i < nvals) {
         int r = r0 + rg;
         for (; r + 15 * FL < r1; r += 16 * FL) {
             float v[16];
 #pragma unroll
-            for (int u = 0; u < 16; ++u) v[u] = j.ws[(long)(r + FL * u) * nvals + i];
+            for (int u = 0; u < 16; ++u) v[u] = j.ws[(long)(r + FL * u) * ld + i];
 #pragma unroll
             for (int u = 0; u < 16; ++u) acc += v[u];
         }
-        for (; r < r1; r += FL) acc += j.ws[(long)r * nvals + i];
+        for (; r < r1; r += FL) acc += j.ws[(long)r * ld + i];
     }
     red[0][rg][l] = acc;
     __syncthreads();
diff --git a/include/bubbleformer_hip.h b/include/bubbleformer_hip.h
--- a/include/bubbleformer_hip.h
+++ b/include/bubbleformer_hip.h
@@ -115,6 +115,11 @@
                 float* dqb, float* dkw, float* dkb, float* demb, float* dhscale, float out_scale, int accumulate,
                 float* ws, int64_t ws_floats,
                 bf_stream_t stream);
+int bf_attn_axial_bwd_partials(int dtype, const void* qkv, const void* dout, void* dqkv, int64_t frames, int h, int w, int heads, int d,
+                               const float* qw, const float* qb, const float* kw, const float* kb, const float* emb, const float* hscale_x,
+                               const float* hscale_y, float* dqw, float* dqb, float* dkw, float* dkb, float* demb, float* dhscale_x,
+                               float* dhscale_y, float* ws, int64_t ws_floats, int* rows, bf_stream_t stream);
+void bf_debug_attn_axial_bwd(int on);
 
 void bf_side_defer(int on);
 int bf_side_join(bf_stream_t stream);
```
